# jklebes/MetropolisEngine

Measured on AMD Instinct MI355X. Metric: MC steps/sec (chains x sweeps) at 2^20 chains, 16 params, higher is better.
Workload: dtype f64

## Files before the change

### metropolisengine_amd/csrc/me_api.hip

```cpp
#include <algorithm>
#include <cmath>
#include <cstdlib>
#include <cstring>
#include <dlfcn.h>
#include <mutex>
#include <memory>
#include <string>
#include <atomic>
#include <chrono>
#include <vector>

#include "me_engine.h"

namespace me {

static std::vector<const KernelSet *> &registry() {
  static std::vector<const KernelSet *> sets;
  return sets;
}
static std::mutex &registry_mutex() {
  static std::mutex m;
  return m;
}
void register_kernel_set(const KernelSet *set) {
// ... 62 lines not shown
    for (int k = 0; k < j; ++k) s -= m[cre(j, k)] * m[cre(j, k)] + m[cim(j, k)] * m[cim(j, k)];
    if (!(s > 0)) return false;
    const double dg = std::sqrt(s);
    m[cdg(j)] = dg;
    for (int i = j + 1; i < nc; ++i) {
      double tr = m[cre(i, j)], ti = m[cim(i, j)];
      for (int k = 0; k < j; ++k) {
        const double ar = m[cre(i, k)], ai = m[cim(i, k)], br = m[cre(j, k)], bi = m[cim(j, k)];
        tr -= ar * br + ai * bi;
        ti -= ai * br - ar * bi;
      }
      m[cre(i, j)] = tr / dg;
      m[cim(i, j)] = ti / dg;
    }
  }
  return true;
}

static bool initial_shape_is_identity(const me_config *c) {
  if (c->covariance_real)
    for (int i = 0; i < c->n_real; ++i)
      for (int j = 0; j <= i; ++j)
        if (c->covariance_real[i * c->n_real + j] != (i == j ? 1.0 : 0.0)) return false;
  if (c->covariance_complex)
    for (int i = 0; i < c->n_complex; ++i)
      for (int j = 0; j <= i; ++j) {
        const double re = c->covariance_complex[2 * (i * c->n_complex + j)], im = c->covariance_complex[2 * (i * c->n_complex + j) + 1];
        if (re != (i == j ? 1.0 : 0.0) || (i != j && im != 0.0)) return false;
      }
  return true;
}

int fail(me_engine *e, int code, const std::string &msg) {
  if (e) e->err = msg;
  else g_create_error = msg;
  return code;
}

static void to_device_type(const double *src, size_t count, int dtype, std::vector<unsigned char> &out) {
  out.resize(count * (dtype == ME_F32 ? 4 : 8));
  if (dtype == ME_F32) {
    float *o = reinterpret_cast<float *>(out.data());
    for (size_t i = 0; i < count; ++i) o[i] = (float)src[i];
  } else {
    std::memcpy(out.data(), src, count * 8);
  }
}

hipError_t upload(DeviceBuffer &dst, const double *src, size_t count, int dtype) {
  std::vector<unsigned char> bytes;
  to_device_type(src, count, dtype, bytes);
  const hipError_t err = dst.resize(bytes.size());
  return err != hipSuccess ? err : hipMemcpy(dst.get(), bytes.data(), bytes.size(), hipMemcpyHostToDevice);
}

int refuse_stale_total(me_engine *e, const char *subject) {
  if (!e->stale_total) return ME_OK;
  return fail(e, ME_ERR_UNSUPPORTED, std::string(subject) + " not available with ME_FLAG_REFERENCE_ENERGY_LEDGERS: its two ledgers "
                                                            "make the energy of a chain ambiguous");
}

static int report_status(me_engine *e, unsigned int bits) {
  if (!bits) return ME_OK;
  ME_HIP(e, hipMemsetAsync(e->status.get(), 0, sizeof(unsigned int), e->stream));
  std::string msg = "numeric failure in at least one chain:";
  if (bits & ST_NONFINITE_ENERGY) msg += " non-finite energy;";
  if (bits & ST_BAD_PIVOT) msg += " non-positive Cholesky pivot (proposal covariance not positive definite);";
  if (bits & ST_BAD_WIDTH) msg += " sampling width <= 0;";
  return fail(e, ME_ERR_NUMERIC, msg);
}
int check_status(me_engine *e) {
  unsigned long long *scratch = e->host_scratch.get<unsigned long long>();
  ME_HIP(e, hipMemcpyAsync(&scratch[0], e->status.get(), sizeof(unsigned int), hipMemcpyDeviceToHost, e->stream));
  ME_HIP(e, hipStreamSynchronize(e->stream));
  return report_status(e, (unsigned int)scratch[0]);
}

}

using namespace me;

namespace {

int broadcast(me_engine *e, DeviceBuffer &dst, const std::vector<double> &row, bool tiled = false) {
  std::vector<unsigned char> bytes;
  to_device_type(row.data(), row.size(), e->dtype, bytes);
  ME_HIP(e, hipMemcpyAsync(e->row_dev.get(), bytes.data(), bytes.size(), hipMemcpyHostToDevice, e->stream));
  if (tiled) ME_HIP(e, launch_broadcast_tiled(dst.get(), e->row_dev.get(), (int)row.size(), e->n, e->dtype, e->stream));
  else ME_HIP(e, launch_broadcast_rows(dst.get(), e->row_dev.get(), (int)row.size(), e->n, e->dtype, e->stream));
  ME_HIP(e, hipStreamSynchronize(e->stream));
  return ME_OK;
}

template <typename T>
void gather_rows(const T *t, int comps, int64_t n_chains, double *dst) {
  for (int r = 0; r < comps; ++r)
    for (int64_t c = 0; c < n_chains; ++c) dst[c * comps + r] = (double)t[(size_t)r * n_chains + c];
}
template <typename T>
void scatter_rows(T *t, int comps, int64_t n_chains, const double *src) {
  for (int r = 0; r < comps; ++r)
    for (int64_t c = 0; c < n_chains; ++c) t[(size_t)r * n_chains + c] = (T)src[c * comps + r];
}
template <typename T>
void transpose_tiled(T *t, int entries, int64_t tile0, int64_t chain_begin, int64_t n_chains, double *dst, const double *src) {
  const size_t tile_values = (size_t)entries * 64;
  auto at = [&](int64_t c, int k) { return (size_t)((c >> 6) - tile0) * tile_values + (size_t)k * 64 + (size_t)(c & 63); };
  for (int64_t i = 0; i < n_chains; ++i)
    for (int k = 0; k < entries; ++k) {
      if (dst) dst[i * entries + k] = (double)t[at(chain_begin + i, k)];
      else t[at(chain_begin + i, k)] = (T)src[i * entries + k];
    }
}

int copy_tiled(me_engine *e, void *field_ptr, int entries, int64_t chain_begin, int64_t n_chains, double *dst, const double *src) {
  const int64_t tile0 = chain_begin >> 6, tile1 = (chain_begin + n_chains - 1) >> 6;
  const size_t tile_values = (size_t)entries * 64, n_values = (size_t)(tile1 - tile0 + 1) * tile_values;
  unsigned char *dev = (unsigned char *)field_ptr + (size_t)tile0 * tile_values * e->esize;
  std::vector<unsigned char> tmp(n_values * e->esize);
  const bool whole = (chain_begin & 63) == 0 && (((chain_begin + n_chains) & 63) == 0 || chain_begin + n_chains == e->n);
  if (dst || !whole) {
    ME_HIP(e, hipMemcpyAsync(tmp.data(), dev, tmp.size(), hipMemcpyDeviceToHost, e->stream));
    ME_HIP(e, hipStreamSynchronize(e->stream));
  }
  if (e->dtype == ME_F32) transpose_tiled(reinterpret_cast<float *>(tmp.data()), entries, tile0, chain_begin, n_chains, dst, src);
  else transpose_tiled(reinterpret_cast<double *>(tmp.data()), entries, tile0, chain_begin, n_chains, dst, src);
  if (src) {
    ME_HIP(e, hipMemcpyAsync(dev, tmp.data(), tmp.size(), hipMemcpyHostToDevice, e->stream));
    ME_HIP(e, hipStreamSynchronize(e->stream));
  }
  return dst ? check_status(e) : ME_OK;
}

int field_info(me_engine *e, int field, void **ptr, int *comps) {
  switch (field) {
    case ME_FIELD_PARAMS: *ptr = e->x.get(); *comps = e->d; return ME_OK;
    case ME_FIELD_ENERGY: *ptr = e->energy.get(); *comps = e->n_terms; return ME_OK;
    case ME_FIELD_WIDTH: *ptr = e->width.get(); *comps = e->width_rows; return ME_OK;
    case ME_FIELD_MEAN: *ptr = e->mean.get(); *comps = e->d; return ME_OK;
    case ME_FIELD_OBS_MEAN: *ptr = e->obs_mean.get(); *comps = e->nobs; return ME_OK;
    case ME_FIELD_COV:
      if (!e->cov)
        return fail(e, ME_ERR_UNSUPPORTED, "this engine keeps no per-chain covariance: for large parameter spaces it is "
                                           "kept on request only (me_config.flags: ME_FLAG_TRACK_COVARIANCE), and not "
                                           "at all where the field would pass 4 GiB");
      *ptr = e->cov.get(); *comps = e->p; return ME_OK;
    case ME_FIELD_ENERGY_TOTAL:
      if (!e->stale_total)
        return fail(e, ME_ERR_UNSUPPORTED, "this engine keeps one coherent energy ledger (sum ME_FIELD_ENERGY); a separate "
                                           "energy_total exists with ME_FLAG_REFERENCE_ENERGY_LEDGERS only");
      *ptr = e->energy.get<unsigned char>() + (size_t)e->n_terms * (size_t)e->n * e->esize; *comps = 1; return ME_OK;
    case ME_FIELD_FACTOR:
      if (!e->factor) return fail(e, ME_ERR_UNSUPPORTED, "this engine keeps no per-chain proposal factors (dimensions "
                                                         "without per-chain kernels, or a field beyond 4 GiB)");
      *ptr = e->factor.get(); *comps = e->p; return ME_OK;
    default: return fail(e, ME_ERR_INVALID, "unknown field id");
  }
}

int upload_shared_factor(me_engine *e, const double *packed) {
  ME_HIP(e, upload(e->shared_factor, packed, (size_t)e->p, e->dtype));
  if (e->shared_full) {
    std::vector<double> full((size_t)e->nr * e->nr, 0.0);
    for (int i = 0; i < e->nr; ++i)
      for (int j = 0; j <= i; ++j) full[(size_t)i * e->nr + j] = packed[i * (i + 1) / 2 + j];
    ME_HIP(e, upload(e->shared_full, full.data(), full.size(), e->dtype));
    if (e->shared_image) ME_HIP(e, e->ks->prepare_matrix(e->shared_full.get(), e->shared_image.get(), e->stream));
  }
  return ME_OK;
}

void fill_step_launch(me_engine *e, StepLaunch &l, int n_sweeps) {
  l.n_real = e->nr;
  l.n_complex = e->nc;
  l.x = e->x.get();
  l.energy = e->energy.get();
  l.width = e->width.get();
  l.factor = e->cov_kind == CK_PER_CHAIN ? e->factor.get() : e->shared_factor.get();
  l.factor_full = e->shared_full.get();
  l.factor_image = e->shared_image.get();
  l.energy_image = e->energy_image.get();
  l.coef_device = e->coef_dev.get();
  l.coef_host = e->coef.data();
  l.n_coef = (int)e->coef.size();
  l.inj_normals = nullptr;
  l.inj_uniforms = nullptr;
  l.group = GROUP_ALL;
  l.split_widths = (e->width_rows == 3 && !e->widths_synced) ? 1 : 0;
  l.stale_total = e->stale_total ? 1 : 0;
  l.cov = e->cov.get();
  l.accept_slots = e->accept_slots.get<unsigned long long>();
  l.status = e->status.get<unsigned int>();
  l.n = e->n;
  l.chain_offset = e->chain_offset;
  l.step_index = e->step_index;
  l.seed = e->seed;
  l.n_sweeps = n_sweeps;
  l.energy_kind = e->energy_kind;
  l.cov_kind = e->cov_kind;
  l.reject_kind = e->reject_kind;
  l.grid_blocks = e->grid_blocks;
  l.reject_bound = e->reject_bound;
  l.temp = e->temp;
  l.ratio = e->ratio;
  l.target_acceptance = e->target_acceptance;
  l.damping = std::max((double)e->measure_count / (double)e->m, 200.0);
  l.ladder = e->ladder.n_rungs ? e->ladder.table.get() : nullptr;
  l.tiles_per_rung = e->ladder.n_rungs ? (int)(e->n / (64ll * e->ladder.n_rungs)) : 0;
}
// ... 30 lines not shown
  return ME_OK;
}

int me_abi_version(void) { return ME_ABI_VERSION; }

int me_supported(int32_t dtype, int32_t n_real, int32_t n_complex, int32_t energy_kind) {
  return find_kernel_set(dtype, n_real, n_complex, energy_kind, nullptr) ? 1 : 0;
}

namespace {

int validate_config(const me_config *c, const KernelSet **ks_out) {
  if (c->abi_version != ME_ABI_VERSION) return fail(nullptr, ME_ERR_INVALID, "me_config.abi_version mismatch");
  if (c->n_real < 0 || c->n_complex < 0 || c->n_real + c->n_complex == 0)
    return fail(nullptr, ME_ERR_INVALID,
                "must give at least one real or complex parameter (metropolis_engine.py:37-39)");
  if (c->n_chains <= 0) return fail(nullptr, ME_ERR_INVALID, "n_chains must be positive");
  if (!(c->temp >= 0)) return fail(nullptr, ME_ERR_INVALID, "temp must be >= 0 (metropolis_engine.py:92)");
  if (!(c->target_acceptance > 0 && c->target_acceptance < 1))
    return fail(nullptr, ME_ERR_INVALID, "target_acceptance must be in (0, 1)");
  if (!(c->sampling_width > 0)) return fail(nullptr, ME_ERR_INVALID, "sampling_width must be > 0");
  if (c->dtype != ME_F32 && c->dtype != ME_F64) return fail(nullptr, ME_ERR_INVALID, "unknown dtype");
  if (!c->initial_params) return fail(nullptr, ME_ERR_INVALID, "initial_params is required");
  if (c->n_energy_coeffs < 0 || (c->n_energy_coeffs > 0 && !c->energy_coeffs))
    return fail(nullptr, ME_ERR_INVALID, "energy coefficients missing");
  int rc = check_reject_kind(nullptr, c->reject_kind, c->energy_kind, c->n_real);
  if (rc != ME_OK) return rc;
  if (c->cov_mode < ME_COV_REFERENCE || c->cov_mode > ME_COV_POOLED)
    return fail(nullptr, ME_ERR_INVALID, "unknown cov_mode");
  const KernelSet *ks = *ks_out = find_kernel_set(c->dtype, c->n_real, c->n_complex, c->energy_kind, c->user_energy_name);
  if (!ks) {
    if (is_user_kind(c->energy_kind))
      return fail(nullptr, ME_ERR_UNSUPPORTED,
                  std::string("no user-energy plugin named '") + (c->user_energy_name ? c->user_energy_name : "") +
                      "' is loaded for these dimensions (build it with metropolisengine_amd.build.build_user_energy "
                      "and load it with me_load_plugin)");
    if (!has_dims(c->dtype, c->n_real, c->n_complex))
      return fail(nullptr, ME_ERR_UNSUPPORTED,
                  "no kernel set compiled for (dtype, n_real, n_complex) = (" + std::to_string(c->dtype) + ", " +
                      std::to_string(c->n_real) + ", " + std::to_string(c->n_complex) + ")");
    return fail(nullptr, ME_ERR_UNSUPPORTED, "energy kind " + std::to_string(c->energy_kind) +
                                                  " is not compiled for these dimensions");
  }
  if ((rc = check_user_reject(nullptr, c->reject_kind, ks)) != ME_OK) return rc;
  if (ks->n_real < 0) {
    if (c->cov_mode == ME_COV_POOLED && c->n_complex > 0)
      return fail(nullptr, ME_ERR_UNSUPPORTED,
                  "parameter spaces beyond " + std::to_string(kMaxRegisterDof) + " real degrees of freedom with complex "
                  "parameters run with the identity proposal shape (ME_COV_FIXED, cov_mode=\"fixed\") or per-chain shapes "
                  "(ME_COV_REFERENCE); one shared factor (ME_COV_POOLED) is there for pure real spaces");
    const bool starts_shared = !initial_shape_is_identity(c) && c->cov_mode != ME_COV_REFERENCE;
    if (starts_shared && c->n_complex > 0)
      return fail(nullptr, ME_ERR_UNSUPPORTED,
                  "parameter spaces beyond " + std::to_string(kMaxRegisterDof) + " real degrees of freedom with complex "
                  "parameters run with the identity proposal shape only: leave covariance_matrix_real / _complex unset");
    {
      const long long per_block = (long long)(c->n_real + 2 * c->n_complex) * 64 * (c->dtype == ME_F32 ? 4 : 8);
      const bool dense = c->energy_kind == ME_ENERGY_DENSE_QUAD, pooled = c->cov_mode == ME_COV_POOLED || starts_shared;
      const bool per_chain = c->cov_mode == ME_COV_REFERENCE || (c->flags & ME_FLAG_TRACK_COVARIANCE) != 0;
      if ((dense || pooled || per_chain) && per_block * (pooled ? 2 : 1) > 150 * 1024)
        return fail(nullptr, ME_ERR_UNSUPPORTED,
                    "a dense quadratic form, a shared proposal factor or per-chain shapes beyond " + std::to_string(kMaxRegisterDof) +
                        " degrees of freedom are staged in LDS: this many parameters do not fit (float64: about 290, 145 with "
                        "a shared factor or an initial covariance that ME_COV_FIXED keeps; float32 twice that)");
    }
    if (c->flags & ME_FLAG_REFERENCE_ENERGY_LEDGERS)
      return fail(nullptr, ME_ERR_UNSUPPORTED, "ME_FLAG_REFERENCE_ENERGY_LEDGERS is not available beyond " +
                                                   std::to_string(kMaxRegisterDof) + " real degrees of freedom");
    if (c->reject_kind == ME_REJECT_USER) return fail(nullptr, ME_ERR_UNSUPPORTED, "no user plugins at these dimensions");
  }
  if ((c->flags & ME_FLAG_REFERENCE_ENERGY_LEDGERS) && (c->n_real == 0 || c->n_complex == 0))
    return fail(nullptr, ME_ERR_INVALID,
                "ME_FLAG_REFERENCE_ENERGY_LEDGERS applies to mixed engines (real and complex parameters): only their "
                "step_all keeps a separate energy_total (metropolis_engine.py:241-259)");
  if (c->cov_mode == ME_COV_REFERENCE && !ks->per_chain_cov)
    return fail(nullptr, ME_ERR_UNSUPPORTED,
                "per-chain adaptive covariance is not compiled for these dimensions; use ME_COV_FIXED or ME_COV_POOLED");
  return ME_OK;
}

struct Layout {
  bool keep_per_chain;
  bool keep_cov;
  bool x_tiled;
  int width_rows;
};
int decide_layout(const me_config *c, const KernelSet *ks, Layout &l) {
  const long long esz = c->dtype == ME_F32 ? 4 : 8, limit = 1ll << 32, padded = padded_chains(c->n_chains);
  l.keep_per_chain = ks->per_chain_cov && (!ks->streams_packed || c->cov_mode == ME_COV_REFERENCE);
  if (l.keep_per_chain && !ks->streams_packed && (long long)packed_total(c->n_real, c->n_complex) * padded * esz >= limit) {
    if (c->cov_mode == ME_COV_REFERENCE)
      return fail(nullptr, ME_ERR_UNSUPPORTED,
                  "the per-chain covariance field would exceed 4 GiB on this engine; shard the chains over more "
                  "engines or use ME_COV_FIXED / ME_COV_POOLED");
    l.keep_per_chain = false;
  }
  const long long rows = std::max<long long>(c->n_real + 2 * c->n_complex, 2 * c->n_real + c->n_complex);
  if (rows * padded * esz >= limit)
    return fail(nullptr, ME_ERR_UNSUPPORTED,
                "a per-chain field would exceed 4 GiB on this engine; shard the chains over more engines");
  l.keep_cov = l.keep_per_chain ||
               ((!ks->per_chain_cov || ks->streams_packed) && ks->tracks_cov && (c->flags & ME_FLAG_TRACK_COVARIANCE));
  l.x_tiled = ks->tiled_state;
  l.width_rows = (c->n_real > 0 && c->n_complex > 0) ? 3 : 1;
  return ME_OK;
}

std::unique_ptr<me_engine> configure(const me_config *c, const KernelSet *ks, const Layout &l) {
  std::unique_ptr<me_engine> e(new me_engine);
  e->device = c->device_id;
  e->ks = ks;
  e->n_terms = ks->energy_terms(c->energy_kind);
  e->dtype = c->dtype;
  e->esize = c->dtype == ME_F32 ? 4 : 8;
  e->n = c->n_chains;
  e->nr = c->n_real;
  e->nc = c->n_complex;
  e->d = e->nr + 2 * e->nc;
  e->p = packed_total(e->nr, e->nc);
  e->nobs = n_observables(e->nr, e->nc);
  e->chain_offset = c->chain_offset;
  e->seed = c->seed;
  e->temp = c->temp;
  e->target_acceptance = c->target_acceptance;
  e->energy_kind = c->energy_kind;
  e->reject_kind = c->reject_kind;
  e->reject_bound = c->reject_bound;
  e->cov_mode = c->cov_mode;
  e->coef.assign(c->energy_coeffs, c->energy_coeffs + c->n_energy_coeffs);
  e->alpha = -norm_ppf(c->target_acceptance / 2.0);
  e->m = e->nr + e->nc;
  e->ratio = (1.0 - 1.0 / e->m) * std::sqrt(2.0 * M_PI) * std::exp(e->alpha * e->alpha / 2.0) / 2.0 * e->alpha +
             1.0 / (e->m * c->target_acceptance * (1.0 - c->target_acceptance));
  if (const char *g = std::getenv("ME_GRID_BLOCKS")) e->grid_blocks = std::atoi(g);
  e->x_tiled = l.x_tiled;
  e->stale_total = (c->flags & ME_FLAG_REFERENCE_ENERGY_LEDGERS) != 0;
  e->width_rows = l.width_rows;
  e->n_slots = (e->n + 31) / 32 + 8;
  return e;
}

int allocate(me_engine *e, const Layout &l) {
  const KernelSet *ks = e->ks;
  ME_HIP(e, hipSetDevice(e->device));
  ME_HIP(e, e->stream.create());
  const size_t n = (size_t)e->n, tiles = (size_t)padded_chains(e->n), es = e->esize;
  ME_HIP(e, e->x.resize((e->x_tiled ? tiles : n) * e->d * es));
  ME_HIP(e, e->energy.resize(n * (e->n_terms + (e->stale_total ? 1 : 0)) * es));
  ME_HIP(e, e->width.resize(n * e->width_rows * es));
  ME_HIP(e, e->mean.resize(n * e->d * es));
  ME_HIP(e, e->obs_mean.resize(n * e->nobs * es));
  if (l.keep_cov) ME_HIP(e, e->cov.resize(tiles * e->p * es));
  if (l.keep_per_chain) ME_HIP(e, e->factor.resize(tiles * e->p * es));
  ME_HIP(e, e->shared_factor.resize((size_t)e->p * es));
  if (e->nc == 0) ME_HIP(e, e->shared_full.resize((size_t)e->nr * e->nr * es));
  if (e->shared_full && ks->prepare_matrix) ME_HIP(e, e->shared_image.resize(ks->matrix_image_bytes));
  ME_HIP(e, e->row_dev.resize((size_t)std::max(std::max(e->d, e->p), e->nobs) * es));
  ME_HIP(e, e->accept_slots.resize((size_t)e->n_slots * sizeof(unsigned long long)));
  ME_HIP(e, e->accept_total.resize(sizeof(unsigned long long)));
  ME_HIP(e, e->status.resize(sizeof(unsigned int)));
  const size_t moments_bytes = sizeof(double) * (size_t)moments_size(e->nr, e->nc);
  ME_HIP(e, e->pool.dev.resize(moments_bytes));
  ME_HIP(e, e->host_scratch.allocate(64));
  e->host_scratch.get<unsigned long long>()[0] = e->host_scratch.get<unsigned long long>()[1] = 0;
  ME_HIP(e, e->pool.host.allocate(moments_bytes));
  if (pool_reduce_supported(e->nr, e->nc, e->dtype))
    ME_HIP(e, e->pool.partials.resize(sizeof(double) * (size_t)pool_reduce_blocks(e->n, e->nr, e->nc) *
                                      (size_t)(1 + e->d + e->nr + e->nc + e->d * (e->d + 1) / 2)));
  ME_HIP(e, hipMemsetAsync(e->accept_slots.get(), 0, e->accept_slots.bytes(), e->stream));
  ME_HIP(e, hipMemsetAsync(e->status.get(), 0, sizeof(unsigned int), e->stream));
  return ME_OK;
}

int upload_coefficients(me_engine *e) {
  const std::vector<double> &coef = e->coef;
  const bool runtime_dims = e->ks->n_real < 0;
  std::vector<double> form;
  if (runtime_dims && e->energy_kind == ME_ENERGY_DIAG_QUAD) {
    if ((int)coef.size() != e->nr + e->nc) return fail(e, ME_ERR_INVALID, "wrong number of energy coefficients for this energy kind");
    form.assign(coef.begin(), coef.end());
    form.insert(form.end(), coef.begin() + e->nr, coef.end());
  } else if (runtime_dims && e->energy_kind == ME_ENERGY_DENSE_QUAD) {
    if ((int)coef.size() != e->d * e->d) return fail(e, ME_ERR_INVALID, "wrong number of energy coefficients for this energy kind");
    form.reserve((size_t)e->d * (e->d + 1) / 2);
    for (int i = 0; i < e->d; ++i)
      for (int j = 0; j <= i; ++j)
        form.push_back(i == j ? coef[(size_t)i * e->d + i] : coef[(size_t)i * e->d + j] + coef[(size_t)j * e->d + i]);
  } else if (e->energy_kind == ME_ENERGY_DENSE_QUAD || (is_user_kind(e->energy_kind) && !coef.empty())) {
    form = coef;
  } else {
    return ME_OK;
  }
  ME_HIP(e, upload(e->coef_dev, form.data(), form.size(), e->dtype));
  if (!runtime_dims && e->energy_kind == ME_ENERGY_DENSE_QUAD && e->ks->prepare_matrix) {
    ME_HIP(e, e->energy_image.resize(e->ks->matrix_image_bytes));
    ME_HIP(e, e->ks->prepare_matrix(e->coef_dev.get(), e->energy_image.get(), e->stream));
  }
  return ME_OK;
}

int initial_state(me_engine *e, const me_config *c) {
  std::vector<double> init(c->initial_params, c->initial_params + e->d);
  std::vector<double> obs(e->nobs);
  for (int i = 0; i < e->nr; ++i) {
    obs[i] = std::fabs(init[i]);
    obs[e->nr + e->nc + i] = init[i] * init[i];
  }
  for (int j = 0; j < e->nc; ++j) obs[e->nr + j] = std::hypot(init[e->nr + j], init[e->nr + e->nc + j]);
  const int pr = packed_real(e->nr);
  std::vector<double> c0(e->p, 0.0);
  bool identity = true;
  for (int i = 0; i < e->nr; ++i)
    for (int j = 0; j <= i; ++j) {
      const double v = c->covariance_real ? c->covariance_real[i * e->nr + j] : (i == j ? 1.0 : 0.0);
      c0[i * (i + 1) / 2 + j] = v;
      identity = identity && v == (i == j ? 1.0 : 0.0);
    }
  for (int i = 0; i < e->nc; ++i) {
    for (int j = 0; j < i; ++j) {
      const double re = c->covariance_complex ? c->covariance_complex[2 * (i * e->nc + j)] : 0.0;
      const double im = c->covariance_complex ? c->covariance_complex[2 * (i * e->nc + j) + 1] : 0.0;
      c0[pr + i * i + 2 * j] = re;
      c0[pr + i * i + 2 * j + 1] = im;
      identity = identity && re == 0.0 && im == 0.0;
    }
    const double dg = c->covariance_complex ? c->covariance_complex[2 * (i * e->nc + i)] : 1.0;
    c0[pr + i * i + 2 * i] = dg;
    identity = identity && dg == 1.0;
  }
  std::vector<double> f0 = c0;
  for (int i = 0; i < e->nc; ++i)
    for (int j = 0; j < i; ++j) f0[pr + i * i + 2 * j + 1] = -f0[pr + i * i + 2 * j + 1];
  if (!host_factor(f0, e->nr, e->nc))
    return fail(e, ME_ERR_INVALID, "initial covariance matrix is not positive definite (metropolis_engine.py:270)");
  int rc = ME_OK;
  std::vector<double> width_row((size_t)e->width_rows, c->sampling_width);
  if ((rc = broadcast(e, e->x, init, e->x_tiled)) || (rc = broadcast(e, e->mean, init)) || (rc = broadcast(e, e->obs_mean, obs)) ||
      (rc = broadcast(e, e->width, width_row)) || (e->cov && (rc = broadcast(e, e->cov, c0, true))) ||
      (e->factor && (rc = broadcast(e, e->factor, f0, true))) || (rc = upload_shared_factor(e, f0.data())))
    return rc;
  e->cov_kind = identity ? CK_IDENTITY : (e->ks->n_real < 0 && e->factor) ? CK_PER_CHAIN : CK_SHARED;
  return ME_OK;
}

int initial_energy(me_engine *e) {
  const int rc = me_recompute_energy(e);
  if (rc != ME_OK) return rc;
  const hipError_t herr = hipStreamSynchronize(e->stream);
  if (herr != hipSuccess) return fail(e, ME_ERR_HIP, std::string("initial energy evaluation: ") + hipGetErrorString(herr));
  return ME_OK;
}

}

int me_create(const me_config *c, me_engine **out) {
  if (!c || !out) return fail(nullptr, ME_ERR_INVALID, "null config or output pointer");
  *out = nullptr;
  const KernelSet *ks = nullptr;
  Layout layout;
  int rc;
  if ((rc = validate_config(c, &ks)) || (rc = decide_layout(c, ks, layout))) return rc;
  int n_dev = 0;
  if (hipGetDeviceCount(&n_dev) != hipSuccess || n_dev <= 0)
    return fail(nullptr, ME_ERR_HIP, "no HIP device available (this library has no CPU fallback)");
  if (c->device_id < 0 || c->device_id >= n_dev) return fail(nullptr, ME_ERR_INVALID, "device_id out of range");

  std::unique_ptr<me_engine> e = configure(c, ks, layout);
  if ((rc = allocate(e.get(), layout)) || (rc = upload_coefficients(e.get())) || (rc = initial_state(e.get(), c)) ||
      (rc = initial_energy(e.get())))
    return fail(nullptr, rc, e->err);
  *out = e.release();
  return ME_OK;
}

int me_set_reject_condition(me_engine *e, int32_t reject_kind, double reject_bound) {
  if (!e) return ME_ERR_INVALID;
  int rc;
  if ((rc = check_reject_kind(e, reject_kind, e->energy_kind, e->nr)) || (rc = check_user_reject(e, reject_kind, e->ks))) return rc;
  e->reject_kind = reject_kind;
  e->reject_bound = reject_bound;
  return ME_OK;
}

int me_set_energy(me_engine *e, int32_t energy_kind, const double *coeffs, int32_t n_coeffs, const char *user_name) {
  if (!e) return ME_ERR_INVALID;
  if (n_coeffs < 0 || (n_coeffs > 0 && !coeffs)) return fail(e, ME_ERR_INVALID, "energy coefficients missing");
  if (e->ks->n_real < 0) return fail(e, ME_ERR_UNSUPPORTED, "me_set_energy: not available on the runtime-dimension kernel set");
  if (energy_kind == ME_ENERGY_DENSE_QUAD)
    return fail(e, ME_ERR_UNSUPPORTED, "me_set_energy: the dense quadratic form keeps device images of its matrix; create a new engine");
  const KernelSet *ks = find_kernel_set(e->dtype, e->nr, e->nc, energy_kind, user_name);
  if (!ks || ks->n_real < 0)
    return fail(e, ME_ERR_UNSUPPORTED, is_user_kind(energy_kind)
                    ? std::string("no user-energy plugin named '") + (user_name ? user_name : "") + "' is loaded for these dimensions"
                    : "energy kind " + std::to_string(energy_kind) + " is not compiled for these dimensions");
  if (ks->tiled_state != e->ks->tiled_state || ks->per_chain_cov != e->ks->per_chain_cov || ks->streams_packed != e->ks->streams_packed ||
      ks->tracks_cov != e->ks->tracks_cov)
    return fail(e, ME_ERR_UNSUPPORTED, "me_set_energy: the plugin was built with other per-chain covariance options than this engine's kernel set");
  if (e->reject_kind == ME_REJECT_USER && !ks->has_user_reject)
    return fail(e, ME_ERR_UNSUPPORTED, "me_set_energy: the engine's wall is the plugin's me_user_reject, which the new energy does not define");
  const int n_terms = ks->energy_terms(energy_kind);
  ME_HIP(e, hipSetDevice(e->device));
  ME_HIP(e, hipStreamSynchronize(e->stream));
  DeviceBuffer ledger, coef_dev;
  if (n_terms != e->n_terms)
    ME_HIP(e, ledger.resize((size_t)e->n * (size_t)(n_terms + (e->stale_total ? 1 : 0)) * e->esize));
  if (is_user_kind(energy_kind) && n_coeffs > 0) ME_HIP(e, upload(coef_dev, coeffs, (size_t)n_coeffs, e->dtype));
  if (n_terms != e->n_terms) {
    e->energy = std::move(ledger);
    e->n_terms = n_terms;
    if (e->trace.chains > 0) e->trace.restart();
  }
  e->coef.assign(coeffs, coeffs + n_coeffs);
  e->coef_dev = std::move(coef_dev);
  e->ks = ks;
  e->energy_kind = energy_kind;
  const int rc = me_recompute_energy(e);
  if (rc != ME_OK) return rc;
  ME_HIP(e, hipStreamSynchronize(e->stream));
  return check_status(e);
}

int me_load_plugin(const char *path) {
  if (!path) return fail(nullptr, ME_ERR_INVALID, "null plugin path");
  void *handle = dlopen(path, RTLD_NOW | RTLD_GLOBAL);
  if (!handle) return fail(nullptr, ME_ERR_INVALID, std::string("dlopen failed: ") + dlerror());
  return ME_OK;
}

int me_destroy(me_engine *e) {
  if (!e) return ME_ERR_INVALID;
  (void)hipSetDevice(e->device);
  if (e->stream) (void)hipStreamSynchronize(e->stream);
  if (e->pool.copy_stream) (void)hipStreamSynchronize(e->pool.copy_stream);
  delete e;
  return ME_OK;
}

int me_recompute_energy(me_engine *e) {
  if (!e) return ME_ERR_INVALID;
  ME_HIP(e, hipSetDevice(e->device));
  EnergyLaunch l;
  l.n_real = e->nr;
  l.n_complex = e->nc;
  l.total_row = e->stale_total ? e->n_terms : -1;
  l.x = e->x.get();
  l.energy = e->energy.get();
  l.coef_device = e->coef_dev.get();
  l.coef_host = e->coef.data();
  l.n_coef = (int)e->coef.size();
  l.status = e->status.get<unsigned int>();
  l.n = e->n;
  l.energy_kind = e->energy_kind;
  l.grid_blocks = e->grid_blocks;
  hipError_t err = e->ks->init_energy(l, e->stream);
  if (err == hipErrorInvalidValue) return fail(e, ME_ERR_INVALID, "wrong number of energy coefficients for this energy kind");
  ME_HIP(e, err);
  return ME_OK;
}

static int split_widths(me_engine *e) {
  if (e->width_rows != 3 || !e->widths_synced) return ME_OK;
  const size_t row = (size_t)e->n * e->esize;
  for (int r = 1; r <= 2; ++r)
    ME_HIP(e, hipMemcpyAsync(e->width.get<unsigned char>() + r * row, e->width.get(), row, hipMemcpyDeviceToDevice, e->stream));
  e->widths_synced = false;
  return ME_OK;
}

static int resolve_step_kind(me_engine *e, int kind, int *group, bool *magphase) {
  *magphase = false;
  *group = GROUP_ALL;
  const bool mixed = e->nr > 0 && e->nc > 0;
  switch (kind) {
    case ME_STEP_ALL: return ME_OK;
    case ME_STEP_REAL_GROUP:
      if (e->nr == 0) return fail(e, ME_ERR_INVALID, "this engine has no real parameters");
      *group = mixed ? GROUP_REAL : GROUP_ALL;
      return ME_OK;
// ... 28 lines not shown
  l.group = group;
  l.inj_normals = inj_normals;
  l.inj_uniforms = inj_uniforms;
  hipError_t err = magphase ? e->ks->magphase(l, e->stream) : e->ks->step(l, e->stream);
  if (err == hipErrorNotSupported) return fail(e, ME_ERR_UNSUPPORTED, "this step kind is not compiled for this engine");
  ME_HIP(e, err);
  count_steps(e, n_sweeps, group, magphase);
  return ME_OK;
}

int me_step(me_engine *e, int32_t n_sweeps) { return me_step_kind(e, ME_STEP_ALL, n_sweeps); }

int me_step_kind(me_engine *e, int32_t kind, int32_t n_sweeps) {
  if (!e) return ME_ERR_INVALID;
  if (n_sweeps <= 0) return fail(e, ME_ERR_INVALID, "n_sweeps must be positive");
  ME_HIP(e, hipSetDevice(e->device));
  return launch_step_kind(e, kind, n_sweeps, nullptr, nullptr);
}

int me_step_injected(me_engine *e, int32_t kind, int32_t n_sweeps, const double *normals, const double *uniforms) {
  if (!e || !normals || !uniforms) return ME_ERR_INVALID;
  if (n_sweeps <= 0) return fail(e, ME_ERR_INVALID, "n_sweeps must be positive");
  if (e->dtype != ME_F64) return fail(e, ME_ERR_UNSUPPORTED, "injected-stream replay is compiled for float64 engines only");
  ME_HIP(e, hipSetDevice(e->device));
  const bool magphase = kind == ME_STEP_COMPLEX_MAGNITUDE_PHASE;
  const size_t n = (size_t)e->n, k = (size_t)n_sweeps;
  const size_t nz = magphase ? (size_t)e->nc : (size_t)e->d, nu = magphase ? (size_t)e->nc + 2 : 1;
  std::vector<double> zn(k * nz * n), un(k * nu * n);
  for (size_t s = 0; s < k; ++s)
    for (size_t c = 0; c < n; ++c) {
      for (size_t j = 0; j < nz; ++j) zn[(s * nz + j) * n + c] = normals[(s * n + c) * nz + j];
      for (size_t j = 0; j < nu; ++j) un[(s * nu + j) * n + c] = uniforms[(s * n + c) * nu + j];
    }
  DeviceBuffer zd, ud;
  ME_HIP(e, zd.resize(zn.size() * sizeof(double)));
  if (ud.resize(un.size() * sizeof(double)) != hipSuccess) return fail(e, ME_ERR_HIP, "hipMalloc of the injected uniforms failed");
  if (hipMemcpy(zd.get(), zn.data(), zd.bytes(), hipMemcpyHostToDevice) != hipSuccess ||
      hipMemcpy(ud.get(), un.data(), ud.bytes(), hipMemcpyHostToDevice) != hipSuccess)
    return fail(e, ME_ERR_HIP, "upload of the injected streams failed");
  int rc = launch_step_kind(e, kind, n_sweeps, zd.get(), ud.get());
  if (rc == ME_OK && hipStreamSynchronize(e->stream) != hipSuccess) rc = fail(e, ME_ERR_HIP, "injected step failed");
  return rc;
}

namespace {
void fill_measure_launch(me_engine *e, MeasureLaunch &l, unsigned long long count) {
  l.n_real = e->nr;
  l.n_complex = e->nc;
  l.x = e->x.get();
  l.width = e->width.get();
  l.mean = e->mean.get();
  l.cov = e->cov.get();
  l.obs_mean = e->obs_mean.get();
  l.factor = e->factor.get();
  l.status = e->status.get<unsigned int>();
  l.n = e->n;
  l.measure_count = count;
  l.update_cov = (count > 50 && e->cov) ? 1 : 0;
  l.split_widths = (e->width_rows == 3 && !e->widths_synced) ? 1 : 0;
  l.write_factor = (l.update_cov && e->cov_mode == ME_COV_REFERENCE) ? 1 : 0;
  l.grid_blocks = e->grid_blocks;
}

int commit_measure(me_engine *e, const MeasureLaunch &l) {
  e->measure_count = l.measure_count;
  if (l.write_factor) e->cov_kind = CK_PER_CHAIN;
  if (e->trace.chains > 0) {
    const long long cols = e->d + e->n_terms + e->width_rows;
    if (e->trace.rows == e->trace.capacity) {
      const long long cap = e->trace.capacity ? 2 * e->trace.capacity : 1024;
      DeviceBuffer bigger;
      ME_HIP(e, bigger.resize(sizeof(double) * (size_t)(cap * cols * e->trace.chains)));
      if (e->trace.dev) {
        ME_HIP(e, hipMemcpyAsync(bigger.get(), e->trace.dev.get(), sizeof(double) * (size_t)(e->trace.rows * cols * e->trace.chains),
                                 hipMemcpyDeviceToDevice, e->stream));
        ME_HIP(e, hipStreamSynchronize(e->stream));
      }
      e->trace.dev = std::move(bigger);
      e->trace.capacity = cap;
    }
    const int rows_valid = (e->width_rows == 3 && e->widths_synced) ? 1 : e->width_rows;
    double *row = e->trace.dev.get<double>() + e->trace.rows * cols * e->trace.chains;
    ME_HIP(e, launch_trace(e->x.get(), e->energy.get(), e->width.get(), e->n, e->d, e->n_terms, rows_valid, e->dtype, e->trace.chains,
                           e->trace.stride, row, e->stream, e->x_tiled));
    if (rows_valid != e->width_rows) {
      double *widths = row + (size_t)(e->d + e->n_terms) * e->trace.chains;
      for (int r = 1; r < 3; ++r)
        ME_HIP(e, hipMemcpyAsync(widths + (size_t)r * e->trace.chains, widths, sizeof(double) * (size_t)e->trace.chains,
                                 hipMemcpyDeviceToDevice, e->stream));
    }
    e->trace.rows += 1;
  }
  return ME_OK;
}
}

int me_measure(me_engine *e) {
  if (!e) return ME_ERR_INVALID;
  ME_HIP(e, hipSetDevice(e->device));
  MeasureLaunch l;
  fill_measure_launch(e, l, e->measure_count + 1);
  ME_HIP(e, e->ks->measure(l, e->stream));
  return commit_measure(e, l);
}

int me_cycle(me_engine *e, int32_t n_sweeps) {
  if (!e) return ME_ERR_INVALID;
  if (n_sweeps <= 0) return fail(e, ME_ERR_INVALID, "n_sweeps must be positive");
  ME_HIP(e, hipSetDevice(e->device));
  if (e->ks->cycle) {
    StepLaunch sl;
    fill_step_launch(e, sl, n_sweeps);
    MeasureLaunch ml;
    fill_measure_launch(e, ml, e->measure_count + 1);
    ml.split_widths = 0;
    const hipError_t err = e->ks->cycle(sl, ml, e->stream);
    if (err == hipSuccess) {
      count_steps(e, n_sweeps);
      e->fused_cycles += 1;
      return commit_measure(e, ml);
    }
    if (err != hipErrorNotSupported) ME_HIP(e, err);
    (void)hipGetLastError();
  }
  const int rc = me_step(e, n_sweeps);
  return rc != ME_OK ? rc : me_measure(e);
}

int me_cycle_stats(me_engine *e, uint64_t *fused_cycles) {
  if (!e || !fused_cycles) return ME_ERR_INVALID;
  *fused_cycles = e->fused_cycles;
  return ME_OK;
}

int me_trace_enable(me_engine *e, int64_t n_traced, int64_t stride) {
  if (!e) return ME_ERR_INVALID;
  if (n_traced < 0 || stride < 1 || (n_traced > 0 && (n_traced - 1) * stride >= e->n))
    return fail(e, ME_ERR_INVALID, "traced chains out of range");
  ME_HIP(e, hipSetDevice(e->device));
  ME_HIP(e, hipStreamSynchronize(e->stream));
  e->trace.restart();
  e->trace.chains = n_traced;
  e->trace.stride = stride;
  return ME_OK;
}

int me_trace_shape(me_engine *e, int64_t *rows, int64_t *cols, int64_t *n_traced) {
  if (!e) return ME_ERR_INVALID;
  if (rows) *rows = e->trace.rows;
  if (cols) *cols = e->d + e->n_terms + e->width_rows;
  if (n_traced) *n_traced = e->trace.chains;
  return ME_OK;
}

int me_trace_get(me_engine *e, double *dst, int64_t n_doubles) {
  if (!e || !dst) return ME_ERR_INVALID;
  const long long want = e->trace.rows * (e->d + e->n_terms + e->width_rows) * e->trace.chains;
  if (n_doubles != want) return fail(e, ME_ERR_INVALID, "wrong trace buffer length");
  if (want == 0) return ME_OK;
  ME_HIP(e, hipSetDevice(e->device));
  ME_HIP(e, hipStreamSynchronize(e->stream));
  ME_HIP(e, hipMemcpy(dst, e->trace.dev.get(), sizeof(double) * (size_t)want, hipMemcpyDeviceToHost));
  return ME_OK;
}

int me_field_components(me_engine *e, int32_t field, int32_t *n_components) {
  if (!e || !n_components) return ME_ERR_INVALID;
  void *ptr;
  int comps;
  int rc = field_info(e, field, &ptr, &comps);
  if (rc == ME_OK) *n_components = comps;
  return rc;
}

int me_energy_terms(me_engine *e, int32_t *n_terms) {
  if (!e || !n_terms) return ME_ERR_INVALID;
  *n_terms = e->n_terms;
  return ME_OK;
}

int me_get(me_engine *e, int32_t field, int64_t chain_begin, int64_t n_chains, double *dst) {
  if (!e || !dst) return ME_ERR_INVALID;
  if (chain_begin < 0 || n_chains < 0 || chain_begin + n_chains > e->n) return fail(e, ME_ERR_INVALID, "chain range out of bounds");
  ME_HIP(e, hipSetDevice(e->device));
  void *ptr;
  int comps;
  int rc = field_info(e, field, &ptr, &comps);
  if (rc != ME_OK) return rc;
  if (n_chains == 0) return ME_OK;
  if (field == ME_FIELD_COV || field == ME_FIELD_FACTOR || (field == ME_FIELD_PARAMS && e->x_tiled))
    return copy_tiled(e, ptr, comps, chain_begin, n_chains, dst, nullptr);
  std::vector<unsigned char> tmp((size_t)comps * n_chains * e->esize);
  for (int r = 0; r < comps; ++r)
    ME_HIP(e, hipMemcpyAsync(tmp.data() + (size_t)r * n_chains * e->esize,
                             (const unsigned char *)ptr + ((size_t)r * e->n + chain_begin) * e->esize,
                             (size_t)n_chains * e->esize, hipMemcpyDeviceToHost, e->stream));
  ME_HIP(e, hipStreamSynchronize(e->stream));
  if (e->dtype == ME_F32) gather_rows(reinterpret_cast<const float *>(tmp.data()), comps, n_chains, dst);
  else gather_rows(reinterpret_cast<const double *>(tmp.data()), comps, n_chains, dst);
  if (field == ME_FIELD_WIDTH && e->width_rows == 3 && e->widths_synced)
    for (int64_t c = 0; c < n_chains; ++c) dst[c * 3 + 1] = dst[c * 3 + 2] = dst[c * 3];
  return check_status(e);
}

int me_set(me_engine *e, int32_t field, int64_t chain_begin, int64_t n_chains, const double *src) {
  if (!e || !src) return ME_ERR_INVALID;
  if (chain_begin < 0 || n_chains < 0 || chain_begin + n_chains > e->n) return fail(e, ME_ERR_INVALID, "chain range out of bounds");
  ME_HIP(e, hipSetDevice(e->device));
  void *ptr;
  int comps;
  int rc = field_info(e, field, &ptr, &comps);
  if (rc != ME_OK) return rc;
  if (field == ME_FIELD_WIDTH && e->width_rows == 3 && (chain_begin != 0 || n_chains != e->n))
    return fail(e, ME_ERR_INVALID, "widths of a mixed engine must be set for all chains at once");
  if (n_chains == 0) return ME_OK;
  if (field == ME_FIELD_COV || field == ME_FIELD_FACTOR || (field == ME_FIELD_PARAMS && e->x_tiled)) {
    rc = copy_tiled(e, ptr, comps, chain_begin, n_chains, nullptr, src);
    if (rc != ME_OK) return rc;
    if (field == ME_FIELD_FACTOR) e->cov_kind = CK_PER_CHAIN;
    return ME_OK;
  }
  std::vector<unsigned char> tmp((size_t)comps * n_chains * e->esize);
  if (e->dtype == ME_F32) scatter_rows(reinterpret_cast<float *>(tmp.data()), comps, n_chains, src);
  else scatter_rows(reinterpret_cast<double *>(tmp.data()), comps, n_chains, src);
  for (int r = 0; r < comps; ++r)
    ME_HIP(e, hipMemcpyAsync((unsigned char *)ptr + ((size_t)r * e->n + chain_begin) * e->esize,
                             tmp.data() + (size_t)r * n_chains * e->esize, (size_t)n_chains * e->esize,
                             hipMemcpyHostToDevice, e->stream));
  ME_HIP(e, hipStreamSynchronize(e->stream));
  if (field == ME_FIELD_FACTOR) e->cov_kind = CK_PER_CHAIN;
  if (field == ME_FIELD_WIDTH && e->width_rows == 3) e->widths_synced = false;
  return ME_OK;
}

int me_constants(me_engine *e, double *alpha, int32_t *m, double *ratio) {
  if (!e) return ME_ERR_INVALID;
  if (alpha) *alpha = e->alpha;
  if (m) *m = e->m;
  if (ratio) *ratio = e->ratio;
  return ME_OK;
}

int me_counters(me_engine *e, uint64_t *step_index, uint64_t *measure_step_counter) {
  if (!e) return ME_ERR_INVALID;
  if (step_index) *step_index = e->step_index;
  if (measure_step_counter) *measure_step_counter = e->measure_count;
  return ME_OK;
}

int me_set_counters(me_engine *e, uint64_t step_index, uint64_t measure_step_counter) {
  if (!e) return ME_ERR_INVALID;
  if (measure_step_counter < 1) return fail(e, ME_ERR_INVALID, "measure_step_counter starts at 1");
  e->step_index = step_index;
  e->measure_count = measure_step_counter;
  return ME_OK;
}

int me_accept_stats(me_engine *e, uint64_t *accepted, uint64_t *proposed) {
  if (!e) return ME_ERR_INVALID;
  ME_HIP(e, hipSetDevice(e->device));
  unsigned long long *scratch = e->host_scratch.get<unsigned long long>();
  ME_HIP(e, launch_sum_slots(e->accept_slots.get<unsigned long long>(), e->n_slots, e->accept_total.get<unsigned long long>(), e->stream));
  ME_HIP(e, hipMemcpyAsync(&scratch[1], e->accept_total.get(), sizeof(unsigned long long), hipMemcpyDeviceToHost, e->stream));
  ME_HIP(e, hipMemcpyAsync(&scratch[0], e->status.get(), sizeof(unsigned int), hipMemcpyDeviceToHost, e->stream));
  ME_HIP(e, hipStreamSynchronize(e->stream));
  if (accepted) *accepted = scratch[1];
  if (proposed) *proposed = e->proposed;
  return report_status(e, (unsigned int)scratch[0]);
}

int me_set_accept_stats(me_engine *e, uint64_t accepted, uint64_t proposed) {
  if (!e) return ME_ERR_INVALID;
  if (accepted > proposed) return fail(e, ME_ERR_INVALID, "accepted exceeds proposed");
  ME_HIP(e, hipSetDevice(e->device));
  const unsigned long long total = accepted;
  ME_HIP(e, hipMemsetAsync(e->accept_slots.get(), 0, e->accept_slots.bytes(), e->stream));
  ME_HIP(e, hipMemcpyAsync(e->accept_slots.get(), &total, sizeof(total), hipMemcpyHostToDevice, e->stream));
  ME_HIP(e, hipStreamSynchronize(e->stream));
  e->proposed = proposed;
  return ME_OK;
}

int me_pooled_moments_size(me_engine *e, int64_t *n_doubles) {
  if (!e || !n_doubles) return ME_ERR_INVALID;
  *n_doubles = moments_size(e->nr, e->nc);
  return ME_OK;
}

int me_pooled_moments_geometry(me_engine *e, int32_t *matrix_core, int32_t *tile_chains, int32_t *partial_rows) {
  if (!e || !matrix_core || !tile_chains || !partial_rows) return ME_ERR_INVALID;
  if (!e->pool.partials) return fail(e, ME_ERR_UNSUPPORTED, "pooled moments: dimension too large for the reduction kernel");
  *matrix_core = e->ks->pool_stage1 ? 1 : 0;
  *tile_chains = e->ks->pool_stage1 ? 64 : pool_tile_chains(e->nr, e->nc, e->dtype);
  *partial_rows = pool_reduce_blocks(e->n, e->nr, e->nc);
  return ME_OK;
}

namespace {
hipError_t wait_polling(hipEvent_t ev) {
  const auto t0 = std::chrono::steady_clock::now();
  for (;;) {
    const hipError_t rc = hipEventQuery(ev);
    if (rc != hipErrorNotReady) return rc;
    if (std::chrono::steady_clock::now() - t0 > std::chrono::milliseconds(2)) return hipEventSynchronize(ev);
  }
}
hipError_t wait_polling(hipStream_t stream) {
  const auto t0 = std::chrono::steady_clock::now();
  for (;;) {
    const hipError_t rc = hipStreamQuery(stream);
    if (rc != hipErrorNotReady) return rc;
    if (std::chrono::steady_clock::now() - t0 > std::chrono::milliseconds(2)) return hipStreamSynchronize(stream);
  }
}

int check_pooled(me_engine *e, int64_t n_doubles) {
  if (n_doubles != moments_size(e->nr, e->nc)) return fail(e, ME_ERR_INVALID, "wrong pooled-moment buffer length");
  if (e->pool.pending) return fail(e, ME_ERR_STATE, "a pooled-moment reduction is in flight (me_pooled_moments_end first)");
  if (!e->pool.partials) return fail(e, ME_ERR_UNSUPPORTED, "pooled moments: dimension too large for the reduction kernel");
  ME_HIP(e, hipSetDevice(e->device));
  return ME_OK;
}
int enqueue_pool_reduce(me_engine *e, const void *x, long long n_chains, long long n_slots, double proposed, double *device_out) {
  hipError_t err = launch_pool_reduce(x, n_chains, e->nr, e->nc, e->dtype, e->accept_slots.get<unsigned long long>(), n_slots, proposed,
                                      e->pool.partials.get<double>(), device_out, e->stream, e->ks->pool_stage1, e->x_tiled);
  if (err == hipErrorInvalidValue) return fail(e, ME_ERR_UNSUPPORTED, "pooled moments: dimension too large for the reduction kernel");
  ME_HIP(e, err);
  return ME_OK;
}
int enqueue_pooled_moments(me_engine *e, double *device_out, int64_t n_doubles) {
  const int rc = check_pooled(e, n_doubles);
  return rc != ME_OK ? rc : enqueue_pool_reduce(e, e->x.get(), e->n, e->n_slots, (double)e->proposed, device_out);
}
int fetch_pooled_moments(me_engine *e, double *host_out, int64_t n_doubles) {
  const size_t bytes = sizeof(double) * (size_t)n_doubles;
  ME_HIP(e, hipMemcpyAsync(e->pool.host.get<double>(), e->pool.dev.get(), bytes, hipMemcpyDeviceToHost, e->stream));
  ME_HIP(e, wait_polling(e->stream));
  std::memcpy(host_out, e->pool.host.get<double>(), bytes);
  return ME_OK;
}
}

int me_pooled_moments_device(me_engine *e, void *device_out, int64_t n_doubles) {
  if (!e || !device_out) return ME_ERR_INVALID;
  int rc = enqueue_pooled_moments(e, (double *)device_out, n_doubles);
  if (rc != ME_OK) return rc;
  ME_HIP(e, wait_polling(e->stream));
  return ME_OK;
}

int me_pooled_moments(me_engine *e, double *host_out, int64_t n_doubles) {
  if (!e || !host_out) return ME_ERR_INVALID;
  const int rc = enqueue_pooled_moments(e, e->pool.dev.get<double>(), n_doubles);
  return rc != ME_OK ? rc : fetch_pooled_moments(e, host_out, n_doubles);
}

int me_pooled_moments_range(me_engine *e, int64_t chain_begin, int64_t n_chains, double *host_out, int64_t n_doubles) {
  if (!e || !host_out) return ME_ERR_INVALID;
  if (chain_begin < 0 || n_chains <= 0 || chain_begin + n_chains > e->n || chain_begin % 64 != 0 || n_chains % 64 != 0)
    return fail(e, ME_ERR_INVALID, "the chain range must be whole 64-chain tiles inside the engine");
  int rc = check_pooled(e, n_doubles);
  if (rc != ME_OK) return rc;
  const unsigned char *x = e->x.get<unsigned char>();
  if (e->x_tiled) {
    x += (size_t)chain_begin * e->d * e->esize;
  } else {
    const size_t row = (size_t)n_chains * e->esize;
    if (row * e->d > e->pool.range_x.bytes()) {
      ME_HIP(e, hipStreamSynchronize(e->stream));
      ME_HIP(e, e->pool.range_x.reserve(row * e->d));
    }
    ME_HIP(e, hipMemcpy2DAsync(e->pool.range_x.get(), row, x + (size_t)chain_begin * e->esize, (size_t)e->n * e->esize, row, (size_t)e->d,
                               hipMemcpyDeviceToDevice, e->stream));
    x = e->pool.range_x.get<unsigned char>();
  }
  if ((rc = enqueue_pool_reduce(e, x, n_chains, 0, 0.0, e->pool.dev.get<double>())) != ME_OK) return rc;
  return fetch_pooled_moments(e, host_out, n_doubles);
}

namespace {
int begin_pooled(me_engine *e, bool allreduce) {
  if (e->pool.pending) return fail(e, ME_ERR_STATE, "a pooled-moment reduction is already in flight: call me_pooled_moments_end first");
  if (allreduce && !e->comm)
    return fail(e, ME_ERR_STATE, "this engine has no communicator: call me_comm_init_rank first (single-GPU engines use me_pooled_moments)");
  ME_HIP(e, hipSetDevice(e->device));
  if (!e->pool.copy_stream) {
    ME_HIP(e, e->pool.copy_stream.create());
    ME_HIP(e, e->pool.reduced.create(hipEventDisableTiming));
    ME_HIP(e, e->pool.copied.create(hipEventDisableTiming));
  }
  const int64_t n_doubles = moments_size(e->nr, e->nc);
  int rc = enqueue_pooled_moments(e, e->pool.dev.get<double>(), n_doubles);
  if (rc != ME_OK) return rc;
  ME_HIP(e, hipEventRecord(e->pool.reduced, e->stream));
  ME_HIP(e, hipStreamWaitEvent(e->pool.copy_stream, e->pool.reduced, 0));
  if (allreduce) {
    const ncclResult_t nrc = e->rccl->all_reduce(e->pool.dev.get<double>(), e->pool.dev.get<double>(), (size_t)n_doubles, ncclDouble, ncclSum, e->comm, e->pool.copy_stream);
    if (nrc != ncclSuccess) return fail(e, ME_ERR_HIP, std::string("ncclAllReduce: ") + e->rccl->error_string(nrc));
  }
  ME_HIP(e, hipMemcpyAsync(e->pool.host.get<double>(), e->pool.dev.get<double>(), sizeof(double) * (size_t)n_doubles, hipMemcpyDeviceToHost, e->pool.copy_stream));
  ME_HIP(e, hipEventRecord(e->pool.copied, e->pool.copy_stream));
  e->pool.pending = true;
  return ME_OK;
}
}

int me_pooled_moments_begin(me_engine *e) {
  if (!e) return ME_ERR_INVALID;
  return begin_pooled(e, false);
}

int me_pooled_moments_allreduce_begin(me_engine *e) {
  if (!e) return ME_ERR_INVALID;
  return begin_pooled(e, true);
}

int me_pooled_moments_allreduce(me_engine *e, double *host_out, int64_t n_doubles) {
  if (!e || !host_out) return ME_ERR_INVALID;
  if (n_doubles != moments_size(e->nr, e->nc)) return fail(e, ME_ERR_INVALID, "wrong pooled-moment buffer length");
  const int rc = begin_pooled(e, true);
  return rc != ME_OK ? rc : me_pooled_moments_end(e, host_out, n_doubles);
}

int me_comm_unique_id(void *id_out, size_t bytes) {
  if (!id_out || bytes != ME_COMM_ID_BYTES) return fail(nullptr, ME_ERR_INVALID, "the unique id is ME_COMM_ID_BYTES bytes");
  static_assert(sizeof(ncclUniqueId) == ME_COMM_ID_BYTES, "ME_COMM_ID_BYTES must be sizeof(ncclUniqueId)");
  std::string err;
  const RcclApi *api = rccl_api(&err);
  if (!api) return fail(nullptr, ME_ERR_UNSUPPORTED, err);
  ncclUniqueId id;
  const ncclResult_t nrc = api->get_unique_id(&id);
  if (nrc != ncclSuccess) return fail(nullptr, ME_ERR_HIP, std::string("ncclGetUniqueId: ") + api->error_string(nrc));
  std::memcpy(id_out, &id, sizeof(id));
  return ME_OK;
}

int me_comm_init_rank(me_engine *e, const void *unique_id, size_t bytes, int32_t rank, int32_t world) {
  if (!e || !unique_id) return ME_ERR_INVALID;
  if (bytes != ME_COMM_ID_BYTES) return fail(e, ME_ERR_INVALID, "the unique id is ME_COMM_ID_BYTES bytes");
  if (world < 1 || rank < 0 || rank >= world) return fail(e, ME_ERR_INVALID, "rank out of range");
  if (e->comm) return fail(e, ME_ERR_STATE, "this engine already has a communicator (me_comm_destroy first)");
  if (e->pool.pending) return fail(e, ME_ERR_STATE, "a pooled-moment reduction is in flight");
  std::string err;
  const RcclApi *api = rccl_api(&err);
  if (!api) return fail(e, ME_ERR_UNSUPPORTED, err);
  ME_HIP(e, hipSetDevice(e->device));
  ncclUniqueId id;
// ... 118 lines not shown
```

### metropolisengine_amd/csrc/me_device.h

```cpp
#pragma once

#include <type_traits>
#include <utility>

#include <hip/hip_runtime.h>
#include <stdint.h>

#include "me_internal.h"
#include "me_math64.h"

namespace me {

struct U4 {
  uint32_t x, y, z, w;
};

__device__ __forceinline__ uint32_t xor3(uint32_t a, uint32_t b, uint32_t c) {
  return __builtin_amdgcn_bitop3_b32(a, b, c, 0x96);
}
__device__ __forceinline__ U4 philox4x32_10(U4 c, uint32_t k0, uint32_t k1) {
#pragma unroll
  for (int r = 0; r < 10; ++r) {
    const uint64_t p0 = (uint64_t)0xD2511F53u * c.x;
    const uint64_t p1 = (uint64_t)0xCD9E8D57u * c.z;
// ... 129 lines not shown
  __device__ __forceinline__ void store(int row, unsigned int chain_off, R value) const {
    if constexpr (sizeof(R) == 4) {
      __builtin_amdgcn_raw_buffer_store_b32(__builtin_bit_cast(unsigned int, value), rsrc, chain_off,
                                            (unsigned int)row * row_bytes, 0);
    } else {
      using v2 = decltype(__builtin_amdgcn_raw_buffer_load_b64(rsrc, 0u, 0u, 0));
      __builtin_amdgcn_raw_buffer_store_b64(__builtin_bit_cast(v2, value), rsrc, chain_off,
                                            (unsigned int)row * row_bytes, 0);
    }
  }
};

template <typename R>
__device__ __forceinline__ R chain_energy(const Field<R> &fe, unsigned int chain_off, int n_terms) {
  R e = fe.load(0, chain_off);
  for (int t = 1; t < n_terms; ++t) e = e + fe.load(t, chain_off);
  return e;
}

template <typename R>
__device__ __forceinline__ unsigned int tiled_offset(long long c, int entries) {
  return (unsigned int)(((c >> 6) * (long long)entries * 64 + (c & 63)) * (long long)sizeof(R));
}
template <typename R>
struct TiledField {
  __amdgpu_buffer_rsrc_t rsrc;
  __device__ __forceinline__ TiledField(const R *base, long long n, int entries)
      : rsrc(__builtin_amdgcn_make_buffer_rsrc(const_cast<R *>(base), 0,
                                               (unsigned int)(((n + 63) >> 6) * (long long)entries * 64 * (long long)sizeof(R)),
                                               0x00020000)) {}
  static constexpr unsigned int kEntryBytes = 64u * (unsigned int)sizeof(R);
  template <int AUX>
  __device__ __forceinline__ R load_aux(int k, unsigned int tile_off) const {
    if constexpr (sizeof(R) == 4) {
      return __builtin_bit_cast(R, __builtin_amdgcn_raw_buffer_load_b32(rsrc, tile_off, (unsigned int)k * kEntryBytes, AUX));
    } else {
      const auto v = __builtin_amdgcn_raw_buffer_load_b64(rsrc, tile_off, (unsigned int)k * kEntryBytes, AUX);
      return __builtin_bit_cast(R, v);
    }
  }
  template <int AUX>
  __device__ __forceinline__ void store_aux(int k, unsigned int tile_off, R value) const {
    if constexpr (sizeof(R) == 4) {
      __builtin_amdgcn_raw_buffer_store_b32(__builtin_bit_cast(unsigned int, value), rsrc, tile_off, (unsigned int)k * kEntryBytes, AUX);
    } else {
      using v2 = decltype(__builtin_amdgcn_raw_buffer_load_b64(rsrc, 0u, 0u, 0));
      __builtin_amdgcn_raw_buffer_store_b64(__builtin_bit_cast(v2, value), rsrc, tile_off, (unsigned int)k * kEntryBytes, AUX);
    }
  }
  __device__ __forceinline__ R load(int k, unsigned int tile_off) const { return load_aux<0>(k, tile_off); }
  __device__ __forceinline__ R load_nt(int k, unsigned int tile_off) const { return load_aux<ME_NT_AUX>(k, tile_off); }
  __device__ __forceinline__ void store(int k, unsigned int tile_off, R value) const { store_aux<0>(k, tile_off, value); }
  __device__ __forceinline__ void store_nt(int k, unsigned int tile_off, R value) const { store_aux<ME_NT_AUX>(k, tile_off, value); }
};

template <bool NT, class F>
__device__ __forceinline__ auto packed_load(const F &f, int row, unsigned int chain_off) {
  if constexpr (NT) return f.load_nt(row, chain_off);
  else return f.load(row, chain_off);
}
template <bool NT, class F, typename R>
__device__ __forceinline__ void packed_store(const F &f, int row, unsigned int chain_off, R value) {
  if constexpr (NT) f.store_nt(row, chain_off, value);
  else f.store(row, chain_off, value);
}

template <typename R, bool NTS>
struct StateField : Field<R> {
  using Field<R>::Field;
  __device__ __forceinline__ R load(int row, unsigned int chain_off) const {
    if constexpr (NTS) return Field<R>::load_nt(row, chain_off);
    else return Field<R>::load(row, chain_off);
  }
  __device__ __forceinline__ void store(int row, unsigned int chain_off, R value) const {
    if constexpr (NTS) Field<R>::store_nt(row, chain_off, value);
    else Field<R>::store(row, chain_off, value);
  }
};

#ifndef ME_TILED_STATE_DOF
#define ME_TILED_STATE_DOF 16
#endif
constexpr int kTiledStateDof = ME_TILED_STATE_DOF;
template <typename R, int D, bool NTS = false>
struct XField {
  static constexpr bool kTiled = D >= kTiledStateDof;
  std::conditional_t<kTiled, TiledField<R>, StateField<R, NTS>> f;
  __device__ __forceinline__ XField(const R *base, long long n) : f(base, n, D) {}
  static __device__ __forceinline__ unsigned int offset(long long c) {
    if constexpr (kTiled) return tiled_offset<R>(c, D);
    else return (unsigned int)c * (unsigned int)sizeof(R);
  }
  __device__ __forceinline__ R load(int row, unsigned int off) const {
    if constexpr (kTiled && NTS) return f.load_nt(row, off);
    else return f.load(row, off);
  }
  __device__ __forceinline__ void store(int row, unsigned int off, R value) const {
    if constexpr (kTiled && NTS) f.store_nt(row, off, value);
    else f.store(row, off, value);
  }
};
template <typename R, int D>
__device__ __forceinline__ long long state_index(long long c, int row, long long n) {
  if constexpr (D >= kTiledStateDof) return ((c >> 6) * (long long)D + row) * 64 + (c & 63);
  else return (long long)row * n + c;
}

constexpr int kMaxPackedInRegisters = 160;
#ifndef ME_STREAM_F64_ENTRIES
#define ME_STREAM_F64_ENTRIES 96
#endif
constexpr int kStreamF64Entries = ME_STREAM_F64_ENTRIES;

template <typename R, int NR, int NC>
struct EnergyIso {
  static constexpr int D = NR + 2 * NC;
  R a;
  __device__ __forceinline__ R operator()(const R (&x)[D]) const {
    R s0 = 0, s1 = 0;
#pragma unroll
    for (int d = 0; d + 1 < D; d += 2) {
      s0 += x[d] * x[d];
      s1 += x[d + 1] * x[d + 1];
    }
    if constexpr (D % 2 == 1) s0 += x[D - 1] * x[D - 1];
    return a * (s0 + s1);
  }
};

template <typename R, int NR, int NC>
struct EnergyDiag {
  static constexpr int D = NR + 2 * NC;
  R w[D];
  __device__ __forceinline__ R operator()(const R (&x)[D]) const {
    R s0 = 0, s1 = 0;
#pragma unroll
    for (int d = 0; d + 1 < D; d += 2) {
      s0 += w[d] * x[d] * x[d];
      s1 += w[d + 1] * x[d + 1] * x[d + 1];
    }
    if constexpr (D % 2 == 1) s0 += w[D - 1] * x[D - 1] * x[D - 1];
    return s0 + s1;
  }
};

template <typename R, int NR, int NC>
struct EnergyDense {
  static constexpr int D = NR + 2 * NC;
  static constexpr int PT = D * (D + 1) / 2;
  const R *a;
  static __device__ __forceinline__ R *folded() {
    __shared__ R t[PT];
    return t;
  }
  __device__ __forceinline__ void prepare() const {
    R *t = folded();
    constexpr int kBatch = 8;
    for (int k0 = threadIdx.x; k0 < PT; k0 += kBatch * (int)blockDim.x) {
      R lo[kBatch], hi[kBatch];
#pragma unroll
      for (int u = 0; u < kBatch; ++u) {
        const int k = k0 + u * (int)blockDim.x;
        lo[u] = hi[u] = R(0);
        if (k < PT) {
          int i = (int)((__builtin_sqrtf((float)(8 * k + 1)) - 1.0f) * 0.5f);
          if ((i + 1) * (i + 2) / 2 <= k) ++i;
          if (i * (i + 1) / 2 > k) --i;
          const int j = k - i * (i + 1) / 2;
          lo[u] = a[i * D + j];
          if (i != j) hi[u] = a[j * D + i];
        }
      }
#pragma unroll
      for (int u = 0; u < kBatch; ++u) {
        const int k = k0 + u * (int)blockDim.x;
        if (k < PT) t[k] = lo[u] + hi[u];
      }
    }
    __syncthreads();
  }
  __device__ __forceinline__ R operator()(const R (&x)[D]) const {
    const R *t = folded();
    asm volatile("" ::: "memory");
    R e = 0;
#pragma unroll
    for (int i = 0; i < D; ++i) {
      R y = 0;
#pragma unroll
// ... 237 lines not shown
  constexpr int NW = 2 * ((D + 1) / 2);
  constexpr int NBLK = (NW + 1 + 3) / 4;
  using N_ = Num<R>;
  [[maybe_unused]] const unsigned long long step = a.step_index + (unsigned long long)s;
  if constexpr (INJECT) {
#pragma unroll
    for (int j = 0; j < D; ++j) g[j] = a.inj_normals[((long long)s * D + j) * a.n + c];
    u = a.inj_uniforms[(long long)s * a.n + c];
  } else {
    uint32_t words[4 * NBLK];
#pragma unroll
    for (int b = 0; b < NBLK; ++b) {
      const U4 o = philox_block(gid, step, b, a.seed_lo, a.seed_hi);
      words[4 * b + 0] = o.x;
      words[4 * b + 1] = o.y;
      words[4 * b + 2] = o.z;
      words[4 * b + 3] = o.w;
    }
#pragma unroll
    for (int q = 0; q < NW / 2; ++q) N_::normal_pair(words[2 * q], words[2 * q + 1], g[2 * q], g[2 * q + 1]);
    u = N_::unit(words[NW]);
  }

}

template <typename R, int NR, int NC, int CK, int GROUP, class Fac>
__device__ __forceinline__ void propose_registers(const R (&x)[NR + 2 * NC], const R (&g)[2 * ((NR + 2 * NC + 1) / 2)], R w_r, R w_c,
                                                  Fac &&fac, R (&xp)[NR + 2 * NC]) {
  constexpr int D = NR + 2 * NC;
  [[maybe_unused]] constexpr int PR = NR * (NR + 1) / 2;
  constexpr bool MOVE_REAL = NR > 0 && GROUP != GROUP_COMPLEX;
  constexpr bool MOVE_COMPLEX = NC > 0 && GROUP != GROUP_REAL;
#pragma unroll
  for (int d = 0; d < D; ++d) xp[d] = x[d];
  if constexpr (CK == CK_IDENTITY) {
    if constexpr (MOVE_REAL) {
#pragma unroll
      for (int i = 0; i < NR; ++i) xp[i] = x[i] + w_r * g[i];
    }
    if constexpr (MOVE_COMPLEX) {
#pragma unroll
      for (int j = 0; j < NC; ++j) {
        xp[NR + j] = x[NR + j] + w_c * (g[NR + j] * R(0.70710678118654752440));
        xp[NR + NC + j] = x[NR + NC + j] + w_c * (g[NR + NC + j] * R(0.70710678118654752440));
      }
    }
  } else {
    if constexpr (MOVE_REAL) {
#pragma unroll
      for (int i = 0; i < NR; ++i) {
        R acc = 0;
#pragma unroll
        for (int j = 0; j <= i; ++j) acc += fac(tri(i, j)) * g[j];
        xp[i] = x[i] + w_r * acc;
      }
    }
    if constexpr (MOVE_COMPLEX) {
#pragma unroll
      for (int i = 0; i < NC; ++i) {
        R are = 0, aim = 0;
#pragma unroll
        for (int j = 0; j < i; ++j) {
          const R lre = fac(cre(PR, i, j));
          const R lim = fac(cim(PR, i, j));
          const R wre = g[NR + j] * R(0.70710678118654752440), wim = g[NR + NC + j] * R(0.70710678118654752440);
          are += lre * wre - lim * wim;
          aim += lre * wim + lim * wre;
        }
        const R ld = fac(cdiag(PR, i));
        are += ld * (g[NR + i] * R(0.70710678118654752440));
        aim += ld * (g[NR + NC + i] * R(0.70710678118654752440));
        xp[NR + i] = x[NR + i] + w_c * are;
        xp[NR + NC + i] = x[NR + NC + i] + w_c * aim;
      }
    }
  }

}

template <typename R, int NR, int NC, class Energy, int CK, int GROUP, bool LADDER, class Ledger>
__device__ __forceinline__ void decide_step(const StepArgs<R> &a, long long c, const Energy &en, bool stale_total, R u,
                                            const R (&g)[2 * ((NR + 2 * NC + 1) / 2)], R (&x)[NR + 2 * NC], const R (&xp)[NR + 2 * NC],
                                            Ledger &ledger, R &total_q5, R &w, R &w_r, R &w_c, unsigned int &wave_accepted,
                                            bool &bad_energy) {
  [[maybe_unused]] constexpr int D = NR + 2 * NC;
  constexpr bool MOVE_REAL = NR > 0 && GROUP != GROUP_COMPLEX;
  constexpr bool MOVE_COMPLEX = NC > 0 && GROUP != GROUP_REAL;
  using N_ = Num<R>;
  bool rejected = false;
  if (a.reject_kind == ME_REJECT_ABS_REAL0_GE) rejected = !(N_::abs_(xp[0]) < a.reject_bound);
  else if (a.reject_kind == ME_REJECT_USER) rejected = energy_reject(en, xp, 0);
  R terms_new[Ledger::T];
  const R e_new = ledger.propose(en, xp, terms_new);
  const R diff = e_new - (stale_total ? total_q5 : ledger.partial());
  bool accept = diff <= R(0);
  if constexpr (LADDER) accept = accept || uphill_at<true>(a, c, u, diff);
  else if (a.temp > R(0)) accept = accept || N_::uphill(u, diff, a.inv_temp, a.inv_temp_log2e);
  accept = accept && !rejected;
  bad_energy |= (!rejected && !N_::finite(e_new));
  if constexpr (CK == CK_IDENTITY) {
    const R wa_r = accept ? w_r : R(0), wa_c = accept ? w_c : R(0);
    if constexpr (MOVE_REAL) {
#pragma unroll
      for (int i = 0; i < NR; ++i) x[i] = x[i] + wa_r * g[i];
    }
    if constexpr (MOVE_COMPLEX) {
#pragma unroll
      for (int j = 0; j < NC; ++j) {
        x[NR + j] = x[NR + j] + wa_c * (g[NR + j] * R(0.70710678118654752440));
        x[NR + NC + j] = x[NR + NC + j] + wa_c * (g[NR + NC + j] * R(0.70710678118654752440));
      }
    }
  } else {
#pragma unroll
    for (int d = 0; d < D; ++d) x[d] = accept ? xp[d] : x[d];
  }
  if (stale_total) total_q5 = accept ? e_new : total_q5;
  else ledger.commit(accept, terms_new);
  w = N_::adapt(w, accept, a.ratio, a.p, a.damping, a.up, a.down);
  if constexpr (GROUP == GROUP_ALL) w_r = w_c = w;
  else if constexpr (GROUP == GROUP_REAL) w_r = w;
  else w_c = w;
  wave_accepted += (unsigned int)__popcll(__ballot(accept));
}

template <typename R, int NR, int NC, class Energy, int CK, bool INJECT, int GROUP, bool LADDER, class Ledger, class Fac>
__device__ __forceinline__ void run_sweeps(const StepArgs<R> &a, const Energy &en, long long c, unsigned long long gid,
                                           bool stale_total, R (&x)[NR + 2 * NC], Ledger &ledger, R &total_q5, R &w, R &w_r,
                                           R &w_c, Fac &&fac, unsigned int &wave_accepted, bool &bad_energy) {
  constexpr int D = NR + 2 * NC;
  constexpr int NW = 2 * ((D + 1) / 2);
  for (int s = 0; s < a.n_sweeps; ++s) {
    R g[NW], u, xp[D];
    draw_step<R, NR, NC, INJECT>(a, c, gid, s, g, u);
    propose_registers<R, NR, NC, CK, GROUP>(x, g, w_r, w_c, fac, xp);
    decide_step<R, NR, NC, Energy, CK, GROUP, LADDER>(a, c, en, stale_total, u, g, x, xp, ledger, total_q5, w, w_r, w_c, wave_accepted, bad_energy);
  }
}

#ifndef ME_STEP_WAVES_PER_EU
#define ME_STEP_WAVES_PER_EU 0
#endif
#if ME_STEP_WAVES_PER_EU > 0
#define ME_STEP_BOUNDS __launch_bounds__(kFusedStepThreads, ME_STEP_WAVES_PER_EU)
#else
#define ME_STEP_BOUNDS __launch_bounds__(kFusedStepThreads)
#endif

#ifndef ME_STEP_PRIO_SHIFT
#define ME_STEP_PRIO_SHIFT 8
#endif
__device__ __forceinline__ void stagger_priority() {
#if ME_STEP_PRIO_SHIFT >= 0
  switch ((blockIdx.x >> ME_STEP_PRIO_SHIFT) & 3u) {
    case 0: __builtin_amdgcn_s_setprio(3); break;
    case 1: __builtin_amdgcn_s_setprio(2); break;
    case 2: __builtin_amdgcn_s_setprio(1); break;
    default: break;
  }
#endif
}

template <typename R, int NR, int NC, class Energy, int CK, bool INJECT = false, int GROUP = GROUP_ALL, bool NTS = false,
          bool LADDER = false>
__global__ void ME_STEP_BOUNDS k_step(StepArgs<R> a, Energy en) {
  constexpr int D = NR + 2 * NC;
  constexpr bool MIXED = NR > 0 && NC > 0;
  static_assert(GROUP == GROUP_ALL || MIXED, "group-wise kernels exist for mixed engines only");
  using N_ = Num<R>;

  stagger_priority();
  if constexpr (!INJECT) N_::prepare();
  energy_prepare(en, 0);
  unsigned int wave_accepted = 0;
  bool bad_energy = false, bad_width = false;
  const long long stride = (long long)gridDim.x * blockDim.x;
  using Ledger = EnergyLedger<R, Energy, GROUP>;
  const XField<R, D, NTS> fx(a.x, a.n);
  const StateField<R, NTS> fe(a.energy, a.n, Ledger::T + (MIXED ? 1 : 0)), fw(a.width, a.n, MIXED ? 3 : 1);
  const bool stale_total = MIXED && GROUP == GROUP_ALL && a.stale_total != 0;
  constexpr bool PER_CHAIN = CK == CK_PER_CHAIN || CK == CK_PER_CHAIN_NT;
  constexpr int PF = PER_CHAIN ? NR * (NR + 1) / 2 + NC * NC : 0;
  constexpr bool STREAM_FACTOR = PER_CHAIN && (PF > kMaxPackedInRegisters ||
                                               (!INJECT && sizeof(R) == 8 && NC == 0 && PF > kStreamF64Entries));
  const TiledField<R> ffac(a.factor, a.n, STREAM_FACTOR ? 0 : PF);
  for (long long c = (long long)blockIdx.x * blockDim.x + threadIdx.x; c < a.n; c += stride) {
    const unsigned int coff = (unsigned int)c * (unsigned int)sizeof(R);
    const unsigned int xoff = fx.offset(c);
    R x[D];
#pragma unroll
    for (int d = 0; d < D; ++d) x[d] = fx.load(d, xoff);
    Ledger ledger;
    R total_q5 = R(0);
    if (stale_total) total_q5 = fe.load(Ledger::T, coff);
    else ledger.load(fe, coff);
    R w = fw.load(MIXED ? GROUP : 0, coff);
    R w_r = w, w_c = w;
    if constexpr (MIXED && GROUP == GROUP_ALL) {
      if (a.split_widths) {
        w_r = fw.load(GROUP_REAL, coff);
        w_c = fw.load(GROUP_COMPLEX, coff);
      }
    }
    const unsigned long long gid = a.chain_offset + (unsigned long long)c;
    [[maybe_unused]] const unsigned int toff = tiled_offset<R>(c, PF);
    auto fac = [&](int k) -> R {
      if constexpr (CK == CK_PER_CHAIN_NT) return ffac.load_nt(k, toff);
      else if constexpr (CK == CK_PER_CHAIN) return ffac.load(k, toff);
      else return a.factor[k];
    };

    if constexpr (STREAM_FACTOR) {
      constexpr int NW = 2 * ((D + 1) / 2);
      for (int s = 0; s < a.n_sweeps; ++s) {
        static_assert(!INJECT, "the streamed-factor form has no replay hook");
        constexpr int NBLK = (NW + 1 + 3) / 4;
        const unsigned long long step = a.step_index + (unsigned long long)s;
        R g[NW];
        R u_accept;
        {
          uint32_t words[4 * NBLK];
#pragma unroll
          for (int b = 0; b < NBLK; ++b) {
            const U4 o = philox_block(gid, step, b, a.seed_lo, a.seed_hi);
            words[4 * b + 0] = o.x;
            words[4 * b + 1] = o.y;
            words[4 * b + 2] = o.z;
            words[4 * b + 3] = o.w;
          }
#pragma unroll
          for (int q = 0; q < NW / 2; ++q) N_::normal_pair(words[2 * q], words[2 * q + 1], g[2 * q], g[2 * q + 1]);
          u_accept = N_::unit(words[NW]);
        }
        R xp[D];
#pragma unroll
        for (int d = 0; d < D; ++d) xp[d] = x[d];
        asm volatile("" ::: "memory");
        constexpr int CH = (int)(ME_STREAM_CHUNK_BYTES / sizeof(R));
        const R *tile_base = a.factor + (c >> 6) * (long long)PF * 64;
        const unsigned long long tb = (unsigned long long)tile_base;
        const R *tile_uniform = (const R *)join_halves(__builtin_amdgcn_readfirstlane((int)(tb >> 32)),
                                                       __builtin_amdgcn_readfirstlane((int)(unsigned int)tb));
        const __amdgpu_buffer_rsrc_t tile = __builtin_amdgcn_make_buffer_rsrc(const_cast<R *>(tile_uniform), 0,
                                                                               (unsigned int)(PF * 64 * sizeof(R)), 0x00020000);
        const unsigned int lane_off = (unsigned int)(c & 63) * (unsigned int)sizeof(R);
        auto entry = [&](int k) -> R {
          constexpr int AUX = CK == CK_PER_CHAIN_NT ? ME_NT_AUX : 0;
          if constexpr (sizeof(R) == 4)
            return __builtin_bit_cast(R, __builtin_amdgcn_raw_buffer_load_b32(tile, lane_off, (unsigned int)k * 64u * 4u, AUX));
          else
            return __builtin_bit_cast(R, __builtin_amdgcn_raw_buffer_load_b64(tile, lane_off, (unsigned int)k * 64u * 8u, AUX));
        };
        R f[2][CH];
#pragma unroll
        for (int u = 0; u < CH; ++u)
          if (u < PF) f[0][u] = entry(u);
        auto use = [&](auto entry_index) -> R {
          constexpr int k = decltype(entry_index)::value;
          if constexpr (k % CH == 0) {
            __builtin_amdgcn_sched_barrier(0);
#pragma unroll
            for (int u = 0; u < CH; ++u)
              if (k + CH + u < PF) f[(k / CH + 1) & 1][u] = entry(k + CH + u);
            __builtin_amdgcn_sched_barrier(0);
          }
          return f[(k / CH) & 1][k % CH];
        };
        static_for<NR>([&](auto row_index) {
          constexpr int i = decltype(row_index)::value;
          R acc = 0;
          static_for<i + 1>([&](auto col_index) {
            constexpr int j = decltype(col_index)::value, k = tri(i, j);
            const R l = use(std::integral_constant<int, k>{});
            acc = j == 0 ? l * g[0] : acc + l * g[j];
          });
          if constexpr (GROUP != GROUP_COMPLEX) xp[i] = x[i] + w_r * acc;
        });
        static_for<NC>([&](auto row_index) {
          constexpr int i = decltype(row_index)::value;
          R are = 0, aim = 0;
          static_for<i>([&](auto col_index) {
            constexpr int j = decltype(col_index)::value;
            const R lre = use(std::integral_constant<int, cre(NR * (NR + 1) / 2, i, j)>{});
            const R lim = use(std::integral_constant<int, cim(NR * (NR + 1) / 2, i, j)>{});
            const R wre = g[NR + j] * R(0.70710678118654752440), wim = g[NR + NC + j] * R(0.70710678118654752440);
            are += lre * wre - lim * wim;
            aim += lre * wim + lim * wre;
          });
          const R ld = use(std::integral_constant<int, cdiag(NR * (NR + 1) / 2, i)>{});
          are += ld * (g[NR + i] * R(0.70710678118654752440));
          aim += ld * (g[NR + NC + i] * R(0.70710678118654752440));
          if constexpr (GROUP != GROUP_REAL) {
            xp[NR + i] = x[NR + i] + w_c * are;
            xp[NR + NC + i] = x[NR + NC + i] + w_c * aim;
          }
        });
        bool rejected = false;
        if (a.reject_kind == ME_REJECT_ABS_REAL0_GE) rejected = !(N_::abs_(xp[0]) < a.reject_bound);
        else if (a.reject_kind == ME_REJECT_USER) rejected = energy_reject(en, xp, 0);
        R terms_new[Ledger::T];
        const R e_new = ledger.propose(en, xp, terms_new);
        const R diff = e_new - (stale_total ? total_q5 : ledger.partial());
        bool accept = diff <= R(0);
        if constexpr (LADDER) accept = accept || uphill_at<true>(a, c, u_accept, diff);
        else if (a.temp > R(0)) accept = accept || N_::uphill(u_accept, diff, a.inv_temp, a.inv_temp_log2e);
        accept = accept && !rejected;
        bad_energy |= (!rejected && !N_::finite(e_new));
#pragma unroll
        for (int d = 0; d < D; ++d) x[d] = accept ? xp[d] : x[d];
        if (stale_total) total_q5 = accept ? e_new : total_q5;
        else ledger.commit(accept, terms_new);
        w = N_::adapt(w, accept, a.ratio, a.p, a.damping, a.up, a.down);
        if constexpr (GROUP == GROUP_ALL) w_r = w_c = w;
        else if constexpr (GROUP == GROUP_REAL) w_r = w;
        else w_c = w;
        wave_accepted += (unsigned int)__popcll(__ballot(accept));
      }
    } else {
      run_sweeps<R, NR, NC, Energy, CK, INJECT, GROUP, LADDER>(a, en, c, gid, stale_total, x, ledger, total_q5, w, w_r, w_c, fac, wave_accepted, bad_energy);
    }
    bad_width |= !(w > R(0));
#pragma unroll
    for (int d = 0; d < D; ++d) fx.store(d, xoff, x[d]);
    if (stale_total) fe.store(Ledger::T, coff, total_q5);
    else ledger.store(fe, coff);
    fw.store(MIXED ? GROUP : 0, coff, w);
  }
  publish_step(a, blockDim.x >> 6, wave_accepted, bad_energy, bad_width);
}

template <typename R, int NR, int NC, class Energy>
__global__ void __launch_bounds__(kStepThreads) k_init_energy(const R *xs, R *energy, long long n, unsigned int *status,
                                                                Energy en, int total_row) {
  constexpr int D = NR + 2 * NC;
  energy_prepare(en, 0);
  const long long stride = (long long)gridDim.x * kStepThreads;
  for (long long c = (long long)blockIdx.x * kStepThreads + threadIdx.x; c < n; c += stride) {
    R x[D];
#pragma unroll
    for (int d = 0; d < D; ++d) x[d] = xs[state_index<R, D>(c, d, n)];
    constexpr int T = term_count<Energy>::value;
    bool finite = true;
    R total = R(0);
#pragma unroll
    for (int t = 0; t < T; ++t) {
      R e;
      if constexpr (T == 1) e = en(x);
      else e = en.term(t, x);
      energy[(long long)t * n + c] = e;
      total = t == 0 ? e : total + e;
      finite = finite && Num<R>::finite(e);
    }
    if (total_row >= 0) energy[(long long)total_row * n + c] = total;
    if (!finite) atomicOr(status, (unsigned int)ST_NONFINITE_ENERGY);
  }
}

}
#include "me_packed_walk.h"
namespace me {

template <typename R>
struct MeasureArgs {
  const R *x, *width;
  R *mean, *cov, *obs_mean, *factor;
  unsigned int *status;
  long long n;
  R keep;
  R inv_i;
  R cov_keep;
  int update_cov, write_factor, split_widths;
};

template <typename R>
MeasureArgs<R> typed_measure(const MeasureLaunch &l) {
  MeasureArgs<R> a;
  a.x = (const R *)l.x;
  a.width = (const R *)l.width;
  a.mean = (R *)l.mean;
  a.cov = (R *)l.cov;
  a.obs_mean = (R *)l.obs_mean;
  a.factor = (R *)l.factor;
  a.status = l.status;
  a.n = l.n;
  const double i = (double)l.measure_count;
  a.keep = (R)((i - 1.0) / i);
  a.inv_i = (R)(1.0 / i);
  a.cov_keep = (R)((i - 2.0) / (i - 1.0));
  a.update_cov = l.update_cov;
  a.split_widths = l.split_widths;
  a.write_factor = l.write_factor;
  return a;
}

template <typename R, int NR, int NC>
__device__ __forceinline__ void cholesky_packed(R (&m)[NR * (NR + 1) / 2 + NC * NC], bool &bad_pivot) {
  constexpr int PR = NR * (NR + 1) / 2;
  using N_ = Num<R>;
#pragma unroll
    for (int j = 0; j < NR; ++j) {
      R s = m[tri(j, j)];
#pragma unroll
      for (int k = 0; k < j; ++k) s = fma_(-m[tri(j, k)], m[tri(j, k)], s);
      if (!(s > R(0))) { bad_pivot = true; s = R(1e-30); }
      const R dg = N_::sqrt_(s);
      const R inv = R(1) / dg;
// ... 69 lines not shown
      if (k0 + u < NOBS) m[u] = packed_load<NTM>(fobs, k0 + u, coff);
#pragma unroll
    for (int u = 0; u < kBatch; ++u) {
      const int k = k0 + u;
      if (k < NOBS) {
        R o;
        if (k < NR) o = N_::abs_(x[k]);
        else if (k < NR + NC) o = N_::sqrt_(fma_(x[k], x[k], x[k + NC] * x[k + NC]));
        else o = x[k - NR - NC] * x[k - NR - NC];
        packed_store<NTM>(fobs, k, coff, fma_(o, a.inv_i, m[u] * a.keep));
      }
    }
  }
  if constexpr (PER_CHAIN_COV) {
    if (a.update_cov) {
      R w_real, w_cplx;
      widths(w_real, w_cplx);
      const R w2_real = w_real * w_real, w2_cplx = w_cplx * w_cplx;
      if constexpr (STREAM) {
        covariance_walk(a.cov + (c >> 6) * (long long)P * 64 + (c & 63), s_delta, NR, NC, (int)threadIdx.x, a.inv_i, a.cov_keep,
                        w2_real, w2_cplx);
      } else {
      R m[P];
#pragma unroll
      for (int k = 0; k < P; ++k) m[k] = packed_load<NT>(fcov, k, toff);
#pragma unroll
      for (int i = 0; i < NR; ++i)
#pragma unroll
        for (int j = 0; j <= i; ++j) {
          const int k = tri(i, j);
          R v = fma_(delta[i] * delta[j], a.inv_i, m[k] * a.cov_keep);
          if (i == j) v = fma_(w2_real, a.inv_i, v);
          packed_store<NT>(fcov, k, toff, v);
          m[k] = v;
        }
#pragma unroll
      for (int i = 0; i < NC; ++i) {
        const R ai = delta[NR + i], bi = delta[NR + NC + i];
#pragma unroll
        for (int j = 0; j < i; ++j) {
          const R aj = delta[NR + j], bj = delta[NR + NC + j];
          const int kr = cre(PR, i, j), ki = cim(PR, i, j);
          const R vr = fma_(fma_(ai, aj, bi * bj), a.inv_i, m[kr] * a.cov_keep);
          const R vi = fma_(fma_(bi, aj, -(ai * bj)), a.inv_i, m[ki] * a.cov_keep);
          packed_store<NT>(fcov, kr, toff, vr);
          packed_store<NT>(fcov, ki, toff, vi);
          m[kr] = vr;
          m[ki] = -vi;
        }
        const int kd = cdiag(PR, i);
        const R vd = fma_(w2_cplx, a.inv_i, fma_(fma_(ai, ai, bi * bi), a.inv_i, m[kd] * a.cov_keep));
        packed_store<NT>(fcov, kd, toff, vd);
        m[kd] = vd;
      }
      if constexpr (FUSED) {
        if (a.write_factor) {
          cholesky_packed<R, NR, NC>(m, bad_pivot);
#pragma unroll
          for (int k = 0; k < P; ++k) packed_store<NT>(ffac, k, toff, m[k]);
        }
      }
      }
    }
  }
}

template <typename R, int NR, int NC, bool PER_CHAIN_COV, bool FUSED, bool NT, bool NTM>
__global__ void __launch_bounds__(kStepThreads, ME_MEASURE_WAVES) k_measure(MeasureArgs<R> a) {
  constexpr int D = NR + 2 * NC;
  constexpr int P = NR * (NR + 1) / 2 + NC * NC;
  constexpr int NOBS = 2 * NR + NC;
  bool bad_pivot = false;
  const long long stride = (long long)gridDim.x * kStepThreads;
  const XField<R, D> fx(a.x, a.n);
  const Field<R> fw(a.width, a.n, (NR > 0 && NC > 0) ? 3 : 1), fmean(a.mean, a.n, D), fobs(a.obs_mean, a.n, NOBS);
  constexpr bool STREAM = PER_CHAIN_COV && P > kMaxPackedInRegisters;
  const TiledField<R> fcov(a.cov, a.n, (PER_CHAIN_COV && !STREAM) ? P : 0);
  const TiledField<R> ffac(a.factor, a.n, (PER_CHAIN_COV && FUSED) ? P : 0);
  __shared__ R s_delta[STREAM ? D : 1][kStepThreads];
  for (long long c = (long long)blockIdx.x * kStepThreads + threadIdx.x; c < a.n; c += stride) {
    const unsigned int coff = (unsigned int)c * (unsigned int)sizeof(R);
    const unsigned int xoff = fx.offset(c);
    R x[D];
#pragma unroll
    for (int d = 0; d < D; ++d) x[d] = fx.load(d, xoff);
    measure_chain<R, NR, NC, PER_CHAIN_COV, FUSED, NT, NTM>(a, c, x, fmean, fobs, fcov, ffac, s_delta, [&](R &w_real, R &w_cplx) {
      constexpr bool MIXED = NR > 0 && NC > 0;
      w_real = fw.load((MIXED && a.split_widths) ? 1 : 0, coff);
      w_cplx = fw.load((MIXED && a.split_widths) ? 2 : 0, coff);
    }, bad_pivot);
  }
  if (bad_pivot) atomicOr(a.status, (unsigned int)ST_BAD_PIVOT);
}

template <typename R, int NR, int NC, class Energy, int CK, bool NT, bool NTM, bool LADDER = false>
__global__ void ME_STEP_BOUNDS k_cycle(StepArgs<R> a, MeasureArgs<R> ma, Energy en) {
  constexpr int D = NR + 2 * NC;
  constexpr int P = NR * (NR + 1) / 2 + NC * NC;
  constexpr int NOBS = 2 * NR + NC;
  constexpr bool MIXED = NR > 0 && NC > 0;
  static_assert(P <= kMaxPackedInRegisters, "k_cycle keeps the packed matrix in registers");
  static_assert(CK == CK_IDENTITY || CK == CK_SHARED || CK == CK_PER_CHAIN, "NT selects the non-temporal factor read");
  constexpr int CKX = CK == CK_PER_CHAIN ? (NT ? CK_PER_CHAIN_NT : CK_PER_CHAIN) : CK;
  using N_ = Num<R>;
  N_::prepare();
  energy_prepare(en, 0);
  unsigned int wave_accepted = 0;
  bool bad_energy = false, bad_width = false, bad_pivot = false;
  const long long stride = (long long)gridDim.x * blockDim.x;
  using Ledger = EnergyLedger<R, Energy, GROUP_ALL>;
  const XField<R, D> fx(a.x, a.n);
  const Field<R> fe(a.energy, a.n, Ledger::T + (MIXED ? 1 : 0)), fw(a.width, a.n, MIXED ? 3 : 1);
  const Field<R> fmean(ma.mean, a.n, D), fobs(ma.obs_mean, a.n, NOBS);
  const TiledField<R> fcov(ma.cov, a.n, P), ffac(ma.factor, a.n, P);
  const bool stale_total = MIXED && a.stale_total != 0;
  for (long long c = (long long)blockIdx.x * blockDim.x + threadIdx.x; c < a.n; c += stride) {
    const unsigned int coff = (unsigned int)c * (unsigned int)sizeof(R);
    const unsigned int xoff = fx.offset(c);
    R x[D];
#pragma unroll
    for (int d = 0; d < D; ++d) x[d] = fx.load(d, xoff);
    Ledger ledger;
    R total_q5 = R(0);
    if (stale_total) total_q5 = fe.load(Ledger::T, coff);
    else ledger.load(fe, coff);
    R w = fw.load(0, coff);
    R w_r = w, w_c = w;
    if constexpr (MIXED) {
      if (a.split_widths) {
        w_r = fw.load(GROUP_REAL, coff);
        w_c = fw.load(GROUP_COMPLEX, coff);
      }
    }
    const unsigned long long gid = a.chain_offset + (unsigned long long)c;
    [[maybe_unused]] const unsigned int toff = tiled_offset<R>(c, P);
    auto fac = [&](int k) -> R {
      if constexpr (CK == CK_PER_CHAIN) return packed_load<NT>(ffac, k, toff);
      else return a.factor[k];
    };
    run_sweeps<R, NR, NC, Energy, CKX, false, GROUP_ALL, LADDER>(a, en, c, gid, stale_total, x, ledger, total_q5, w, w_r, w_c, fac,
                                                         wave_accepted, bad_energy);
    bad_width |= !(w > R(0));
#pragma unroll
    for (int d = 0; d < D; ++d) fx.store(d, xoff, x[d]);
    if (stale_total) fe.store(Ledger::T, coff, total_q5);
    else ledger.store(fe, coff);
    fw.store(0, coff, w);
    measure_chain<R, NR, NC, true, true, NT, NTM>(ma, c, x, fmean, fobs, fcov, ffac, nullptr,
                                                  [&](R &w_real, R &w_cplx) { w_real = w_cplx = w; }, bad_pivot);
  }
  publish_step(a, blockDim.x >> 6, wave_accepted, bad_energy, bad_width, bad_pivot);
}

template <typename R, int NR, bool NT>
__global__ void __launch_bounds__(kStepThreads) k_factor_stream(const R *cov, R *factor, unsigned int *status, long long n) {
  constexpr int P = NR * (NR + 1) / 2;
  constexpr int ROWS = sizeof(R) == 4 ? 4 : 2;
  __shared__ R rows[ROWS * NR][kStepThreads];
  bool bad_pivot = false;
  const long long stride = (long long)gridDim.x * kStepThreads;
  for (long long c = (long long)blockIdx.x * kStepThreads + threadIdx.x; c < n; c += stride) {
    const long long base = (c >> 6) * (long long)P * 64 + (c & 63);
    factor_real_rows<R, ROWS, NT>(cov + base, factor + base, NR, rows, (int)threadIdx.x, bad_pivot);
  }
  if (bad_pivot) atomicOr(status, (unsigned int)ST_BAD_PIVOT);
}

template <typename R, int NR, int NC, bool NT>
__global__ void __launch_bounds__(kStepThreads) k_factor_mixed(const R *cov, R *factor, unsigned int *status, long long n) {
  constexpr int PR = NR * (NR + 1) / 2, P = PR + NC * NC;
  using N_ = Num<R>;
  bool bad_pivot = false;
  const long long stride = (long long)gridDim.x * kStepThreads;
  for (long long c = (long long)blockIdx.x * kStepThreads + threadIdx.x; c < n; c += stride) {
    const long long base = (c >> 6) * (long long)P * 64 + (c & 63);
    const R *cv = cov + base;
    R *fc = factor + base;
    auto in = [&](int k) -> R { return NT ? __builtin_nontemporal_load(cv + (long long)k * 64) : cv[(long long)k * 64]; };
    for (int i = 0; i < NR; ++i)
      for (int j = 0; j <= i; ++j) {
        R s = in(tri(i, j));
        for (int k = 0; k < j; ++k) s = fma_(-fc[(long long)tri(i, k) * 64], fc[(long long)tri(j, k) * 64], s);
        if (j < i) {
          fc[(long long)tri(i, j) * 64] = s / fc[(long long)tri(j, j) * 64];
        } else {
          if (!(s > R(0))) { bad_pivot = true; s = R(1e-30); }
          fc[(long long)tri(i, i) * 64] = N_::sqrt_(s);
        }
      }
    factor_complex_rows<R, NT>(cv, fc, PR, NC, bad_pivot);
  }
  if (bad_pivot) atomicOr(status, (unsigned int)ST_BAD_PIVOT);
}

}
```

### metropolisengine_amd/csrc/me_engine.h

```cpp
#pragma once

#include <string>
#include <utility>
#include <vector>

#include "me_comm.h"
#include "me_internal.h"

#pragma GCC visibility push(hidden)

namespace me {


class DeviceBuffer {
 public:
  DeviceBuffer() = default;
  DeviceBuffer(DeviceBuffer &&o) noexcept : ptr_(std::exchange(o.ptr_, nullptr)), bytes_(std::exchange(o.bytes_, 0)) {}
  DeviceBuffer &operator=(DeviceBuffer &&o) noexcept {
    if (this != &o) {
      reset();
      ptr_ = std::exchange(o.ptr_, nullptr);
      bytes_ = std::exchange(o.bytes_, 0);
    }
    return *this;
// ... 36 lines not shown
  }
  hipError_t allocate(size_t bytes) {
    reset();
    return hipHostMalloc(&ptr_, bytes, hipHostMallocDefault);
  }
  template <typename T>
  T *get() const { return static_cast<T *>(ptr_); }

 private:
  void *ptr_ = nullptr;
};

class Stream {
 public:
  Stream() = default;
  Stream(const Stream &) = delete;
  Stream &operator=(const Stream &) = delete;
  ~Stream() { lend(nullptr); }
  hipError_t create() {
    lend(nullptr);
    const hipError_t err = hipStreamCreateWithFlags(&stream_, hipStreamNonBlocking);
    owned_ = err == hipSuccess;
    return err;
  }
  void lend(hipStream_t theirs) {
    if (owned_ && stream_) (void)hipStreamDestroy(stream_);
    stream_ = theirs;
    owned_ = false;
  }
  operator hipStream_t() const { return stream_; }

 private:
  hipStream_t stream_ = nullptr;
  bool owned_ = false;
};

class Event {
 public:
  Event() = default;
  Event(const Event &) = delete;
  Event &operator=(const Event &) = delete;
  ~Event() { reset(); }
  void reset() {
    if (event_) (void)hipEventDestroy(event_);
    event_ = nullptr;
  }
  hipError_t create(unsigned flags = hipEventDefault) {
    reset();
    return hipEventCreateWithFlags(&event_, flags);
  }
  operator hipEvent_t() const { return event_; }

 private:
  hipEvent_t event_ = nullptr;
};

}

struct me_engine {
  int device = 0;
  me::Stream stream;
  const me::KernelSet *ks = nullptr;
  int dtype = ME_F32;
  size_t esize = 4;
  long long n = 0;
  int nr = 0, nc = 0, d = 0, p = 0, nobs = 0;
  unsigned long long chain_offset = 0, seed = 0;
  double temp = 0, target_acceptance = 0.3, alpha = 0, ratio = 0, reject_bound = 0;
  int m = 0, energy_kind = 0, reject_kind = 0, cov_mode = 0;
  bool stale_total = false;
  me::Event time_start, time_stop;
  std::vector<double> shared_host;
  int cov_kind = me::CK_IDENTITY;
  int grid_blocks = 0;
  int n_terms = 1;
  std::vector<double> coef;
  unsigned long long step_index = 0, measure_count = 1;
  unsigned long long fused_cycles = 0;
  me::DeviceBuffer x, energy, width, mean, cov, obs_mean;
  me::DeviceBuffer factor, shared_factor, shared_full, shared_image, energy_image, coef_dev, row_dev;
  me::DeviceBuffer accept_slots, accept_total;
  long long n_slots = 0;
  unsigned long long proposed = 0;
  bool x_tiled = false;
  int width_rows = 1;
  bool widths_synced = true;
  me::DeviceBuffer status;
  me::PinnedBuffer host_scratch;
  struct Pool {
    me::DeviceBuffer dev, partials;
    me::PinnedBuffer host;
    me::DeviceBuffer range_x;
    me::Stream copy_stream;
    me::Event reduced, copied;
    bool pending = false;
  } pool;
  const me::RcclApi *rccl = nullptr;
  ncclComm_t comm = nullptr;
  int comm_rank = 0, comm_world = 1;
  struct Trace {
    me::DeviceBuffer dev;
    long long chains = 0, stride = 1, rows = 0, capacity = 0;
    void restart() {
      dev.reset();
      rows = capacity = 0;
    }
  } trace;
  struct Ladder {
    int n_rungs = 0;
    std::vector<double> temps;
    me::DeviceBuffer table;
    me::DeviceBuffer pair_counts;
    unsigned long long round = 0;
  } ladder;
  struct Population {
    me::DeviceBuffer fam, fam_out;
    me::DeviceBuffer x, energy;
    me::DeviceBuffer anc;
    me::DeviceBuffer scratch;
    me::DeviceBuffer records;
    unsigned long long stages = 0, capacity = 0;
    std::vector<double> temps;
  } population;
  struct Samples {
    me::DeviceBuffer data;
    long long capacity = 0, rows = 0;
    me::DeviceBuffer obs;
    int n_obs = 0;
    int obs_index[ME_MAX_RECORDED_OBSERVABLES] = {};
  } samples;
  std::string err;

  ~me_engine() {
    (void)hipSetDevice(device);
    if (comm && rccl) (void)rccl->comm_destroy(comm);
  }
};

namespace me {

int fail(me_engine *e, int code, const std::string &msg);

#define ME_HIP(e, call)                                                                                      \
  do {                                                                                                       \
    hipError_t err__ = (call);                                                                               \
    if (err__ != hipSuccess)                                                                                 \
      return me::fail((e), ME_ERR_HIP, std::string(#call) + ": " + hipGetErrorString(err__));                \
  } while (0)

int check_status(me_engine *e);

hipError_t upload(DeviceBuffer &dst, const double *src, size_t count, int dtype);

int refuse_stale_total(me_engine *e, const char *subject);

inline long long padded_chains(long long n) { return (n + 63) / 64 * 64; }

}

#pragma GCC visibility pop
```

### metropolisengine_amd/csrc/me_generic.hip

```cpp
#include "me_internal.h"
#include "me_launch.h"

namespace me {
namespace {

template <typename R>
__global__ void __launch_bounds__(kBlockThreads) k_broadcast_rows(R *dst, const R *row_values, int rows, long long n) {
  const long long stride = (long long)gridDim.x * kBlockThreads;
  for (long long c = (long long)blockIdx.x * kBlockThreads + threadIdx.x; c < n; c += stride)
    for (int r = 0; r < rows; ++r) dst[(long long)r * n + c] = row_values[r];
}

template <typename R>
__global__ void __launch_bounds__(kBlockThreads) k_broadcast_tiled(R *dst, const R *entry_values, int entries, long long n_padded) {
  const long long total = n_padded * entries, stride = (long long)gridDim.x * kBlockThreads;
  for (long long i = (long long)blockIdx.x * kBlockThreads + threadIdx.x; i < total; i += stride)
    dst[i] = entry_values[(i >> 6) % entries];
}

__device__ __forceinline__ void pair_of(int p, int &i, int &j) {
  i = (int)((sqrtf(8.0f * (float)p + 1.0f) - 1.0f) * 0.5f);
  while (i * (i + 1) / 2 > p) --i;
  while ((i + 1) * (i + 2) / 2 <= p) ++i;
  j = p - i * (i + 1) / 2;
}

constexpr int kMaxEntries = 12;

template <typename R, int TILE>
__global__ void __launch_bounds__(kBlockThreads) k_pool_reduce(const R *x, long long n, int nr, int nc, int entry_base, int tiled, double *partials) {
  extern __shared__ __attribute__((aligned(16))) unsigned char smem_raw[];
  R *tile = reinterpret_cast<R *>(smem_raw);
  constexpr int kTilePitch = TILE + 1;
  const int d = nr + 2 * nc;
  const int n_aug = d + nr + nc;
  const int n_pair = d * (d + 1) / 2;
  const int n_entries = 1 + n_aug + n_pair;
  const int tid = threadIdx.x;
  auto at = [&](int r, long long c) -> long long { return tiled ? ((c >> 6) * (long long)d + r) * 64 + (c & 63) : (long long)r * n + c; };

  int row_i[kMaxEntries], row_j[kMaxEntries];
  bool active[kMaxEntries];
  double acc[kMaxEntries];
#pragma unroll
  for (int k = 0; k < kMaxEntries; ++k) {
    const int e = entry_base + tid + k * kBlockThreads;
    acc[k] = 0.0;
    row_i[k] = row_j[k] = -1;
    active[k] = e < n_entries;
    if (!active[k] || e == 0) continue;
    if (e <= n_aug) {
      row_i[k] = e - 1;
    } else {
      pair_of(e - 1 - n_aug, row_i[k], row_j[k]);
    }
  }

  const long long n_tiles = (n + TILE - 1) / TILE;
  for (long long t = blockIdx.x; t < n_tiles; t += gridDim.x) {
    const long long base = t * TILE;
    const int valid = (int)((n - base) < TILE ? (n - base) : TILE);
    for (int r = tid / TILE; r < n_aug; r += kBlockThreads / TILE) {
      const int col = tid % TILE;
      R v = 0;
      if (col < valid) {
        const long long c = base + col;
        if (r < d) v = x[at(r, c)];
        else if (r < d + nr) {
          const R xv = x[at(r - d, c)];
          v = xv < 0 ? -xv : xv;
        } else {
          const int j = r - d - nr;
          const R re = x[at(nr + j, c)], im = x[at(nr + nc + j, c)];
          v = (R)sqrt((double)re * re + (double)im * im);
        }
      }
      tile[r * kTilePitch + col] = v;
    }
    __syncthreads();
#pragma unroll
    for (int k = 0; k < kMaxEntries; ++k) {
      if (!active[k]) continue;
      if (row_i[k] < 0) {
        acc[k] += (double)valid;
      } else if (row_j[k] < 0) {
        const R *ri = tile + row_i[k] * kTilePitch;
        R s = 0;
        for (int col = 0; col < TILE; ++col) s += ri[col];
        acc[k] += (double)s;
      } else {
        const R *ri = tile + row_i[k] * kTilePitch;
        const R *rj = tile + row_j[k] * kTilePitch;
        R s = 0;
        for (int col = 0; col < TILE; ++col) s += ri[col] * rj[col];
        acc[k] += (double)s;
      }
    }
    __syncthreads();
  }
#pragma unroll
  for (int k = 0; k < kMaxEntries; ++k)
    if (active[k]) partials[(long long)blockIdx.x * n_entries + entry_base + tid + k * kBlockThreads] = acc[k];
}

constexpr int kFinishThreads = 1024, kFinishSlices = kFinishThreads / 64;
__global__ void __launch_bounds__(kFinishThreads) k_pool_finish(const double *partials, int n_blocks, int nr, int nc,
                                                                const unsigned long long *slots, long long n_slots,
                                                                double proposed, double *out) {
  const int d = nr + 2 * nc;
  const int n_aug = d + nr + nc;
  const int n_pair = d * (d + 1) / 2;
  const int n_entries = 1 + n_aug + n_pair;
  const int lane = threadIdx.x & 63, slice = threadIdx.x >> 6;
  if (blockIdx.x == gridDim.x - 1) {
    __shared__ unsigned long long wave_sum[kFinishSlices];
    unsigned long long s = 0;
    long long i = threadIdx.x;
    for (; i + 7 * kFinishThreads < n_slots; i += 8 * kFinishThreads) {
      unsigned long long v[8];
#pragma unroll
      for (int u = 0; u < 8; ++u) v[u] = slots[i + u * kFinishThreads];
#pragma unroll
      for (int u = 0; u < 8; ++u) s += v[u];
    }
    for (; i < n_slots; i += kFinishThreads) s += slots[i];
#pragma unroll
    for (int w = 32; w > 0; w >>= 1) s += __shfl_xor(s, w, 64);
    if (lane == 0) wave_sum[slice] = s;
    __syncthreads();
    if (threadIdx.x == 0) {
      unsigned long long t = 0;
#pragma unroll
      for (int w = 0; w < kFinishSlices; ++w) t += wave_sum[w];
      const long long size = moments_size(nr, nc);
      out[size - 2] = (double)t;
      out[size - 1] = proposed;
    }
    return;
  }
  __shared__ double part[kFinishSlices][64];
  const int e = blockIdx.x * 64 + lane;
  double s = 0.0;
  if (e < n_entries) {
#pragma unroll 8
    for (int b = slice; b < n_blocks; b += kFinishSlices) s += partials[(long long)b * n_entries + e];
  }
  part[slice][lane] = s;
  __syncthreads();
  if (slice != 0) return;
  s = 0.0;
#pragma unroll
  for (int w = 0; w < kFinishSlices; ++w) s += part[w][lane];
  if (e == 0) {
    out[0] = s;
  } else if (e <= n_aug) {
    const int r = e - 1;
    out[r < d ? 1 + r : 1 + d + n_pair + (r - d)] = s;
  } else if (e < n_entries) {
    const int p = e - 1 - n_aug;
    int i, j;
    pair_of(p, i, j);
    out[1 + d + p] = s;
    if (i == j && i < nr) out[1 + d + n_pair + nr + nc + i] = s;
  }
}

}

hipError_t launch_broadcast_rows(void *dst, const void *row_values, int rows, long long n, int dtype,
                                 hipStream_t stream) {
  long long blocks = (n + kBlockThreads - 1) / kBlockThreads;
  if (blocks > 4096) blocks = 4096;
  if (blocks < 1) blocks = 1;
  if (dtype == ME_F32)
    hipLaunchKernelGGL(k_broadcast_rows<float>, dim3((unsigned)blocks), dim3(kBlockThreads), 0, stream, (float *)dst,
                       (const float *)row_values, rows, n);
  else
    hipLaunchKernelGGL(k_broadcast_rows<double>, dim3((unsigned)blocks), dim3(kBlockThreads), 0, stream, (double *)dst,
                       (const double *)row_values, rows, n);
  return hipGetLastError();
}

hipError_t launch_broadcast_tiled(void *dst, const void *entry_values, int entries, long long n, int dtype,
                                  hipStream_t stream) {
  const long long n_padded = (n + 63) / 64 * 64;
  long long blocks = (n_padded * entries + kBlockThreads - 1) / kBlockThreads;
  if (blocks > 8192) blocks = 8192;
  if (blocks < 1) blocks = 1;
  if (dtype == ME_F32)
    hipLaunchKernelGGL(k_broadcast_tiled<float>, dim3((unsigned)blocks), dim3(kBlockThreads), 0, stream, (float *)dst,
                       (const float *)entry_values, entries, n_padded);
  else
    hipLaunchKernelGGL(k_broadcast_tiled<double>, dim3((unsigned)blocks), dim3(kBlockThreads), 0, stream, (double *)dst,
                       (const double *)entry_values, entries, n_padded);
  return hipGetLastError();
}

constexpr int kSumThreads = 1024;
__global__ void __launch_bounds__(kSumThreads) k_sum_slots(const unsigned long long *slots, long long n_slots,
                                                           unsigned long long *total) {
  __shared__ unsigned long long part[kSumThreads / 64];
  unsigned long long s = 0;
  long long i = threadIdx.x;
  for (; i + 7 * kSumThreads < n_slots; i += 8 * kSumThreads) {
    unsigned long long v[8];
#pragma unroll
    for (int u = 0; u < 8; ++u) v[u] = slots[i + u * kSumThreads];
#pragma unroll
    for (int u = 0; u < 8; ++u) s += v[u];
  }
  for (; i < n_slots; i += kSumThreads) s += slots[i];
#pragma unroll
  for (int w = 32; w > 0; w >>= 1) s += __shfl_xor(s, w, 64);
  if ((threadIdx.x & 63) == 0) part[threadIdx.x >> 6] = s;
  __syncthreads();
  if (threadIdx.x == 0) {
    unsigned long long t = 0;
#pragma unroll
    for (int w = 0; w < kSumThreads / 64; ++w) t += part[w];
    total[0] = t;
  }
}

template <typename R>
__global__ void __launch_bounds__(kBlockThreads) k_trace(const R *x, const R *energy, const R *width, long long n, int d,
                                                         int n_terms, int width_rows, long long n_traced, long long stride,
                                                         int tiled, double *out) {
  const long long t = (long long)blockIdx.x * kBlockThreads + threadIdx.x;
  if (t >= n_traced) return;
  const long long c = t * stride;
  for (int k = 0; k < d; ++k)
    out[(long long)k * n_traced + t] = (double)x[tiled ? ((c >> 6) * (long long)d + k) * 64 + (c & 63) : (long long)k * n + c];
  for (int k = 0; k < n_terms; ++k) out[(long long)(d + k) * n_traced + t] = (double)energy[(long long)k * n + c];
  for (int r = 0; r < width_rows; ++r)
    out[(long long)(d + n_terms + r) * n_traced + t] = (double)width[(long long)r * n + c];
}

hipError_t launch_trace(const void *x, const void *energy, const void *width, long long n, int d, int n_terms,
                        int width_rows, int dtype, long long n_traced, long long stride, double *out, hipStream_t stream,
                        bool tiled_state) {
  const dim3 grid((unsigned)((n_traced + kBlockThreads - 1) / kBlockThreads)), block(kBlockThreads);
  if (dtype == ME_F32)
    hipLaunchKernelGGL(k_trace<float>, grid, block, 0, stream, (const float *)x, (const float *)energy, (const float *)width,
                       n, d, n_terms, width_rows, n_traced, stride, tiled_state ? 1 : 0, out);
  else
    hipLaunchKernelGGL(k_trace<double>, grid, block, 0, stream, (const double *)x, (const double *)energy,
                       (const double *)width, n, d, n_terms, width_rows, n_traced, stride, tiled_state ? 1 : 0, out);
  return hipGetLastError();
}

hipError_t launch_sum_slots(const unsigned long long *slots, long long n_slots, unsigned long long *total,
                            hipStream_t stream) {
  hipLaunchKernelGGL(k_sum_slots, dim3(1), dim3(kSumThreads), 0, stream, slots, n_slots, total);
  return hipGetLastError();
}

constexpr size_t kPoolLdsLimit = 160 * 1024;
int pool_tile_chains(int nr, int nc, int dtype) {
  const int n_aug = nr + 2 * nc + nr + nc;
  const size_t elem = dtype == ME_F32 ? sizeof(float) : sizeof(double);
  for (int tile : {64, 32, 16})
    if ((size_t)n_aug * (size_t)(tile + 1) * elem <= kPoolLdsLimit) return tile;
  return 0;
}

bool pool_reduce_supported(int nr, int nc, int dtype) { return pool_tile_chains(nr, nc, dtype) != 0; }

int pool_reduce_blocks(long long n, int nr, int nc) {
  const int d = nr + 2 * nc;
  const long long n_entries = 1 + d + nr + nc + (long long)d * (d + 1) / 2;
  long long cap = (32ll << 20) / (8 * n_entries);
  if (cap > 1024) cap = 1024;
  if (cap < 64) cap = 64;
  if (d + nr + nc <= 32) cap = 256;
  const long long tiles = (n + 63) / 64;
  return (int)(tiles < cap ? (tiles < 1 ? 1 : tiles) : cap);
}

namespace {
template <typename R, int TILE>
hipError_t launch_pool_stage1(const void *x, long long n, int nr, int nc, int n_entries, int blocks, double *partials, hipStream_t stream, bool tiled) {
  const size_t lds = (size_t)(nr + 2 * nc + nr + nc) * (size_t)(TILE + 1) * sizeof(R);
  if (lds > 64 * 1024)
    if (hipError_t rc = raise_lds_limit<k_pool_reduce<R, TILE>>(kPoolLdsLimit); rc != hipSuccess) return rc;
  for (int base = 0; base < n_entries; base += kMaxEntries * kBlockThreads)
    hipLaunchKernelGGL((k_pool_reduce<R, TILE>), dim3((unsigned)blocks), dim3(kBlockThreads), lds, stream, (const R *)x, n, nr, nc, base,
                       tiled ? 1 : 0, partials);
  return hipGetLastError();
}
template <typename R>
hipError_t launch_pool_stage1_tile(int tile, const void *x, long long n, int nr, int nc, int n_entries, int blocks, double *partials, hipStream_t stream, bool tiled) {
  switch (tile) {
    case 64: return launch_pool_stage1<R, 64>(x, n, nr, nc, n_entries, blocks, partials, stream, tiled);
    case 32: return launch_pool_stage1<R, 32>(x, n, nr, nc, n_entries, blocks, partials, stream, tiled);
    case 16: return launch_pool_stage1<R, 16>(x, n, nr, nc, n_entries, blocks, partials, stream, tiled);
    default: return hipErrorInvalidValue;
  }
}
}

hipError_t launch_pool_reduce(const void *x, long long n, int nr, int nc, int dtype, const unsigned long long *slots,
                              long long n_slots, double proposed, double *partials, double *out_device,
                              hipStream_t stream,
                              hipError_t (*stage1)(const void *, long long, double *, int, hipStream_t), bool tiled_state) {
  const int d = nr + 2 * nc;
  const int n_aug = d + nr + nc;
  const int n_entries = 1 + n_aug + d * (d + 1) / 2;
  const int tile = pool_tile_chains(nr, nc, dtype);
  if (!stage1 && tile == 0) return hipErrorInvalidValue;
  const int blocks = pool_reduce_blocks(n, nr, nc);
  hipError_t err;
  if (stage1) err = stage1(x, n, partials, blocks, stream);
  else if (dtype == ME_F32) err = launch_pool_stage1_tile<float>(tile, x, n, nr, nc, n_entries, blocks, partials, stream, tiled_state);
  else err = launch_pool_stage1_tile<double>(tile, x, n, nr, nc, n_entries, blocks, partials, stream, tiled_state);
  if (err != hipSuccess) return err;
  hipLaunchKernelGGL(k_pool_finish, dim3((unsigned)((n_entries + 63) / 64 + 1)), dim3(kFinishThreads), 0, stream,
                     (const double *)partials, blocks, nr, nc, slots, n_slots, proposed, out_device);
  return hipGetLastError();
}

}
```

### metropolisengine_amd/csrc/me_internal.h

```cpp
#pragma once

#include <hip/hip_runtime.h>
#include <stdint.h>

#include "../../include/metropolis_engine.h"

namespace me {

enum CovKind { CK_IDENTITY = 0, CK_SHARED = 1, CK_PER_CHAIN = 2, CK_PER_CHAIN_NT = 3 };

enum StepGroup { GROUP_ALL = 0, GROUP_REAL = 1, GROUP_COMPLEX = 2 };

enum StatusBits : uint32_t {
  ST_NONFINITE_ENERGY = 1u,
  ST_BAD_PIVOT = 2u,
  ST_BAD_WIDTH = 4u
};

long long cache_budget_bytes();
void set_cache_budget_bytes(long long bytes);

constexpr int kBlockThreads = 256;
#ifndef ME_STEP_THREADS
#define ME_STEP_THREADS 64
#endif
constexpr int kStepThreads = ME_STEP_THREADS;
constexpr int kFusedStepThreads = 256;
constexpr int kFusedSweepsThreshold = 4;

struct StepLaunch {
  int n_real, n_complex;
  void *x, *energy, *width;
  const void *factor;
  const void *factor_full;
  const void *factor_image;
  const void *energy_image;
  const void *coef_device;
  const double *coef_host;
  int n_coef;
  const void *inj_normals;
  const void *inj_uniforms;
  unsigned long long *accept_slots;
  unsigned int *status;
  long long n;
  unsigned long long chain_offset, step_index, seed;
  int n_sweeps, energy_kind, cov_kind, reject_kind, grid_blocks;
  int group;
  int split_widths;
  int stale_total;
  const void *cov;
  double reject_bound, temp, ratio, target_acceptance, damping;
  const void *ladder;
  int tiles_per_rung;
};

struct MeasureLaunch {
  int n_real, n_complex;
  void *x, *width, *mean, *cov, *obs_mean, *factor;
  unsigned int *status;
  long long n;
  unsigned long long measure_count;
  int update_cov;
  int split_widths;
  int write_factor;
  int grid_blocks;
};

struct EnergyLaunch {
  int n_real, n_complex;
  int total_row;
  void *x, *energy;
  const void *coef_device;
  const double *coef_host;
  int n_coef;
  unsigned int *status;
  long long n;
  int energy_kind, grid_blocks;
};

constexpr int kMaxRegisterDof = 96;

struct KernelSet {
  const char *user_name;
  int dtype, n_real, n_complex;
  bool per_chain_cov;
  bool tracks_cov;
  bool (*has_energy)(int energy_kind);
  int (*energy_terms)(int energy_kind);
  hipError_t (*step)(const StepLaunch &, hipStream_t);
  hipError_t (*magphase)(const StepLaunch &, hipStream_t);
  hipError_t (*measure)(const MeasureLaunch &, hipStream_t);
  hipError_t (*init_energy)(const EnergyLaunch &, hipStream_t);
  size_t matrix_image_bytes;
  hipError_t (*prepare_matrix)(const void *matrix, void *image, hipStream_t);
  hipError_t (*pool_stage1)(const void *x, long long n, double *partials, int n_rows, hipStream_t);
  bool has_user_reject;
  bool streams_packed;
  hipError_t (*cycle)(const StepLaunch &, const MeasureLaunch &, hipStream_t);
  bool tiled_state;
};

void register_kernel_set(const KernelSet *set);
const KernelSet *find_kernel_set(int dtype, int n_real, int n_complex, int energy_kind, const char *user_name);
bool has_dims(int dtype, int n_real, int n_complex);

hipError_t launch_broadcast_rows(void *dst, const void *row_values, int rows, long long n, int dtype,
                                 hipStream_t stream);
hipError_t launch_broadcast_tiled(void *dst, const void *entry_values, int entries, long long n, int dtype,
                                  hipStream_t stream);
hipError_t launch_pool_reduce(const void *x, long long n, int n_real, int n_complex, int dtype,
                              const unsigned long long *slots, long long n_slots, double proposed, double *partials,
                              double *out_device, hipStream_t stream,
                              hipError_t (*stage1)(const void *, long long, double *, int, hipStream_t) = nullptr,
                              bool tiled_state = false);
int pool_reduce_blocks(long long n, int n_real, int n_complex);
bool pool_reduce_supported(int n_real, int n_complex, int dtype);
int pool_tile_chains(int n_real, int n_complex, int dtype);
hipError_t launch_trace(const void *x, const void *energy, const void *width, long long n, int d, int n_terms,
                        int width_rows, int dtype, long long n_traced, long long stride, double *out, hipStream_t stream,
                        bool tiled_state = false);
hipError_t launch_sum_slots(const unsigned long long *slots, long long n_slots, unsigned long long *total,
                            hipStream_t stream);

inline int grid_for(long long n, int requested, int threads = kStepThreads) {
  long long blocks = (n + threads - 1) / threads;
  if (requested > 0 && blocks > requested) blocks = requested;
  if (blocks < 1) blocks = 1;
  return (int)blocks;
}

__host__ __device__ inline int packed_real(int nr) { return nr * (nr + 1) / 2; }
__host__ __device__ inline int packed_total(int nr, int nc) { return nr * (nr + 1) / 2 + nc * nc; }
__host__ __device__ inline int n_observables(int nr, int nc) { return 2 * nr + nc; }
__host__ __device__ inline long long moments_size(int nr, int nc) {
  const int d = nr + 2 * nc;
  return 1 + d + (long long)d * (d + 1) / 2 + n_observables(nr, nc) + 2;
}

}
```

### metropolisengine_amd/csrc/me_kernels.hip

```cpp
#include <type_traits>

#include "me_device.h"
#include "me_dense_mfma.h"
#include "me_dense_bf16x3.h"
#include "me_dense_f64.h"
#include "me_factor_tile.h"
#include "me_per_device.h"
#include "me_pool_gram.h"
#include "me_magphase.h"

#ifdef ME_USER_SOURCE
#include ME_USER_SOURCE
#endif

#ifndef ME_NR
#error "compile with -DME_NR=<n_real> -DME_NC=<n_complex>"
#endif
#ifndef ME_DENSE
#define ME_DENSE 0
#endif
#ifndef ME_PER_CHAIN
#define ME_PER_CHAIN 1
#endif
#ifndef ME_TRACK_COV
// ... 354 lines not shown
  static_assert(ME_PER_CHAIN != 1 || P <= kMaxPackedInRegisters, "ME_PER_CHAIN=1 keeps the packed matrix in registers");
  const dim3 grid(grid_for(l.n, l.grid_blocks)), block(kStepThreads);
  constexpr long long mean_bytes = (long long)sizeof(R) * (2 * D + (2 * NR + NC));
  constexpr long long all_bytes = mean_bytes + (long long)sizeof(R) * 2 * P;
  const bool nt = all_bytes * l.n > cache_budget_bytes(), ntm = mean_bytes * l.n > cache_budget_bytes();
  constexpr bool kCov = (ME_PER_CHAIN != 0 || ME_TRACK_COV != 0);
  if (l.cov) {
    if (ntm) hipLaunchKernelGGL((k_measure<R, NR, NC, kCov, kFused, true, true>), grid, block, 0, stream, a);
    else if (nt) hipLaunchKernelGGL((k_measure<R, NR, NC, kCov, kFused, true, false>), grid, block, 0, stream, a);
    else hipLaunchKernelGGL((k_measure<R, NR, NC, kCov, kFused, false, false>), grid, block, 0, stream, a);
  } else {
    if (ntm) hipLaunchKernelGGL((k_measure<R, NR, NC, false, false, false, true>), grid, block, 0, stream, a);
    else hipLaunchKernelGGL((k_measure<R, NR, NC, false, false, false, false>), grid, block, 0, stream, a);
  }
#if ME_PER_CHAIN == 2
  static_assert(P > kMaxPackedInRegisters, "ME_PER_CHAIN=2 is for spaces with more than 160 packed entries");
  if (l.cov && l.update_cov && l.write_factor) {
    if constexpr (NC > 0) {
      if (nt) hipLaunchKernelGGL((k_factor_mixed<R, NR, NC, true>), grid, block, 0, stream, (const R *)l.cov, (R *)l.factor, l.status, l.n);
      else hipLaunchKernelGGL((k_factor_mixed<R, NR, NC, false>), grid, block, 0, stream, (const R *)l.cov, (R *)l.factor, l.status, l.n);
    } else if constexpr (NR <= 64 && ME_FACTOR_TILE) {
      const hipError_t err = nt ? launch_factor_tile<R, NR, true>((const R *)l.cov, (R *)l.factor, l.status, l.n, stream)
                                : launch_factor_tile<R, NR, false>((const R *)l.cov, (R *)l.factor, l.status, l.n, stream);
      if (err != hipSuccess) return err;
    } else {
      if (nt) hipLaunchKernelGGL((k_factor_stream<R, NR, true>), grid, block, 0, stream, (const R *)l.cov, (R *)l.factor, l.status, l.n);
      else hipLaunchKernelGGL((k_factor_stream<R, NR, false>), grid, block, 0, stream, (const R *)l.cov, (R *)l.factor, l.status, l.n);
    }
  }
#endif
  return hipGetLastError();
}

#ifdef ME_USER_SOURCE
#define ME_SET_NAME ME_USER_NAME
#else
#define ME_SET_NAME nullptr
#endif
constexpr auto pool_stage1_f32() -> hipError_t (*)(const void *, long long, double *, int, hipStream_t) {
  if constexpr (NR == 64 && NC == 0) return launch_pool_gram64;
  else if constexpr (D + NR + NC <= 32) return launch_pool_gram32<NR, NC>;
  else return nullptr;
}
constexpr auto pool_stage1_f64() -> hipError_t (*)(const void *, long long, double *, int, hipStream_t) {
  if constexpr (NR == 64 && NC == 0) return launch_pool_gram64_f64;
  else if constexpr (D + NR + NC <= 32) return launch_pool_gram32_f64<NR, NC>;
  else return nullptr;
}
#if ME_DENSE && !defined(ME_USER_SOURCE)
hipError_t prepare_matrix_f32(const void *factor_full, void *image, hipStream_t stream) {
  if constexpr (NR == 64 && NC == 0) {
    hipLaunchKernelGGL(k_dense64_bf16_fragments<0>, dim3(1), dim3(256), 0, stream, (const float *)factor_full,
                       (unsigned int *)image);
    return hipGetLastError();
  }
  return hipSuccess;
}
[[maybe_unused]] constexpr size_t kMatrixImageBytes = (NR == 64 && NC == 0) ? sizeof(unsigned int) * kBf16FragWords : 0;
#define ME_PREPARE_MATRIX_F32 kMatrixImageBytes, (kMatrixImageBytes ? prepare_matrix_f32 : nullptr), pool_stage1_f32()
hipError_t prepare_matrix_f64(const void *matrix, void *image, hipStream_t stream) {
  if constexpr (NR == 64 && NC == 0) {
    hipLaunchKernelGGL(k_dense64_f64_fragments<0>, dim3(1), dim3(256), 0, stream, (const double *)matrix, (double *)image);
    return hipGetLastError();
  }
  return hipSuccess;
}
[[maybe_unused]] constexpr size_t kMatrixImageBytesF64 = (NR == 64 && NC == 0) ? sizeof(double) * kDense64F64ImageDoubles : 0;
#define ME_PREPARE_MATRIX_F64 kMatrixImageBytesF64, (kMatrixImageBytesF64 ? prepare_matrix_f64 : nullptr), pool_stage1_f64()
#else
#define ME_PREPARE_MATRIX_F32 0, nullptr, pool_stage1_f32()
#define ME_PREPARE_MATRIX_F64 0, nullptr, pool_stage1_f64()
#endif
#ifdef ME_USER_HAS_REJECT
constexpr bool kHasUserReject = true;
#else
constexpr bool kHasUserReject = false;
#endif
#ifndef ME_ONLY_DTYPE
#define ME_ONLY_DTYPE 0
#endif
#if ME_ONLY_DTYPE != 64
const KernelSet kSetF32 = {ME_SET_NAME, ME_F32, NR, NC, ME_PER_CHAIN != 0, (ME_PER_CHAIN != 0 || ME_TRACK_COV != 0), has_energy, energy_terms, step<float>,
                           (NC > 0 && ME_PER_CHAIN == 1) ? magphase<float> : nullptr, measure<float>, init_energy<float>,
                           ME_PREPARE_MATRIX_F32, kHasUserReject, ME_PER_CHAIN == 2, cycle<float>, D >= kTiledStateDof};
#endif
#if ME_ONLY_DTYPE != 32
const KernelSet kSetF64 = {ME_SET_NAME, ME_F64, NR, NC, ME_PER_CHAIN != 0, (ME_PER_CHAIN != 0 || ME_TRACK_COV != 0), has_energy, energy_terms, step<double>,
                           (NC > 0 && ME_PER_CHAIN == 1) ? magphase<double> : nullptr, measure<double>, init_energy<double>,
                           ME_PREPARE_MATRIX_F64, kHasUserReject, ME_PER_CHAIN == 2, cycle<double>, D >= kTiledStateDof};
#endif

struct Registrar {
  Registrar() {
#if ME_ONLY_DTYPE != 64
    register_kernel_set(&kSetF32);
#endif
#if ME_ONLY_DTYPE != 32
    register_kernel_set(&kSetF64);
#endif
  }
} registrar;

}
}
```

### metropolisengine_amd/csrc/me_mbar_obs.hip

```cpp
#include "me_mbar.h"

#pragma clang fp contract(off)

namespace me {
namespace mbar {
namespace {

constexpr int kObsTargets = 4;
constexpr int kObsCols = 4;

struct ObsSelection {
  int q[ME_MAX_RECORDED_OBSERVABLES];
};

template <typename R>
__global__ void __launch_bounds__(kThreads) k_observable_record(const R *__restrict__ x, const R *__restrict__ energy, long long n,
                                                                 int nr, int nc, int n_terms, int tiled, ObsSelection sel,
                                                                 int n_sel, double *dst) {
  const long long c = (long long)blockIdx.x * kThreads + threadIdx.x;
  if (c >= n) return;
  const int d = nr + 2 * nc, nobs = 2 * nr + nc;
  const long long x0 = tiled ? (c >> 6) * (long long)d * 64 + (c & 63) : c;
  const long long xs = tiled ? 64 : n;
  for (int j = 0; j < n_sel; ++j) {
    const int q = sel.q[j];
    double v;
    if (q < d) {
      v = (double)x[x0 + (long long)q * xs];
    } else if (q < d + nobs) {
      const int o = q - d;
      if (o < nr) {
        v = fabs((double)x[x0 + (long long)o * xs]);
      } else if (o < nr + nc) {
        const double re = (double)x[x0 + (long long)o * xs], im = (double)x[x0 + (long long)(o + nc) * xs];
        v = __builtin_sqrt(__builtin_fma(re, re, im * im));
      } else {
        const double xr = (double)x[x0 + (long long)(o - nr - nc) * xs];
        v = xr * xr;
      }
    } else {
      v = (double)energy[(long long)(q - d - nobs) * n + c];
    }
    dst[(long long)j * n + c] = v;
  }
}

struct TargetState {
  double M, W, Q2, mean_e;
  double mean[kObsCols], M2[kObsCols], C[kObsCols];
};
static_assert(sizeof(TargetState) == 16 * sizeof(double), "partials are addressed as 16 doubles per state");

__device__ __forceinline__ void clear(TargetState &s) {
  s.M = -INFINITY;
  s.W = s.Q2 = s.mean_e = 0.0;
#pragma unroll
  for (int q = 0; q < kObsCols; ++q) s.mean[q] = s.M2[q] = s.C[q] = 0.0;
}

__device__ __forceinline__ void add_sample(TargetState &s, double l, double e, const double (&a)[kObsCols], int nq) {
  const bool higher = l > s.M;
  const double x = math64::exp_nonpos(higher ? s.M - l : l - s.M);
  const double scale = higher ? x : 1.0, w = higher ? 1.0 : x;
  const double W = s.W * scale + w;
  const double r = w / W;
  const double mean_e = s.mean_e + (e - s.mean_e) * r;
  const double we = w * (e - mean_e);
#pragma unroll
  for (int q = 0; q < kObsCols; ++q)
    if (q < nq) {
      const double delta = a[q] - s.mean[q];
      const double mean = s.mean[q] + delta * r;
      s.M2[q] = s.M2[q] * scale + (w * delta) * (a[q] - mean);
      s.C[q] = s.C[q] * scale + delta * we;
      s.mean[q] = mean;
    }
  s.Q2 = s.Q2 * (scale * scale) + w * w;
  s.mean_e = mean_e;
  s.W = W;
  s.M = higher ? l : s.M;
}

__device__ __forceinline__ double pick(bool first, double a, double b) { return first ? a : b; }

__device__ __forceinline__ TargetState merge(const TargetState &a, const TargetState &b, int nq) {
  const bool keep_a = !(b.W > 0.0), keep_b = !keep_a && !(a.W > 0.0);
  TargetState r;
  const double M = fmax(a.M, b.M);
  const double sa = math64::exp_nonpos(a.M - M), sb = math64::exp_nonpos(b.M - M);
  const double Wa = a.W * sa, Wb = b.W * sb;
  const double W = Wa + Wb;
  const double fb = Wb / W, cross = Wa * fb;
  const double delta_e = b.mean_e - a.mean_e;
  r.M = pick(keep_a, a.M, pick(keep_b, b.M, M));
  r.W = pick(keep_a, a.W, pick(keep_b, b.W, W));
  r.mean_e = pick(keep_a, a.mean_e, pick(keep_b, b.mean_e, a.mean_e + delta_e * fb));
  r.Q2 = pick(keep_a, a.Q2, pick(keep_b, b.Q2, a.Q2 * (sa * sa) + b.Q2 * (sb * sb)));
#pragma unroll
  for (int q = 0; q < kObsCols; ++q) {
    if (q < nq) {
      const double delta = b.mean[q] - a.mean[q];
      r.mean[q] = pick(keep_a, a.mean[q], pick(keep_b, b.mean[q], a.mean[q] + delta * fb));
      r.M2[q] = pick(keep_a, a.M2[q], pick(keep_b, b.M2[q], (a.M2[q] * sa + b.M2[q] * sb) + (delta * delta) * cross));
      r.C[q] = pick(keep_a, a.C[q], pick(keep_b, b.C[q], (a.C[q] * sa + b.C[q] * sb) + (delta * delta_e) * cross));
    } else {
      r.mean[q] = a.mean[q], r.M2[q] = a.M2[q], r.C[q] = a.C[q];
// ... 123 lines not shown
  if (threadIdx.x != 0) return;
#pragma unroll
  for (int q = 0; q < kObsCols; ++q)
    if (q < nq) {
      mean[(size_t)t * q_total + q] = b.mean[q];
      var[(size_t)t * q_total + q] = b.M2[q] / b.W;
      cov[(size_t)t * q_total + q] = b.C[q] / b.W;
    }
  if (write_neff) neff[t] = (b.W * b.W) / (n_used * b.Q2);
}

hipError_t reweight_observables(Problem &p, const Source &src, const double *f, const double *temps, int n_temps, double *mean,
                                double *var, double *cov, double *neff) {
  ME_MBAR_HIP(prepare(p, src, f));
  if (p.empty_rung >= 0) return hipSuccess;
  Work &w = p.w;
  const size_t cells = (size_t)n_temps * src.columns.n_columns;
  std::vector<double> inv;
  ObsScratch scratch;
  ME_MBAR_HIP(upload_targets(p, temps, n_temps, 3 * cells + (size_t)n_temps, inv));
  ME_MBAR_HIP(reweight_observables_enqueue(p, p.sm, src.columns, w.inv_temps.get<const double>(), n_temps, scratch, w.out.get<double>()));
  std::vector<double> out(3 * cells + (size_t)n_temps);
  ME_MBAR_HIP(hipMemcpyAsync(out.data(), w.out.get(), out.size() * sizeof(double), hipMemcpyDeviceToHost, p.stream));
  ME_MBAR_HIP(hipStreamSynchronize(p.stream));
  if (mean) std::copy(out.begin(), out.begin() + cells, mean);
  if (var) std::copy(out.begin() + cells, out.begin() + 2 * cells, var);
  if (cov) std::copy(out.begin() + 2 * cells, out.begin() + 3 * cells, cov);
  if (neff) std::copy(out.begin() + 3 * cells, out.end(), neff);
  return hipSuccess;
}

int reweight_observables_common(const Source &src, const double *f, const double *temps, int n, double *mean, double *var, double *cov,
                                double *neff) {
  const int rc = check_f_and_targets(src.e, f, src.n_rungs, temps, n, 1);
  if (rc) return rc;
  Problem p;
  return mbar_check_common(src.e, p, reweight_observables(p, src, f, temps, n, mean, var, cov, neff));
}

int catalogue_size(const me_engine *e) { return e->d + e->nobs + e->n_terms; }

}

hipError_t log_denominator_enqueue(Problem &p, const MbarSamples &sm, DeviceBuffer &d) {
  const long long n_padded = tiles_of(sm.n_samples) * kTile;
  ME_MBAR_HIP(d.resize((size_t)n_padded * sizeof(double)));
  hipLaunchKernelGGL(k_mbar_log_denominator, dim3(blocks_of(sm.n_samples)), dim3(kThreads), 0, p.stream, sm.energies, sm.n_samples,
                     n_padded, p.n_rungs, p.w.table.get<const double>(), d.get<double>());
  return hipGetLastError();
}

hipError_t reweight_observables_enqueue(Problem &p, const MbarSamples &sm, const ObsColumns &oc, const double *inv_temps, int n_temps,
                                        ObsScratch &scratch, double *out) {
  hipStream_t stream = p.stream;
  const int n_blocks = blocks_of(sm.n_samples), nq_all = oc.n_columns;
  const long long n_tiles = tiles_of(sm.n_samples);
  const size_t cells = (size_t)n_temps * nq_all;
  ME_MBAR_HIP(log_denominator_enqueue(p, sm, scratch.d));
  ME_MBAR_HIP(scratch.partials.resize((size_t)n_blocks * kObsTargets * sizeof(TargetState)));
  double *o_mean = out, *o_var = o_mean + cells, *o_cov = o_var + cells, *o_neff = o_cov + cells;
  for (int t0 = 0; t0 < n_temps; t0 += kObsTargets) {
    const int nt = std::min(kObsTargets, n_temps - t0);
    for (int q0 = 0; q0 < nq_all; q0 += kObsCols) {
      const int nq = std::min(kObsCols, nq_all - q0);
      const size_t cell = (size_t)t0 * nq_all + q0;
      hipLaunchKernelGGL(k_mbar_reweight_obs, dim3(n_blocks), dim3(kThreads), 0, stream, sm.energies, scratch.d.get<const double>(),
                         oc.data + (size_t)q0 * oc.column_stride, sm.n_samples, oc.n_chains, oc.record_stride, oc.column_stride, nq,
                         inv_temps + t0, nt, n_tiles, scratch.partials.get<TargetState>());
      hipLaunchKernelGGL(k_mbar_reweight_obs_finish, dim3(nt), dim3(kThreads), 0, stream, scratch.partials.get<const TargetState>(),
                         n_blocks, nq, nq_all, p.n_used, q0 == 0 ? 1 : 0, o_mean + cell, o_var + cell, o_cov + cell, o_neff + t0);
    }
  }
  return hipGetLastError();
}

hipError_t observable_record_enqueue(me_engine *e, long long row) {
  me_engine::Samples &s = e->samples;
  ObsSelection sel;
  for (int j = 0; j < ME_MAX_RECORDED_OBSERVABLES; ++j) sel.q[j] = j < s.n_obs ? s.obs_index[j] : 0;
  double *dst = s.obs.get<double>() + (size_t)row * (size_t)s.n_obs * (size_t)e->n;
  const dim3 grid((unsigned)((e->n + kThreads - 1) / kThreads));
  if (e->dtype == ME_F32)
    hipLaunchKernelGGL(k_observable_record<float>, grid, dim3(kThreads), 0, e->stream, e->x.get<const float>(), e->energy.get<const float>(),
                       e->n, e->nr, e->nc, e->n_terms, e->x_tiled ? 1 : 0, sel, s.n_obs, dst);
  else
    hipLaunchKernelGGL(k_observable_record<double>, grid, dim3(kThreads), 0, e->stream, e->x.get<const double>(),
                       e->energy.get<const double>(), e->n, e->nr, e->nc, e->n_terms, e->x_tiled ? 1 : 0, sel, s.n_obs, dst);
  return hipGetLastError();
}

}
}

using namespace me;
using namespace me::mbar;

extern "C" {

int me_observable_samples_enable(me_engine *e, const int32_t *indices, int32_t n_observables) {
  if (!e) return ME_ERR_INVALID;
  const int rc = refuse_stale_total(e, "observable samples are");
  if (rc != ME_OK) return rc;
  if (n_observables < 0 || n_observables > ME_MAX_RECORDED_OBSERVABLES)
    return fail(e, ME_ERR_INVALID, "n_observables must lie in [0, " + std::to_string(ME_MAX_RECORDED_OBSERVABLES) + "]");
  me_engine::Samples &s = e->samples;
  ME_HIP(e, hipSetDevice(e->device));
  if (n_observables == 0) {
    ME_HIP(e, hipStreamSynchronize(e->stream));
    s.obs.reset();
    s.n_obs = 0;
    return ME_OK;
  }
  if (!s.data) return fail(e, ME_ERR_STATE, "observable samples need the energy store: call me_energy_samples_enable first");
  if (!indices) return fail(e, ME_ERR_INVALID, "indices missing");
  for (int j = 0; j < n_observables; ++j)
    if (indices[j] < 0 || indices[j] >= catalogue_size(e))
      return fail(e, ME_ERR_INVALID, "observable index " + std::to_string(indices[j]) + " outside the catalogue of " +
                                         std::to_string(catalogue_size(e)) + " quantities");
  ME_HIP(e, hipStreamSynchronize(e->stream));
  s.obs.reset();
  s.n_obs = 0;
  s.rows = 0;
  const size_t bytes = (size_t)s.capacity * (size_t)n_observables * (size_t)e->n * sizeof(double);
  ME_HIP(e, s.obs.resize(bytes));
  if (bytes) {
    ME_HIP(e, hipMemsetAsync(s.obs.get(), 0, bytes, e->stream));
    ME_HIP(e, hipStreamSynchronize(e->stream));
  }
  s.n_obs = n_observables;
  for (int j = 0; j < n_observables; ++j) s.obs_index[j] = indices[j];
  return ME_OK;
}

int me_observable_samples_info(me_engine *e, int32_t *n_observables, int32_t *indices) {
  if (!e) return ME_ERR_INVALID;
  if (n_observables) *n_observables = e->samples.n_obs;
  if (indices)
    for (int j = 0; j < e->samples.n_obs; ++j) indices[j] = e->samples.obs_index[j];
  return ME_OK;
}

int me_observable_samples_get(me_engine *e, int64_t record_begin, int64_t n_records, double *dst) {
  if (!e || (!dst && n_records > 0)) return ME_ERR_INVALID;
  const me_engine::Samples &s = e->samples;
  if (s.n_obs == 0) return fail(e, ME_ERR_STATE, "observable samples are not enabled: call me_observable_samples_enable first");
  if (record_begin < 0 || n_records < 0 || record_begin + n_records > s.rows)
    return fail(e, ME_ERR_INVALID, "record range outside the recorded samples");
  if (n_records == 0) return ME_OK;
  const size_t row = (size_t)s.n_obs * (size_t)e->n;
  ME_HIP(e, hipSetDevice(e->device));
  ME_HIP(e, hipMemcpyAsync(dst, s.obs.get<double>() + (size_t)record_begin * row, (size_t)n_records * row * sizeof(double),
                           hipMemcpyDeviceToHost, e->stream));
  ME_HIP(e, hipStreamSynchronize(e->stream));
  return ME_OK;
}

int me_observable_samples_set(me_engine *e, int64_t n_records, const double *src) {
  if (!e || (!src && n_records > 0)) return ME_ERR_INVALID;
  const me_engine::Samples &s = e->samples;
  if (s.n_obs == 0) return fail(e, ME_ERR_STATE, "observable samples are not enabled: call me_observable_samples_enable first");
  if (n_records != s.rows)
    return fail(e, ME_ERR_INVALID, "n_records must equal the energy record count (" + std::to_string(s.rows) +
                                       "): call me_energy_samples_set first");
  if (n_records == 0) return ME_OK;
  ME_HIP(e, hipSetDevice(e->device));
  ME_HIP(e, hipMemcpyAsync(s.obs.get(), src, (size_t)n_records * (size_t)s.n_obs * (size_t)e->n * sizeof(double), hipMemcpyHostToDevice,
                           e->stream));
  ME_HIP(e, hipStreamSynchronize(e->stream));
  return ME_OK;
}
// ... 22 lines not shown
```

### metropolisengine_amd/csrc/me_population.hip

```cpp
#include <algorithm>
#include <cmath>
#include <vector>

#include "me_device.h"
#include "me_engine.h"

namespace me {
namespace {

constexpr int kPopThreads = 256;
constexpr int kPopWaves = kPopThreads / 64;
constexpr int kPopItems = 8;
constexpr int kPopChunk = kPopThreads * kPopItems;
constexpr int kFinalThreads = 256;
constexpr long long kSerialSlots = 8;

struct PopParams {
  double M, W, u;
  long long hi;
  long long n_finite;
};

template <typename R>
__device__ __forceinline__ double chain_log_weight(const Field<R> &fe, long long c, long long n, int n_terms, double neg_dbeta,
// ... 174 lines not shown
  const double u = ((double)philox4x32_10(ctr, seed_lo, seed_hi).x + 0.5) * (1.0 / 4294967296.0);
  PopParams p;
  p.u = u;
  p.n_finite = n_finite;
  p.M = M;
  p.W = W;
  const double t = ceil((N * W) / W - u);
  p.hi = t <= 0.0 ? 0 : (t >= N ? n : (long long)t);
  *params = p;
  record[0] = M + log(W / N);
  record[1] = (W * W) / (N * s2);
  record[2] = (double)n_finite;
}

__device__ __forceinline__ long long slot_bound(double c, double N, double W, double u, long long hi) {
  const double t = ceil((N * c) / W - u);
  return t <= 0.0 ? 0 : (t >= (double)hi ? hi : (long long)t);
}

template <typename R>
__global__ void __launch_bounds__(kPopThreads) k_pop_scan_ancestors(const R *energy, long long n, int n_terms, double neg_dbeta,
                                                                   const double *partials, const double *factors,
                                                                   const double *offsets, const PopParams *params,
                                                                   unsigned int *ancestors) {
  __shared__ double wave_tot[kPopWaves], wave_last[kPopWaves];
  const PopParams p = *params;
  const long long base = (long long)blockIdx.x * kPopChunk;
  if (p.n_finite == 0) {
    for (int r = 0; r < kPopItems; ++r) {
      const long long c = base + r * kPopThreads + threadIdx.x;
      if (c < n) ancestors[c] = (unsigned int)c;
    }
    return;
  }
  const Field<R> fe(energy, n, n_terms);
  const double m = partials[4 * (size_t)blockIdx.x], f = factors[blockIdx.x], o = offsets[blockIdx.x];
  const double N = (double)n;
  double l[kPopItems];
  bool ok[kPopItems];
#pragma unroll
  for (int r = 0; r < kPopItems; ++r) l[r] = chain_log_weight(fe, base + r * kPopThreads + threadIdx.x, n, n_terms, neg_dbeta, ok[r]);
  double carry = 0.0, prev;
#pragma unroll
  for (int r = 0; r < kPopItems; ++r) {
    const double v = ok[r] ? exp(l[r] - m) : 0.0;
    const double q = round_running_sum(v, carry, prev, wave_tot, wave_last);
    const long long c = base + r * kPopThreads + threadIdx.x;
    long long lo = 0, up = 0;
    if (q > prev) {
      lo = slot_bound(o + f * prev, N, p.W, p.u, p.hi);
      up = slot_bound(o + f * q, N, p.W, p.u, p.hi);
    }
    const bool long_run = up - lo > kSerialSlots;
    if (!long_run)
      for (long long j = lo; j < up; ++j) ancestors[j] = (unsigned int)c;
    unsigned long long runs = __ballot(long_run);
    while (runs) {
      const int src = __ffsll((long long)runs) - 1;
      runs &= runs - 1;
      const long long run_lo = __shfl(lo, src), run_up = __shfl(up, src);
      const unsigned int run_c = (unsigned int)__shfl(c, src);
      for (long long j = run_lo + (threadIdx.x & 63); j < run_up; j += 64) ancestors[j] = run_c;
    }
  }
}

template <class F>
__device__ __forceinline__ void copy_rows(const F &src, const F &dst, unsigned int src_off, unsigned int dst_off, int rows) {
  constexpr int B = 8;
  for (int r0 = 0; r0 < rows; r0 += B) {
    decltype(src.load(0, 0u)) v[B];
#pragma unroll
    for (int k = 0; k < B; ++k)
      if (r0 + k < rows) v[k] = src.load(r0 + k, src_off);
#pragma unroll
    for (int k = 0; k < B; ++k)
      if (r0 + k < rows) dst.store(r0 + k, dst_off, v[k]);
  }
}

template <typename R>
__global__ void __launch_bounds__(kPopThreads) k_pop_gather(const R *x, const R *energy, const long long *fam, R *x_out,
                                                           R *energy_out, long long *fam_out, long long n, int d, int n_terms,
                                                           int tiled, const unsigned int *ancestors, const PopParams *params) {
  const long long j = (long long)blockIdx.x * kPopThreads + threadIdx.x;
  if (j >= n) return;
  const long long hi = params->hi;
  const long long a = (long long)ancestors[j < hi ? j : hi - 1];
  const unsigned int a_off = (unsigned int)a * (unsigned int)sizeof(R), j_off = (unsigned int)j * (unsigned int)sizeof(R);
  if (tiled) copy_rows(TiledField<R>(x, n, d), TiledField<R>(x_out, n, d), tiled_offset<R>(a, d), tiled_offset<R>(j, d), d);
  else copy_rows(Field<R>(x, n, d), Field<R>(x_out, n, d), a_off, j_off, d);
  copy_rows(Field<R>(energy, n, n_terms), Field<R>(energy_out, n, n_terms), a_off, j_off, n_terms);
  fam_out[j] = fam[a];
}

__global__ void __launch_bounds__(kPopThreads) k_pop_init_families(long long *fam, long long n, unsigned long long chain_offset) {
  const long long j = (long long)blockIdx.x * kPopThreads + threadIdx.x;
  if (j < n) fam[j] = (long long)(chain_offset + (unsigned long long)j);
}

template <typename R>
hipError_t launch(me_engine *e, double neg_dbeta) {
  me_engine::Population &pop = e->population;
  const long long n = e->n;
  hipStream_t stream = e->stream;
  const int n_blocks = (int)((n + kPopChunk - 1) / kPopChunk);
  const unsigned slot_blocks = (unsigned)((n + kPopThreads - 1) / kPopThreads);
  double *partials = pop.scratch.get<double>(), *factors = partials + 4 * (size_t)n_blocks, *offsets = factors + n_blocks;
  PopParams *params = (PopParams *)(offsets + n_blocks + 1);
  double *record = pop.records.get<double>() + 3 * (size_t)pop.stages;
  hipLaunchKernelGGL(k_pop_weights<R>, dim3(n_blocks), dim3(kPopThreads), 0, stream, e->energy.get<const R>(), n, e->n_terms,
                     neg_dbeta, partials);
  hipLaunchKernelGGL(k_pop_finalize, dim3(1), dim3(kFinalThreads), 0, stream, (const double *)partials, n_blocks, n,
                     e->chain_offset, pop.stages, (uint32_t)e->seed, (uint32_t)(e->seed >> 32), factors, offsets, params, record);
  hipLaunchKernelGGL(k_pop_scan_ancestors<R>, dim3(n_blocks), dim3(kPopThreads), 0, stream, e->energy.get<const R>(), n,
                     e->n_terms, neg_dbeta, (const double *)partials, (const double *)factors, (const double *)offsets,
                     (const PopParams *)params, pop.anc.get<unsigned int>());
  hipLaunchKernelGGL(k_pop_gather<R>, dim3(slot_blocks), dim3(kPopThreads), 0, stream, e->x.get<const R>(), e->energy.get<const R>(),
                     pop.fam.get<const long long>(), pop.x.get<R>(), pop.energy.get<R>(), pop.fam_out.get<long long>(), n, e->d,
                     e->n_terms, e->x_tiled ? 1 : 0, pop.anc.get<const unsigned int>(), (const PopParams *)params);
  return hipGetLastError();
}

size_t population_scratch_doubles(long long n) {
  const long long n_blocks = (n + kPopChunk - 1) / kPopChunk;
  return (size_t)(4 * n_blocks + n_blocks + n_blocks + 1) + (sizeof(PopParams) + sizeof(double) - 1) / sizeof(double);
}

int ensure_families(me_engine *e) {
  me_engine::Population &pop = e->population;
  if (pop.fam) return ME_OK;
  ME_HIP(e, pop.fam.resize((size_t)e->n * sizeof(long long)));
  hipLaunchKernelGGL(k_pop_init_families, dim3((unsigned)((e->n + kPopThreads - 1) / kPopThreads)), dim3(kPopThreads), 0, e->stream,
                     pop.fam.get<long long>(), e->n, e->chain_offset);
  ME_HIP(e, hipGetLastError());
  return ME_OK;
}
int ensure_population_scratch(me_engine *e) {
  me_engine::Population &pop = e->population;
  const size_t energy_bytes = (size_t)e->n * (size_t)e->n_terms * e->esize;
  if (pop.energy.bytes() < energy_bytes) {
    if (pop.energy) ME_HIP(e, hipStreamSynchronize(e->stream));
    ME_HIP(e, pop.energy.reserve(energy_bytes));
  }
  if (!pop.x) {
    ME_HIP(e, pop.x.resize(e->x.bytes()));
    ME_HIP(e, hipMemcpyAsync(pop.x.get(), e->x.get(), pop.x.bytes(), hipMemcpyDeviceToDevice, e->stream));
  }
  ME_HIP(e, pop.fam_out.resize((size_t)e->n * sizeof(long long)));
  ME_HIP(e, pop.anc.resize((size_t)e->n * sizeof(unsigned int)));
  ME_HIP(e, pop.scratch.resize(population_scratch_doubles(e->n) * sizeof(double)));
  return ME_OK;
}
int ensure_records(me_engine *e, unsigned long long stages) {
  me_engine::Population &pop = e->population;
  if (stages <= pop.capacity) return ME_OK;
  unsigned long long cap = std::max<unsigned long long>(256, pop.capacity);
  while (cap < stages) cap *= 2;
  DeviceBuffer grown;
  ME_HIP(e, grown.resize((size_t)cap * 3 * sizeof(double)));
  if (pop.records) {
    ME_HIP(e, hipMemcpyAsync(grown.get(), pop.records.get(), (size_t)pop.stages * 3 * sizeof(double), hipMemcpyDeviceToDevice, e->stream));
    ME_HIP(e, hipStreamSynchronize(e->stream));
  }
  pop.records = std::move(grown);
  pop.capacity = cap;
  return ME_OK;
}
int check_family_range(me_engine *e, int64_t chain_begin, int64_t n) {
  if (chain_begin < 0 || n < 0 || chain_begin + n > e->n) return fail(e, ME_ERR_INVALID, "family range outside the engine's chains");
  return ME_OK;
}

}
}

using namespace me;

extern "C" {

int me_set_temperature(me_engine *e, double temp) {
  if (!e) return ME_ERR_INVALID;
  if (!(std::isfinite(temp) && temp >= 0)) return fail(e, ME_ERR_INVALID, "temp must be finite and >= 0");
  if (e->ladder.n_rungs) return fail(e, ME_ERR_STATE, "this engine has a temperature ladder: its rungs carry the temperatures");
  e->temp = temp;
  return ME_OK;
}

int me_population_resample(me_engine *e, double new_temp) {
  if (!e) return ME_ERR_INVALID;
  if (!(std::isfinite(new_temp) && new_temp > 0)) return fail(e, ME_ERR_INVALID, "the new temperature must be finite and > 0");
  int rc = refuse_stale_total(e, "population annealing is");
  if (rc != ME_OK) return rc;
  if (e->ladder.n_rungs) return fail(e, ME_ERR_STATE, "population annealing needs the scalar temp: this engine has a temperature ladder");
  if (!(e->temp > 0)) return fail(e, ME_ERR_STATE, "population annealing cannot reweight from temp = 0: set a temperature first");
  ME_HIP(e, hipSetDevice(e->device));
  if ((rc = ensure_families(e)) || (rc = ensure_population_scratch(e)) || (rc = ensure_records(e, e->population.stages + 1))) return rc;
  me_engine::Population &pop = e->population;
  const double neg_dbeta = -(1.0 / new_temp - 1.0 / e->temp);
  ME_HIP(e, e->dtype == ME_F32 ? launch<float>(e, neg_dbeta) : launch<double>(e, neg_dbeta));
  ME_HIP(e, hipMemcpyAsync(e->x.get(), pop.x.get(), pop.x.bytes(), hipMemcpyDeviceToDevice, e->stream));
  ME_HIP(e, hipMemcpyAsync(e->energy.get(), pop.energy.get(), (size_t)e->n * (size_t)e->n_terms * e->esize, hipMemcpyDeviceToDevice, e->stream));
  ME_HIP(e, hipMemcpyAsync(pop.fam.get(), pop.fam_out.get(), (size_t)e->n * sizeof(long long), hipMemcpyDeviceToDevice, e->stream));
// ... 79 lines not shown
```

### metropolisengine_amd/csrc/me_replica.hip

```cpp
#include <algorithm>
#include <cmath>
#include <string>
#include <vector>

#include "me_device.h"
#include "me_engine.h"

namespace me {
namespace {

constexpr int kSwapThreads = 256;
constexpr int kSwapBlocks = 2048;

template <typename R>
struct SwapArgs {
  R *x, *energy;
  const R *ladder;
  unsigned long long *pair_counts;
  long long n, rung_chains;
  unsigned long long chain_offset, round;
  uint32_t seed_lo, seed_hi;
  int d, n_terms, first_rung, tiled;
};

template <class F>
__device__ __forceinline__ void swap_rows(const F &f, unsigned int off_a, unsigned int off_b, int rows) {
  constexpr int B = 8;
  for (int r0 = 0; r0 < rows; r0 += B) {
    decltype(f.load(0, 0u)) va[B], vb[B];
#pragma unroll
    for (int u = 0; u < B; ++u)
      if (r0 + u < rows) {
        va[u] = f.load(r0 + u, off_a);
        vb[u] = f.load(r0 + u, off_b);
      }
#pragma unroll
    for (int u = 0; u < B; ++u)
      if (r0 + u < rows) {
        f.store(r0 + u, off_a, vb[u]);
        f.store(r0 + u, off_b, va[u]);
      }
  }
}

template <typename R>
__device__ __forceinline__ bool swap_pair(const SwapArgs<R> &s, const Field<R> &fe, int k, long long j, R dbeta, R dbeta_log2e) {
  using N_ = Num<R>;
  const long long a = (long long)k * s.rung_chains + j, b = a + s.rung_chains;
  const unsigned int ea_off = (unsigned int)a * (unsigned int)sizeof(R), eb_off = (unsigned int)b * (unsigned int)sizeof(R);
  const R ea = chain_energy(fe, ea_off, s.n_terms), eb = chain_energy(fe, eb_off, s.n_terms);
  const unsigned long long gid = s.chain_offset + (unsigned long long)a;
  U4 ctr;
  ctr.x = (uint32_t)gid;
  ctr.y = (uint32_t)(gid >> 32);
  ctr.z = (uint32_t)s.round;
  ctr.w = ((uint32_t)(s.round >> 32) << 16) | 0xffffu;
  const R u = N_::unit(philox4x32_10(ctr, s.seed_lo, s.seed_hi).x);
  const R delta = dbeta * (ea - eb);
  const bool accept = N_::finite(ea) && N_::finite(eb) && (delta >= R(0) || N_::uphill(u, eb - ea, dbeta, dbeta_log2e));
  if (accept) {
    if (s.tiled) swap_rows(TiledField<R>(s.x, s.n, s.d), tiled_offset<R>(a, s.d), tiled_offset<R>(b, s.d), s.d);
    else swap_rows(Field<R>(s.x, s.n, s.d), ea_off, eb_off, s.d);
    swap_rows(fe, ea_off, eb_off, s.n_terms);
  }
  return accept;
}

template <typename R>
__global__ void __launch_bounds__(kSwapThreads) k_replica_swap(SwapArgs<R> s) {
  const int k = s.first_rung + 2 * (int)blockIdx.y;
  const Field<R> fe(s.energy, s.n, s.n_terms);
  const R dbeta = s.ladder[2 * k] - s.ladder[2 * k + 2], dbeta_log2e = s.ladder[2 * k + 1] - s.ladder[2 * k + 3];
  unsigned int attempted = 0, accepted = 0;
  for (long long j = (long long)blockIdx.x * kSwapThreads + threadIdx.x; j < s.rung_chains; j += (long long)gridDim.x * kSwapThreads) {
    const bool acc = swap_pair(s, fe, k, j, dbeta, dbeta_log2e);
    attempted += (unsigned int)__popcll(__ballot(true));
    accepted += (unsigned int)__popcll(__ballot(acc));
  }
  __shared__ unsigned int wave_counts[kSwapThreads / 64][2];
  if ((threadIdx.x & 63) == 0) {
    wave_counts[threadIdx.x >> 6][0] = attempted;
    wave_counts[threadIdx.x >> 6][1] = accepted;
  }
  __syncthreads();
  if (threadIdx.x < 2) {
    unsigned long long total = 0;
#pragma unroll
    for (int w = 0; w < kSwapThreads / 64; ++w) total += wave_counts[w][threadIdx.x];
    if (total) atomicAdd(&s.pair_counts[2 * k + threadIdx.x], total);
  }
}

template <typename R>
hipError_t launch(void *x, void *energy, long long n, int d, int n_terms, bool tiled_state, const void *ladder, int n_rungs,
                  unsigned long long round, unsigned long long chain_offset, unsigned long long seed,
                  unsigned long long *pair_counts, hipStream_t stream) {
  SwapArgs<R> s;
  s.x = (R *)x;
  s.energy = (R *)energy;
  s.ladder = (const R *)ladder;
  s.pair_counts = pair_counts;
  s.n = n;
  s.rung_chains = n / n_rungs;
  s.first_rung = (int)(round & 1ull);
  const int n_pairs = (n_rungs - s.first_rung) / 2;
  s.chain_offset = chain_offset;
  s.round = round;
  s.seed_lo = (uint32_t)seed;
  s.seed_hi = (uint32_t)(seed >> 32);
  s.d = d;
  s.n_terms = n_terms;
  s.tiled = tiled_state ? 1 : 0;
  if (n_pairs == 0) return hipSuccess;
  const long long per_pair = std::min<long long>((s.rung_chains + kSwapThreads - 1) / kSwapThreads, std::max(kSwapBlocks / n_pairs, 1));
  hipLaunchKernelGGL(k_replica_swap<R>, dim3((unsigned)per_pair, (unsigned)n_pairs), dim3(kSwapThreads), 0, stream, s);
  return hipGetLastError();
}

int check_ladder_capable(me_engine *e) {
  if (e->ks->n_real < 0)
    return fail(e, ME_ERR_UNSUPPORTED, "temperature ladders are not available on the runtime-dimension kernel set (beyond " +
                                           std::to_string(kMaxRegisterDof) + " real degrees of freedom)");
  if (e->energy_kind == ME_ENERGY_DENSE_QUAD && e->nr == 64 && e->nc == 0)
    return fail(e, ME_ERR_UNSUPPORTED, "temperature ladders are not available on the matrix-core kernels of the dense 64-parameter form");
  return refuse_stale_total(e, "temperature ladders are");
}
int free_ladder(me_engine *e) {
  ME_HIP(e, hipStreamSynchronize(e->stream));
  e->ladder = me_engine::Ladder();
  e->samples.rows = 0;
  return ME_OK;
}
}
}

using namespace me;

extern "C" {

int me_set_temperature_ladder(me_engine *e, const double *temps, int32_t n_rungs) {
  if (!e) return ME_ERR_INVALID;
  if (n_rungs < 0 || (n_rungs > 0 && !temps)) return fail(e, ME_ERR_INVALID, "n_rungs must be >= 0 and temps given");
  ME_HIP(e, hipSetDevice(e->device));
  if (n_rungs == 0) return free_ladder(e);
  int rc = check_ladder_capable(e);
  if (rc != ME_OK) return rc;
  for (int k = 0; k < n_rungs; ++k) {
    if (!(std::isfinite(temps[k]) && temps[k] > 0))
      return fail(e, ME_ERR_INVALID, "ladder temperatures must be finite and > 0");
    if (k > 0 && !(temps[k] > temps[k - 1]))
      return fail(e, ME_ERR_INVALID, "ladder temperatures must be strictly increasing");
  }
  if (e->n % (64ll * n_rungs) != 0)
    return fail(e, ME_ERR_INVALID, "n_chains must be a multiple of 64 * n_rungs: every rung is a run of whole 64-chain tiles");
  std::vector<double> table(2 * (size_t)n_rungs);
  for (int k = 0; k < n_rungs; ++k) {
    table[2 * k] = 1.0 / temps[k];
    table[2 * k + 1] = 1.4426950408889634 / temps[k];
  }
  if ((rc = free_ladder(e)) != ME_OK) return rc;
  ME_HIP(e, upload(e->ladder.table, table.data(), table.size(), e->dtype));
  ME_HIP(e, e->ladder.pair_counts.resize(2 * (size_t)std::max(n_rungs - 1, 1) * sizeof(unsigned long long)));
  ME_HIP(e, hipMemset(e->ladder.pair_counts.get(), 0, e->ladder.pair_counts.bytes()));
  e->ladder.temps.assign(temps, temps + n_rungs);
  e->ladder.n_rungs = n_rungs;
  return ME_OK;
}

int me_temperature_ladder(me_engine *e, double *temps, int32_t capacity, int32_t *n_rungs) {
  if (!e || !n_rungs) return ME_ERR_INVALID;
  *n_rungs = e->ladder.n_rungs;
  if (e->ladder.n_rungs == 0 || !temps) return ME_OK;
  if (capacity < e->ladder.n_rungs) return fail(e, ME_ERR_INVALID, "temps must hold n_rungs doubles");
  std::copy(e->ladder.temps.begin(), e->ladder.temps.end(), temps);
  return ME_OK;
}

int me_replica_exchange(me_engine *e, int32_t n_rounds) {
  if (!e) return ME_ERR_INVALID;
  if (n_rounds < 0) return fail(e, ME_ERR_INVALID, "n_rounds must be >= 0");
  if (e->ladder.n_rungs == 0) return fail(e, ME_ERR_STATE, "no temperature ladder: call me_set_temperature_ladder first");
  ME_HIP(e, hipSetDevice(e->device));
  const auto swap = e->dtype == ME_F32 ? launch<float> : launch<double>;
  for (int i = 0; i < n_rounds; ++i) {
    ME_HIP(e, swap(e->x.get(), e->energy.get(), e->n, e->d, e->n_terms, e->x_tiled, e->ladder.table.get(), e->ladder.n_rungs, e->ladder.round,
                   e->chain_offset, e->seed, e->ladder.pair_counts.get<unsigned long long>(), e->stream));
    e->ladder.round += 1;
  }
  return ME_OK;
}

int me_replica_stats(me_engine *e, uint64_t *round, uint64_t *attempted, uint64_t *accepted, int32_t n_pairs) {
  if (!e) return ME_ERR_INVALID;
  if (e->ladder.n_rungs == 0) return fail(e, ME_ERR_STATE, "no temperature ladder");
  if (n_pairs != e->ladder.n_rungs - 1) return fail(e, ME_ERR_INVALID, "n_pairs must be n_rungs - 1");
  if (round) *round = e->ladder.round;
  if (n_pairs == 0) return ME_OK;
  ME_HIP(e, hipSetDevice(e->device));
  std::vector<unsigned long long> counts(2 * (size_t)n_pairs);
  ME_HIP(e, hipMemcpyAsync(counts.data(), e->ladder.pair_counts.get(), counts.size() * sizeof(unsigned long long), hipMemcpyDeviceToHost,
                           e->stream));
  ME_HIP(e, hipStreamSynchronize(e->stream));
  for (int k = 0; k < n_pairs; ++k) {
    if (attempted) attempted[k] = counts[2 * k];
    if (accepted) accepted[k] = counts[2 * k + 1];
  }
  return ME_OK;
}

int me_set_replica_stats(me_engine *e, uint64_t round, const uint64_t *attempted, const uint64_t *accepted, int32_t n_pairs) {
  if (!e) return ME_ERR_INVALID;
  if (e->ladder.n_rungs == 0) return fail(e, ME_ERR_STATE, "no temperature ladder");
  if (n_pairs != e->ladder.n_rungs - 1) return fail(e, ME_ERR_INVALID, "n_pairs must be n_rungs - 1");
  if (n_pairs > 0 && (!attempted || !accepted)) return fail(e, ME_ERR_INVALID, "attempted / accepted missing");
  std::vector<unsigned long long> counts(2 * (size_t)n_pairs);
  for (int k = 0; k < n_pairs; ++k) {
    if (accepted[k] > attempted[k]) return fail(e, ME_ERR_INVALID, "accepted swaps exceed attempted ones");
    counts[2 * k] = attempted[k];
    counts[2 * k + 1] = accepted[k];
  }
  ME_HIP(e, hipSetDevice(e->device));
  if (n_pairs > 0) {
    ME_HIP(e, hipMemcpyAsync(e->ladder.pair_counts.get(), counts.data(), counts.size() * sizeof(unsigned long long), hipMemcpyHostToDevice,
                             e->stream));
    ME_HIP(e, hipStreamSynchronize(e->stream));
  }
  e->ladder.round = round;
  return ME_OK;
}

}
```

Measured before the change: 19.29 billion.

## Store 16-dim f64 real chain state as contiguous per-chain lines with 128-bit I/O

Adds a new state layout (STATE_TILE_LINES) for pure-real f64 sets whose state is exactly 128 bytes per chain, storing each chain's parameters contiguously instead of component-interleaved tiles. The sweep kernel loads and stores the whole state with 128-bit buffer ops, and writes back only when some step was accepted (a dirty flag). The aim is fewer memory instructions and skipped stores for chains that never moved. In exchange, lanes access strided 128-byte lines rather than coalesced rows, and every auxiliary path (broadcast, host copies, trace, pooling, population, replica swap, observables) now dispatches on a layout enum.

```diff
diff --git a/metropolisengine_amd/csrc/me_api.hip b/metropolisengine_amd/csrc/me_api.hip
--- a/metropolisengine_amd/csrc/me_api.hip
+++ b/metropolisengine_amd/csrc/me_api.hip
@@ -168,11 +168,12 @@
 
 namespace {
 
-int broadcast(me_engine *e, DeviceBuffer &dst, const std::vector<double> &row, bool tiled = false) {
+int broadcast(me_engine *e, DeviceBuffer &dst, const std::vector<double> &row, int layout = STATE_COMPONENT_MAJOR) {
   std::vector<unsigned char> bytes;
   to_device_type(row.data(), row.size(), e->dtype, bytes);
   ME_HIP(e, hipMemcpyAsync(e->row_dev.get(), bytes.data(), bytes.size(), hipMemcpyHostToDevice, e->stream));
-  if (tiled) ME_HIP(e, launch_broadcast_tiled(dst.get(), e->row_dev.get(), (int)row.size(), e->n, e->dtype, e->stream));
+  if (layout != STATE_COMPONENT_MAJOR)
+    ME_HIP(e, launch_broadcast_tiled(dst.get(), e->row_dev.get(), (int)row.size(), e->n, e->dtype, e->stream, layout == STATE_TILE_LINES));
   else ME_HIP(e, launch_broadcast_rows(dst.get(), e->row_dev.get(), (int)row.size(), e->n, e->dtype, e->stream));
   ME_HIP(e, hipStreamSynchronize(e->stream));
   return ME_OK;
@@ -189,9 +190,8 @@
     for (int64_t c = 0; c < n_chains; ++c) t[(size_t)r * n_chains + c] = (T)src[c * comps + r];
 }
 template <typename T>
-void transpose_tiled(T *t, int entries, int64_t tile0, int64_t chain_begin, int64_t n_chains, double *dst, const double *src) {
-  const size_t tile_values = (size_t)entries * 64;
-  auto at = [&](int64_t c, int k) { return (size_t)((c >> 6) - tile0) * tile_values + (size_t)k * 64 + (size_t)(c & 63); };
+void transpose_tiled(T *t, int entries, int64_t tile0, int64_t chain_begin, int64_t n_chains, double *dst, const double *src, int layout) {
+  auto at = [&](int64_t c, int k) { return (size_t)state_value_index(layout, c - tile0 * 64, k, entries, 0); };
   for (int64_t i = 0; i < n_chains; ++i)
     for (int k = 0; k < entries; ++k) {
       if (dst) dst[i * entries + k] = (double)t[at(chain_begin + i, k)];
@@ -199,7 +199,8 @@
     }
 }
 
-int copy_tiled(me_engine *e, void *field_ptr, int entries, int64_t chain_begin, int64_t n_chains, double *dst, const double *src) {
+int copy_tiled(me_engine *e, void *field_ptr, int entries, int64_t chain_begin, int64_t n_chains, double *dst, const double *src,
+               int layout = STATE_TILE_ROWS) {
   const int64_t tile0 = chain_begin >> 6, tile1 = (chain_begin + n_chains - 1) >> 6;
   const size_t tile_values = (size_t)entries * 64, n_values = (size_t)(tile1 - tile0 + 1) * tile_values;
   unsigned char *dev = (unsigned char *)field_ptr + (size_t)tile0 * tile_values * e->esize;
@@ -209,8 +210,8 @@
     ME_HIP(e, hipMemcpyAsync(tmp.data(), dev, tmp.size(), hipMemcpyDeviceToHost, e->stream));
     ME_HIP(e, hipStreamSynchronize(e->stream));
   }
-  if (e->dtype == ME_F32) transpose_tiled(reinterpret_cast<float *>(tmp.data()), entries, tile0, chain_begin, n_chains, dst, src);
-  else transpose_tiled(reinterpret_cast<double *>(tmp.data()), entries, tile0, chain_begin, n_chains, dst, src);
+  if (e->dtype == ME_F32) transpose_tiled(reinterpret_cast<float *>(tmp.data()), entries, tile0, chain_begin, n_chains, dst, src, layout);
+  else transpose_tiled(reinterpret_cast<double *>(tmp.data()), entries, tile0, chain_begin, n_chains, dst, src, layout);
   if (src) {
     ME_HIP(e, hipMemcpyAsync(dev, tmp.data(), tmp.size(), hipMemcpyHostToDevice, e->stream));
     ME_HIP(e, hipStreamSynchronize(e->stream));
@@ -407,7 +408,7 @@
 struct Layout {
   bool keep_per_chain;
   bool keep_cov;
-  bool x_tiled;
+  int x_layout;
   int width_rows;
 };
 int decide_layout(const me_config *c, const KernelSet *ks, Layout &l) {
@@ -426,7 +427,7 @@
                 "a per-chain field would exceed 4 GiB on this engine; shard the chains over more engines");
   l.keep_cov = l.keep_per_chain ||
                ((!ks->per_chain_cov || ks->streams_packed) && ks->tracks_cov && (c->flags & ME_FLAG_TRACK_COVARIANCE));
-  l.x_tiled = ks->tiled_state;
+  l.x_layout = ks->state_layout;
   l.width_rows = (c->n_real > 0 && c->n_complex > 0) ? 3 : 1;
   return ME_OK;
 }
@@ -458,7 +459,7 @@
   e->ratio = (1.0 - 1.0 / e->m) * std::sqrt(2.0 * M_PI) * std::exp(e->alpha * e->alpha / 2.0) / 2.0 * e->alpha +
              1.0 / (e->m * c->target_acceptance * (1.0 - c->target_acceptance));
   if (const char *g = std::getenv("ME_GRID_BLOCKS")) e->grid_blocks = std::atoi(g);
-  e->x_tiled = l.x_tiled;
+  e->x_layout = l.x_layout;
   e->stale_total = (c->flags & ME_FLAG_REFERENCE_ENERGY_LEDGERS) != 0;
   e->width_rows = l.width_rows;
   e->n_slots = (e->n + 31) / 32 + 8;
@@ -470,7 +471,7 @@
   ME_HIP(e, hipSetDevice(e->device));
   ME_HIP(e, e->stream.create());
   const size_t n = (size_t)e->n, tiles = (size_t)padded_chains(e->n), es = e->esize;
-  ME_HIP(e, e->x.resize((e->x_tiled ? tiles : n) * e->d * es));
+  ME_HIP(e, e->x.resize((e->x_layout != STATE_COMPONENT_MAJOR ? tiles : n) * e->d * es));
   ME_HIP(e, e->energy.resize(n * (e->n_terms + (e->stale_total ? 1 : 0)) * es));
   ME_HIP(e, e->width.resize(n * e->width_rows * es));
   ME_HIP(e, e->mean.resize(n * e->d * es));
@@ -560,9 +561,9 @@
     return fail(e, ME_ERR_INVALID, "initial covariance matrix is not positive definite (metropolis_engine.py:270)");
   int rc = ME_OK;
   std::vector<double> width_row((size_t)e->width_rows, c->sampling_width);
-  if ((rc = broadcast(e, e->x, init, e->x_tiled)) || (rc = broadcast(e, e->mean, init)) || (rc = broadcast(e, e->obs_mean, obs)) ||
-      (rc = broadcast(e, e->width, width_row)) || (e->cov && (rc = broadcast(e, e->cov, c0, true))) ||
-      (e->factor && (rc = broadcast(e, e->factor, f0, true))) || (rc = upload_shared_factor(e, f0.data())))
+  if ((rc = broadcast(e, e->x, init, e->x_layout)) || (rc = broadcast(e, e->mean, init)) || (rc = broadcast(e, e->obs_mean, obs)) ||
+      (rc = broadcast(e, e->width, width_row)) || (e->cov && (rc = broadcast(e, e->cov, c0, STATE_TILE_ROWS))) ||
+      (e->factor && (rc = broadcast(e, e->factor, f0, STATE_TILE_ROWS))) || (rc = upload_shared_factor(e, f0.data())))
     return rc;
   e->cov_kind = identity ? CK_IDENTITY : (e->ks->n_real < 0 && e->factor) ? CK_PER_CHAIN : CK_SHARED;
   return ME_OK;
@@ -618,7 +619,7 @@
     return fail(e, ME_ERR_UNSUPPORTED, is_user_kind(energy_kind)
                     ? std::string("no user-energy plugin named '") + (user_name ? user_name : "") + "' is loaded for these dimensions"
                     : "energy kind " + std::to_string(energy_kind) + " is not compiled for these dimensions");
-  if (ks->tiled_state != e->ks->tiled_state || ks->per_chain_cov != e->ks->per_chain_cov || ks->streams_packed != e->ks->streams_packed ||
+  if (ks->state_layout != e->ks->state_layout || ks->per_chain_cov != e->ks->per_chain_cov || ks->streams_packed != e->ks->streams_packed ||
       ks->tracks_cov != e->ks->tracks_cov)
     return fail(e, ME_ERR_UNSUPPORTED, "me_set_energy: the plugin was built with other per-chain covariance options than this engine's kernel set");
   if (e->reject_kind == ME_REJECT_USER && !ks->has_user_reject)
@@ -813,7 +814,7 @@
     const int rows_valid = (e->width_rows == 3 && e->widths_synced) ? 1 : e->width_rows;
     double *row = e->trace.dev.get<double>() + e->trace.rows * cols * e->trace.chains;
     ME_HIP(e, launch_trace(e->x.get(), e->energy.get(), e->width.get(), e->n, e->d, e->n_terms, rows_valid, e->dtype, e->trace.chains,
-                           e->trace.stride, row, e->stream, e->x_tiled));
+                           e->trace.stride, row, e->stream, e->x_layout));
     if (rows_valid != e->width_rows) {
       double *widths = row + (size_t)(e->d + e->n_terms) * e->trace.chains;
       for (int r = 1; r < 3; ++r)
@@ -919,8 +920,9 @@
   int rc = field_info(e, field, &ptr, &comps);
   if (rc != ME_OK) return rc;
   if (n_chains == 0) return ME_OK;
-  if (field == ME_FIELD_COV || field == ME_FIELD_FACTOR || (field == ME_FIELD_PARAMS && e->x_tiled))
-    return copy_tiled(e, ptr, comps, chain_begin, n_chains, dst, nullptr);
+  if (field == ME_FIELD_PARAMS && e->x_layout != STATE_COMPONENT_MAJOR)
+    return copy_tiled(e, ptr, comps, chain_begin, n_chains, dst, nullptr, e->x_layout);
+  if (field == ME_FIELD_COV || field == ME_FIELD_FACTOR) return copy_tiled(e, ptr, comps, chain_begin, n_chains, dst, nullptr);
   std::vector<unsigned char> tmp((size_t)comps * n_chains * e->esize);
   for (int r = 0; r < comps; ++r)
     ME_HIP(e, hipMemcpyAsync(tmp.data() + (size_t)r * n_chains * e->esize,
@@ -945,8 +947,8 @@
   if (field == ME_FIELD_WIDTH && e->width_rows == 3 && (chain_begin != 0 || n_chains != e->n))
     return fail(e, ME_ERR_INVALID, "widths of a mixed engine must be set for all chains at once");
   if (n_chains == 0) return ME_OK;
-  if (field == ME_FIELD_COV || field == ME_FIELD_FACTOR || (field == ME_FIELD_PARAMS && e->x_tiled)) {
-    rc = copy_tiled(e, ptr, comps, chain_begin, n_chains, nullptr, src);
+  if (field == ME_FIELD_COV || field == ME_FIELD_FACTOR || (field == ME_FIELD_PARAMS && e->x_layout != STATE_COMPONENT_MAJOR)) {
+    rc = copy_tiled(e, ptr, comps, chain_begin, n_chains, nullptr, src, field == ME_FIELD_PARAMS ? e->x_layout : STATE_TILE_ROWS);
     if (rc != ME_OK) return rc;
     if (field == ME_FIELD_FACTOR) e->cov_kind = CK_PER_CHAIN;
     return ME_OK;
@@ -1054,7 +1056,7 @@
 }
 int enqueue_pool_reduce(me_engine *e, const void *x, long long n_chains, long long n_slots, double proposed, double *device_out) {
   hipError_t err = launch_pool_reduce(x, n_chains, e->nr, e->nc, e->dtype, e->accept_slots.get<unsigned long long>(), n_slots, proposed,
-                                      e->pool.partials.get<double>(), device_out, e->stream, e->ks->pool_stage1, e->x_tiled);
+                                      e->pool.partials.get<double>(), device_out, e->stream, e->ks->pool_stage1, e->x_layout);
   if (err == hipErrorInvalidValue) return fail(e, ME_ERR_UNSUPPORTED, "pooled moments: dimension too large for the reduction kernel");
   ME_HIP(e, err);
   return ME_OK;
@@ -1093,7 +1095,7 @@
   int rc = check_pooled(e, n_doubles);
   if (rc != ME_OK) return rc;
   const unsigned char *x = e->x.get<unsigned char>();
-  if (e->x_tiled) {
+  if (e->x_layout != STATE_COMPONENT_MAJOR) {
     x += (size_t)chain_begin * e->d * e->esize;
   } else {
     const size_t row = (size_t)n_chains * e->esize;
diff --git a/metropolisengine_amd/csrc/me_device.h b/metropolisengine_amd/csrc/me_device.h
--- a/metropolisengine_amd/csrc/me_device.h
+++ b/metropolisengine_amd/csrc/me_device.h
@@ -235,28 +235,99 @@
 #define ME_TILED_STATE_DOF 16
 #endif
 constexpr int kTiledStateDof = ME_TILED_STATE_DOF;
+#if defined(ME_NR) && defined(ME_NC)
+constexpr bool kPureRealSet = ME_NC == 0;
+#else
+constexpr bool kPureRealSet = false;
+#endif
+template <typename R, int D>
+constexpr int state_layout() {
+  if (D < kTiledStateDof) return STATE_COMPONENT_MAJOR;
+  return (kPureRealSet && sizeof(R) == 8 && D * sizeof(R) == 128) ? STATE_TILE_LINES : STATE_TILE_ROWS;
+}
+template <typename R>
+__device__ __forceinline__ unsigned int line_offset(long long c, int rows) {
+  return (unsigned int)(c * (long long)rows * (long long)sizeof(R));
+}
+template <typename R>
+struct LineField : TiledField<R> {
+  using TiledField<R>::TiledField;
+  template <int AUX>
+  __device__ __forceinline__ R load_aux(int row, unsigned int line_off) const {
+    if constexpr (sizeof(R) == 4) {
+      return __builtin_bit_cast(R, __builtin_amdgcn_raw_buffer_load_b32(this->rsrc, line_off, (unsigned int)row * 4u, AUX));
+    } else {
+      const auto v = __builtin_amdgcn_raw_buffer_load_b64(this->rsrc, line_off, (unsigned int)row * 8u, AUX);
+      return __builtin_bit_cast(R, v);
+    }
+  }
+  template <int AUX>
+  __device__ __forceinline__ void store_aux(int row, unsigned int line_off, R value) const {
+    if constexpr (sizeof(R) == 4) {
+      __builtin_amdgcn_raw_buffer_store_b32(__builtin_bit_cast(unsigned int, value), this->rsrc, line_off, (unsigned int)row * 4u, AUX);
+    } else {
+      using v2 = decltype(__builtin_amdgcn_raw_buffer_load_b64(this->rsrc, 0u, 0u, 0));
+      __builtin_amdgcn_raw_buffer_store_b64(__builtin_bit_cast(v2, value), this->rsrc, line_off, (unsigned int)row * 8u, AUX);
+    }
+  }
+  __device__ __forceinline__ R load(int row, unsigned int line_off) const { return load_aux<0>(row, line_off); }
+  __device__ __forceinline__ void store(int row, unsigned int line_off, R value) const { store_aux<0>(row, line_off, value); }
+};
 template <typename R, int D, bool NTS = false>
 struct XField {
-  static constexpr bool kTiled = D >= kTiledStateDof;
-  std::conditional_t<kTiled, TiledField<R>, StateField<R, NTS>> f;
+  static constexpr int kLayout = state_layout<R, D>();
+  static constexpr bool kTiled = kLayout != STATE_COMPONENT_MAJOR;
+  static constexpr bool kLines = kLayout == STATE_TILE_LINES;
+  static constexpr int kAux = 0;
+  std::conditional_t<kLines, LineField<R>, std::conditional_t<kTiled, TiledField<R>, StateField<R, NTS>>> f;
   __device__ __forceinline__ XField(const R *base, long long n) : f(base, n, D) {}
   static __device__ __forceinline__ unsigned int offset(long long c) {
-    if constexpr (kTiled) return tiled_offset<R>(c, D);
+    if constexpr (kLines) return line_offset<R>(c, D);
+    else if constexpr (kTiled) return tiled_offset<R>(c, D);
     else return (unsigned int)c * (unsigned int)sizeof(R);
   }
   __device__ __forceinline__ R load(int row, unsigned int off) const {
-    if constexpr (kTiled && NTS) return f.load_nt(row, off);
+    if constexpr (kLines) return f.template load_aux<kAux>(row, off);
+    else if constexpr (kTiled && NTS) return f.load_nt(row, off);
     else return f.load(row, off);
   }
   __device__ __forceinline__ void store(int row, unsigned int off, R value) const {
-    if constexpr (kTiled && NTS) f.store_nt(row, off, value);
+    if constexpr (kLines) f.template store_aux<kAux>(row, off, value);
+    else if constexpr (kTiled && NTS) f.store_nt(row, off, value);
     else f.store(row, off, value);
+  }
+  __device__ __forceinline__ void load_state(unsigned int off, R (&x)[D]) const {
+    if constexpr (kLines) {
+      struct Pair { R a, b; };
+#pragma unroll
+      for (int j = 0; j < D / 2; ++j) {
+        const Pair p = __builtin_bit_cast(Pair, __builtin_amdgcn_raw_buffer_load_b128(f.rsrc, off, (unsigned int)j * 16u, kAux));
+        x[2 * j] = p.a;
+        x[2 * j + 1] = p.b;
+      }
+    } else {
+#pragma unroll
+      for (int d = 0; d < D; ++d) x[d] = load(d, off);
+    }
+  }
+  __device__ __forceinline__ void store_state(unsigned int off, const R (&x)[D], [[maybe_unused]] bool dirty) const {
+    if constexpr (kLines) {
+      struct Pair { R a, b; };
+      using v4 = decltype(__builtin_amdgcn_raw_buffer_load_b128(f.rsrc, 0u, 0u, 0));
+      if (dirty) {
+#pragma unroll
+        for (int j = 0; j < D / 2; ++j)
+          __builtin_amdgcn_raw_buffer_store_b128(__builtin_bit_cast(v4, Pair{x[2 * j], x[2 * j + 1]}), f.rsrc, off, (unsigned int)j * 16u, kAux);
+      }
+    } else {
+#pragma unroll
+      for (int d = 0; d < D; ++d) store(d, off, x[d]);
+    }
   }
 };
 template <typename R, int D>
 __device__ __forceinline__ long long state_index(long long c, int row, long long n) {
-  if constexpr (D >= kTiledStateDof) return ((c >> 6) * (long long)D + row) * 64 + (c & 63);
-  else return (long long)row * n + c;
+  return state_value_index(state_layout<R, D>(), c, row, D, n);
 }
 
 constexpr int kMaxPackedInRegisters = 160;
@@ -660,7 +731,7 @@
 __device__ __forceinline__ void decide_step(const StepArgs<R> &a, long long c, const Energy &en, bool stale_total, R u,
                                             const R (&g)[2 * ((NR + 2 * NC + 1) / 2)], R (&x)[NR + 2 * NC], const R (&xp)[NR + 2 * NC],
                                             Ledger &ledger, R &total_q5, R &w, R &w_r, R &w_c, unsigned int &wave_accepted,
-                                            bool &bad_energy) {
+                                            bool &bad_energy, bool &dirty) {
   [[maybe_unused]] constexpr int D = NR + 2 * NC;
   constexpr bool MOVE_REAL = NR > 0 && GROUP != GROUP_COMPLEX;
   constexpr bool MOVE_COMPLEX = NC > 0 && GROUP != GROUP_REAL;
@@ -700,19 +771,20 @@
   else if constexpr (GROUP == GROUP_REAL) w_r = w;
   else w_c = w;
   wave_accepted += (unsigned int)__popcll(__ballot(accept));
+  dirty |= accept;
 }
 
 template <typename R, int NR, int NC, class Energy, int CK, bool INJECT, int GROUP, bool LADDER, class Ledger, class Fac>
 __device__ __forceinline__ void run_sweeps(const StepArgs<R> &a, const Energy &en, long long c, unsigned long long gid,
                                            bool stale_total, R (&x)[NR + 2 * NC], Ledger &ledger, R &total_q5, R &w, R &w_r,
-                                           R &w_c, Fac &&fac, unsigned int &wave_accepted, bool &bad_energy) {
+                                           R &w_c, Fac &&fac, unsigned int &wave_accepted, bool &bad_energy, bool &dirty) {
   constexpr int D = NR + 2 * NC;
   constexpr int NW = 2 * ((D + 1) / 2);
   for (int s = 0; s < a.n_sweeps; ++s) {
     R g[NW], u, xp[D];
     draw_step<R, NR, NC, INJECT>(a, c, gid, s, g, u);
     propose_registers<R, NR, NC, CK, GROUP>(x, g, w_r, w_c, fac, xp);
-    decide_step<R, NR, NC, Energy, CK, GROUP, LADDER>(a, c, en, stale_total, u, g, x, xp, ledger, total_q5, w, w_r, w_c, wave_accepted, bad_energy);
+    decide_step<R, NR, NC, Energy, CK, GROUP, LADDER>(a, c, en, stale_total, u, g, x, xp, ledger, total_q5, w, w_r, w_c, wave_accepted, bad_energy, dirty);
   }
 }
 
@@ -766,8 +838,8 @@
     const unsigned int coff = (unsigned int)c * (unsigned int)sizeof(R);
     const unsigned int xoff = fx.offset(c);
     R x[D];
-#pragma unroll
-    for (int d = 0; d < D; ++d) x[d] = fx.load(d, xoff);
+    fx.load_state(xoff, x);
+    bool dirty = false;
     Ledger ledger;
     R total_q5 = R(0);
     if (stale_total) total_q5 = fe.load(Ledger::T, coff);
@@ -893,13 +965,13 @@
         else if constexpr (GROUP == GROUP_REAL) w_r = w;
         else w_c = w;
         wave_accepted += (unsigned int)__popcll(__ballot(accept));
+        dirty |= accept;
       }
     } else {
-      run_sweeps<R, NR, NC, Energy, CK, INJECT, GROUP, LADDER>(a, en, c, gid, stale_total, x, ledger, total_q5, w, w_r, w_c, fac, wave_accepted, bad_energy);
+      run_sweeps<R, NR, NC, Energy, CK, INJECT, GROUP, LADDER>(a, en, c, gid, stale_total, x, ledger, total_q5, w, w_r, w_c, fac, wave_accepted, bad_energy, dirty);
     }
     bad_width |= !(w > R(0));
-#pragma unroll
-    for (int d = 0; d < D; ++d) fx.store(d, xoff, x[d]);
+    fx.store_state(xoff, x, dirty);
     if (stale_total) fe.store(Ledger::T, coff, total_q5);
     else ledger.store(fe, coff);
     fw.store(MIXED ? GROUP : 0, coff, w);
@@ -1135,8 +1207,7 @@
     const unsigned int coff = (unsigned int)c * (unsigned int)sizeof(R);
     const unsigned int xoff = fx.offset(c);
     R x[D];
-#pragma unroll
-    for (int d = 0; d < D; ++d) x[d] = fx.load(d, xoff);
+    fx.load_state(xoff, x);
     measure_chain<R, NR, NC, PER_CHAIN_COV, FUSED, NT, NTM>(a, c, x, fmean, fobs, fcov, ffac, s_delta, [&](R &w_real, R &w_cplx) {
       constexpr bool MIXED = NR > 0 && NC > 0;
       w_real = fw.load((MIXED && a.split_widths) ? 1 : 0, coff);
@@ -1171,8 +1242,8 @@
     const unsigned int coff = (unsigned int)c * (unsigned int)sizeof(R);
     const unsigned int xoff = fx.offset(c);
     R x[D];
-#pragma unroll
-    for (int d = 0; d < D; ++d) x[d] = fx.load(d, xoff);
+    fx.load_state(xoff, x);
+    bool dirty = false;
     Ledger ledger;
     R total_q5 = R(0);
     if (stale_total) total_q5 = fe.load(Ledger::T, coff);
@@ -1192,10 +1263,9 @@
       else return a.factor[k];
     };
     run_sweeps<R, NR, NC, Energy, CKX, false, GROUP_ALL, LADDER>(a, en, c, gid, stale_total, x, ledger, total_q5, w, w_r, w_c, fac,
-                                                         wave_accepted, bad_energy);
+                                                         wave_accepted, bad_energy, dirty);
     bad_width |= !(w > R(0));
-#pragma unroll
-    for (int d = 0; d < D; ++d) fx.store(d, xoff, x[d]);
+    fx.store_state(xoff, x, dirty);
     if (stale_total) fe.store(Ledger::T, coff, total_q5);
     else ledger.store(fe, coff);
     fw.store(0, coff, w);
diff --git a/metropolisengine_amd/csrc/me_engine.h b/metropolisengine_amd/csrc/me_engine.h
--- a/metropolisengine_amd/csrc/me_engine.h
+++ b/metropolisengine_amd/csrc/me_engine.h
@@ -142,7 +142,7 @@
   me::DeviceBuffer accept_slots, accept_total;
   long long n_slots = 0;
   unsigned long long proposed = 0;
-  bool x_tiled = false;
+  int x_layout = me::STATE_COMPONENT_MAJOR;
   int width_rows = 1;
   bool widths_synced = true;
   me::DeviceBuffer status;
diff --git a/metropolisengine_amd/csrc/me_generic.hip b/metropolisengine_amd/csrc/me_generic.hip
--- a/metropolisengine_amd/csrc/me_generic.hip
+++ b/metropolisengine_amd/csrc/me_generic.hip
@@ -12,10 +12,10 @@
 }
 
 template <typename R>
-__global__ void __launch_bounds__(kBlockThreads) k_broadcast_tiled(R *dst, const R *entry_values, int entries, long long n_padded) {
+__global__ void __launch_bounds__(kBlockThreads) k_broadcast_tiled(R *dst, const R *entry_values, int entries, long long n_padded, int lines) {
   const long long total = n_padded * entries, stride = (long long)gridDim.x * kBlockThreads;
   for (long long i = (long long)blockIdx.x * kBlockThreads + threadIdx.x; i < total; i += stride)
-    dst[i] = entry_values[(i >> 6) % entries];
+    dst[i] = entry_values[(lines ? i : (i >> 6)) % entries];
 }
 
 __device__ __forceinline__ void pair_of(int p, int &i, int &j) {
@@ -28,7 +28,7 @@
 constexpr int kMaxEntries = 12;
 
 template <typename R, int TILE>
-__global__ void __launch_bounds__(kBlockThreads) k_pool_reduce(const R *x, long long n, int nr, int nc, int entry_base, int tiled, double *partials) {
+__global__ void __launch_bounds__(kBlockThreads) k_pool_reduce(const R *x, long long n, int nr, int nc, int entry_base, int layout, double *partials) {
   extern __shared__ __attribute__((aligned(16))) unsigned char smem_raw[];
   R *tile = reinterpret_cast<R *>(smem_raw);
   constexpr int kTilePitch = TILE + 1;
@@ -37,7 +37,7 @@
   const int n_pair = d * (d + 1) / 2;
   const int n_entries = 1 + n_aug + n_pair;
   const int tid = threadIdx.x;
-  auto at = [&](int r, long long c) -> long long { return tiled ? ((c >> 6) * (long long)d + r) * 64 + (c & 63) : (long long)r * n + c; };
+  auto at = [&](int r, long long c) -> long long { return state_value_index(layout, c, r, d, n); };
 
   int row_i[kMaxEntries], row_j[kMaxEntries];
   bool active[kMaxEntries];
@@ -182,17 +182,17 @@
 }
 
 hipError_t launch_broadcast_tiled(void *dst, const void *entry_values, int entries, long long n, int dtype,
-                                  hipStream_t stream) {
+                                  hipStream_t stream, bool lines) {
   const long long n_padded = (n + 63) / 64 * 64;
   long long blocks = (n_padded * entries + kBlockThreads - 1) / kBlockThreads;
   if (blocks > 8192) blocks = 8192;
   if (blocks < 1) blocks = 1;
   if (dtype == ME_F32)
     hipLaunchKernelGGL(k_broadcast_tiled<float>, dim3((unsigned)blocks), dim3(kBlockThreads), 0, stream, (float *)dst,
-                       (const float *)entry_values, entries, n_padded);
+                       (const float *)entry_values, entries, n_padded, lines ? 1 : 0);
   else
     hipLaunchKernelGGL(k_broadcast_tiled<double>, dim3((unsigned)blocks), dim3(kBlockThreads), 0, stream, (double *)dst,
-                       (const double *)entry_values, entries, n_padded);
+                       (const double *)entry_values, entries, n_padded, lines ? 1 : 0);
   return hipGetLastError();
 }
 
@@ -225,12 +225,12 @@
 template <typename R>
 __global__ void __launch_bounds__(kBlockThreads) k_trace(const R *x, const R *energy, const R *width, long long n, int d,
                                                          int n_terms, int width_rows, long long n_traced, long long stride,
-                                                         int tiled, double *out) {
+                                                         int layout, double *out) {
   const long long t = (long long)blockIdx.x * kBlockThreads + threadIdx.x;
   if (t >= n_traced) return;
   const long long c = t * stride;
   for (int k = 0; k < d; ++k)
-    out[(long long)k * n_traced + t] = (double)x[tiled ? ((c >> 6) * (long long)d + k) * 64 + (c & 63) : (long long)k * n + c];
+    out[(long long)k * n_traced + t] = (double)x[state_value_index(layout, c, k, d, n)];
   for (int k = 0; k < n_terms; ++k) out[(long long)(d + k) * n_traced + t] = (double)energy[(long long)k * n + c];
   for (int r = 0; r < width_rows; ++r)
     out[(long long)(d + n_terms + r) * n_traced + t] = (double)width[(long long)r * n + c];
@@ -238,14 +238,14 @@
 
 hipError_t launch_trace(const void *x, const void *energy, const void *width, long long n, int d, int n_terms,
                         int width_rows, int dtype, long long n_traced, long long stride, double *out, hipStream_t stream,
-                        bool tiled_state) {
+                        int state_layout) {
   const dim3 grid((unsigned)((n_traced + kBlockThreads - 1) / kBlockThreads)), block(kBlockThreads);
   if (dtype == ME_F32)
     hipLaunchKernelGGL(k_trace<float>, grid, block, 0, stream, (const float *)x, (const float *)energy, (const float *)width,
-                       n, d, n_terms, width_rows, n_traced, stride, tiled_state ? 1 : 0, out);
+                       n, d, n_terms, width_rows, n_traced, stride, state_layout, out);
   else
     hipLaunchKernelGGL(k_trace<double>, grid, block, 0, stream, (const double *)x, (const double *)energy,
-                       (const double *)width, n, d, n_terms, width_rows, n_traced, stride, tiled_state ? 1 : 0, out);
+                       (const double *)width, n, d, n_terms, width_rows, n_traced, stride, state_layout, out);
   return hipGetLastError();
 }
 
@@ -279,21 +279,21 @@
 
 namespace {
 template <typename R, int TILE>
-hipError_t launch_pool_stage1(const void *x, long long n, int nr, int nc, int n_entries, int blocks, double *partials, hipStream_t stream, bool tiled) {
+hipError_t launch_pool_stage1(const void *x, long long n, int nr, int nc, int n_entries, int blocks, double *partials, hipStream_t stream, int layout) {
   const size_t lds = (size_t)(nr + 2 * nc + nr + nc) * (size_t)(TILE + 1) * sizeof(R);
   if (lds > 64 * 1024)
     if (hipError_t rc = raise_lds_limit<k_pool_reduce<R, TILE>>(kPoolLdsLimit); rc != hipSuccess) return rc;
   for (int base = 0; base < n_entries; base += kMaxEntries * kBlockThreads)
     hipLaunchKernelGGL((k_pool_reduce<R, TILE>), dim3((unsigned)blocks), dim3(kBlockThreads), lds, stream, (const R *)x, n, nr, nc, base,
-                       tiled ? 1 : 0, partials);
+                       layout, partials);
   return hipGetLastError();
 }
 template <typename R>
-hipError_t launch_pool_stage1_tile(int tile, const void *x, long long n, int nr, int nc, int n_entries, int blocks, double *partials, hipStream_t stream, bool tiled) {
+hipError_t launch_pool_stage1_tile(int tile, const void *x, long long n, int nr, int nc, int n_entries, int blocks, double *partials, hipStream_t stream, int layout) {
   switch (tile) {
-    case 64: return launch_pool_stage1<R, 64>(x, n, nr, nc, n_entries, blocks, partials, stream, tiled);
-    case 32: return launch_pool_stage1<R, 32>(x, n, nr, nc, n_entries, blocks, partials, stream, tiled);
-    case 16: return launch_pool_stage1<R, 16>(x, n, nr, nc, n_entries, blocks, partials, stream, tiled);
+    case 64: return launch_pool_stage1<R, 64>(x, n, nr, nc, n_entries, blocks, partials, stream, layout);
+    case 32: return launch_pool_stage1<R, 32>(x, n, nr, nc, n_entries, blocks, partials, stream, layout);
+    case 16: return launch_pool_stage1<R, 16>(x, n, nr, nc, n_entries, blocks, partials, stream, layout);
     default: return hipErrorInvalidValue;
   }
 }
@@ -302,7 +302,7 @@
 hipError_t launch_pool_reduce(const void *x, long long n, int nr, int nc, int dtype, const unsigned long long *slots,
                               long long n_slots, double proposed, double *partials, double *out_device,
                               hipStream_t stream,
-                              hipError_t (*stage1)(const void *, long long, double *, int, hipStream_t), bool tiled_state) {
+                              hipError_t (*stage1)(const void *, long long, double *, int, hipStream_t), int state_layout) {
   const int d = nr + 2 * nc;
   const int n_aug = d + nr + nc;
   const int n_entries = 1 + n_aug + d * (d + 1) / 2;
@@ -311,8 +311,8 @@
   const int blocks = pool_reduce_blocks(n, nr, nc);
   hipError_t err;
   if (stage1) err = stage1(x, n, partials, blocks, stream);
-  else if (dtype == ME_F32) err = launch_pool_stage1_tile<float>(tile, x, n, nr, nc, n_entries, blocks, partials, stream, tiled_state);
-  else err = launch_pool_stage1_tile<double>(tile, x, n, nr, nc, n_entries, blocks, partials, stream, tiled_state);
+  else if (dtype == ME_F32) err = launch_pool_stage1_tile<float>(tile, x, n, nr, nc, n_entries, blocks, partials, stream, state_layout);
+  else err = launch_pool_stage1_tile<double>(tile, x, n, nr, nc, n_entries, blocks, partials, stream, state_layout);
   if (err != hipSuccess) return err;
   hipLaunchKernelGGL(k_pool_finish, dim3((unsigned)((n_entries + 63) / 64 + 1)), dim3(kFinishThreads), 0, stream,
                      (const double *)partials, blocks, nr, nc, slots, n_slots, proposed, out_device);
diff --git a/metropolisengine_amd/csrc/me_internal.h b/metropolisengine_amd/csrc/me_internal.h
--- a/metropolisengine_amd/csrc/me_internal.h
+++ b/metropolisengine_amd/csrc/me_internal.h
@@ -80,6 +80,13 @@
 
 constexpr int kMaxRegisterDof = 96;
 
+enum StateLayout : int { STATE_COMPONENT_MAJOR = 0, STATE_TILE_ROWS = 1, STATE_TILE_LINES = 2 };
+__host__ __device__ inline long long state_value_index(int layout, long long c, int row, int d, long long n) {
+  if (layout == STATE_TILE_ROWS) return ((c >> 6) * (long long)d + row) * 64 + (c & 63);
+  if (layout == STATE_TILE_LINES) return c * (long long)d + row;
+  return (long long)row * n + c;
+}
+
 struct KernelSet {
   const char *user_name;
   int dtype, n_real, n_complex;
@@ -97,7 +104,7 @@
   bool has_user_reject;
   bool streams_packed;
   hipError_t (*cycle)(const StepLaunch &, const MeasureLaunch &, hipStream_t);
-  bool tiled_state;
+  int state_layout;
 };
 
 void register_kernel_set(const KernelSet *set);
@@ -107,18 +114,18 @@
 hipError_t launch_broadcast_rows(void *dst, const void *row_values, int rows, long long n, int dtype,
                                  hipStream_t stream);
 hipError_t launch_broadcast_tiled(void *dst, const void *entry_values, int entries, long long n, int dtype,
-                                  hipStream_t stream);
+                                  hipStream_t stream, bool lines = false);
 hipError_t launch_pool_reduce(const void *x, long long n, int n_real, int n_complex, int dtype,
                               const unsigned long long *slots, long long n_slots, double proposed, double *partials,
                               double *out_device, hipStream_t stream,
                               hipError_t (*stage1)(const void *, long long, double *, int, hipStream_t) = nullptr,
-                              bool tiled_state = false);
+                              int state_layout = STATE_COMPONENT_MAJOR);
 int pool_reduce_blocks(long long n, int n_real, int n_complex);
 bool pool_reduce_supported(int n_real, int n_complex, int dtype);
 int pool_tile_chains(int n_real, int n_complex, int dtype);
 hipError_t launch_trace(const void *x, const void *energy, const void *width, long long n, int d, int n_terms,
                         int width_rows, int dtype, long long n_traced, long long stride, double *out, hipStream_t stream,
-                        bool tiled_state = false);
+                        int state_layout = STATE_COMPONENT_MAJOR);
 hipError_t launch_sum_slots(const unsigned long long *slots, long long n_slots, unsigned long long *total,
                             hipStream_t stream);
 
diff --git a/metropolisengine_amd/csrc/me_kernels.hip b/metropolisengine_amd/csrc/me_kernels.hip
--- a/metropolisengine_amd/csrc/me_kernels.hip
+++ b/metropolisengine_amd/csrc/me_kernels.hip
@@ -460,12 +460,12 @@
 #if ME_ONLY_DTYPE != 64
 const KernelSet kSetF32 = {ME_SET_NAME, ME_F32, NR, NC, ME_PER_CHAIN != 0, (ME_PER_CHAIN != 0 || ME_TRACK_COV != 0), has_energy, energy_terms, step<float>,
                            (NC > 0 && ME_PER_CHAIN == 1) ? magphase<float> : nullptr, measure<float>, init_energy<float>,
-                           ME_PREPARE_MATRIX_F32, kHasUserReject, ME_PER_CHAIN == 2, cycle<float>, D >= kTiledStateDof};
+                           ME_PREPARE_MATRIX_F32, kHasUserReject, ME_PER_CHAIN == 2, cycle<float>, state_layout<float, D>()};
 #endif
 #if ME_ONLY_DTYPE != 32
 const KernelSet kSetF64 = {ME_SET_NAME, ME_F64, NR, NC, ME_PER_CHAIN != 0, (ME_PER_CHAIN != 0 || ME_TRACK_COV != 0), has_energy, energy_terms, step<double>,
                            (NC > 0 && ME_PER_CHAIN == 1) ? magphase<double> : nullptr, measure<double>, init_energy<double>,
-                           ME_PREPARE_MATRIX_F64, kHasUserReject, ME_PER_CHAIN == 2, cycle<double>, D >= kTiledStateDof};
+                           ME_PREPARE_MATRIX_F64, kHasUserReject, ME_PER_CHAIN == 2, cycle<double>, state_layout<double, D>()};
 #endif
 
 struct Registrar {
diff --git a/metropolisengine_amd/csrc/me_mbar_obs.hip b/metropolisengine_amd/csrc/me_mbar_obs.hip
--- a/metropolisengine_amd/csrc/me_mbar_obs.hip
+++ b/metropolisengine_amd/csrc/me_mbar_obs.hip
@@ -15,13 +15,13 @@
 
 template <typename R>
 __global__ void __launch_bounds__(kThreads) k_observable_record(const R *__restrict__ x, const R *__restrict__ energy, long long n,
-                                                                 int nr, int nc, int n_terms, int tiled, ObsSelection sel,
+                                                                 int nr, int nc, int n_terms, int layout, ObsSelection sel,
                                                                  int n_sel, double *dst) {
   const long long c = (long long)blockIdx.x * kThreads + threadIdx.x;
   if (c >= n) return;
   const int d = nr + 2 * nc, nobs = 2 * nr + nc;
-  const long long x0 = tiled ? (c >> 6) * (long long)d * 64 + (c & 63) : c;
-  const long long xs = tiled ? 64 : n;
+  const long long x0 = state_value_index(layout, c, 0, d, n);
+  const long long xs = state_value_index(layout, c, 1, d, n) - x0;
   for (int j = 0; j < n_sel; ++j) {
     const int q = sel.q[j];
     double v;
@@ -311,10 +311,10 @@
   const dim3 grid((unsigned)((e->n + kThreads - 1) / kThreads));
   if (e->dtype == ME_F32)
     hipLaunchKernelGGL(k_observable_record<float>, grid, dim3(kThreads), 0, e->stream, e->x.get<const float>(), e->energy.get<const float>(),
-                       e->n, e->nr, e->nc, e->n_terms, e->x_tiled ? 1 : 0, sel, s.n_obs, dst);
+                       e->n, e->nr, e->nc, e->n_terms, e->x_layout, sel, s.n_obs, dst);
   else
     hipLaunchKernelGGL(k_observable_record<double>, grid, dim3(kThreads), 0, e->stream, e->x.get<const double>(),
-                       e->energy.get<const double>(), e->n, e->nr, e->nc, e->n_terms, e->x_tiled ? 1 : 0, sel, s.n_obs, dst);
+                       e->energy.get<const double>(), e->n, e->nr, e->nc, e->n_terms, e->x_layout, sel, s.n_obs, dst);
   return hipGetLastError();
 }
 
diff --git a/metropolisengine_amd/csrc/me_population.hip b/metropolisengine_amd/csrc/me_population.hip
--- a/metropolisengine_amd/csrc/me_population.hip
+++ b/metropolisengine_amd/csrc/me_population.hip
@@ -280,13 +280,14 @@
 template <typename R>
 __global__ void __launch_bounds__(kPopThreads) k_pop_gather(const R *x, const R *energy, const long long *fam, R *x_out,
                                                            R *energy_out, long long *fam_out, long long n, int d, int n_terms,
-                                                           int tiled, const unsigned int *ancestors, const PopParams *params) {
+                                                           int layout, const unsigned int *ancestors, const PopParams *params) {
   const long long j = (long long)blockIdx.x * kPopThreads + threadIdx.x;
   if (j >= n) return;
   const long long hi = params->hi;
   const long long a = (long long)ancestors[j < hi ? j : hi - 1];
   const unsigned int a_off = (unsigned int)a * (unsigned int)sizeof(R), j_off = (unsigned int)j * (unsigned int)sizeof(R);
-  if (tiled) copy_rows(TiledField<R>(x, n, d), TiledField<R>(x_out, n, d), tiled_offset<R>(a, d), tiled_offset<R>(j, d), d);
+  if (layout == STATE_TILE_ROWS) copy_rows(TiledField<R>(x, n, d), TiledField<R>(x_out, n, d), tiled_offset<R>(a, d), tiled_offset<R>(j, d), d);
+  else if (layout == STATE_TILE_LINES) copy_rows(LineField<R>(x, n, d), LineField<R>(x_out, n, d), line_offset<R>(a, d), line_offset<R>(j, d), d);
   else copy_rows(Field<R>(x, n, d), Field<R>(x_out, n, d), a_off, j_off, d);
   copy_rows(Field<R>(energy, n, n_terms), Field<R>(energy_out, n, n_terms), a_off, j_off, n_terms);
   fam_out[j] = fam[a];
@@ -316,7 +317,7 @@
                      (const PopParams *)params, pop.anc.get<unsigned int>());
   hipLaunchKernelGGL(k_pop_gather<R>, dim3(slot_blocks), dim3(kPopThreads), 0, stream, e->x.get<const R>(), e->energy.get<const R>(),
                      pop.fam.get<const long long>(), pop.x.get<R>(), pop.energy.get<R>(), pop.fam_out.get<long long>(), n, e->d,
-                     e->n_terms, e->x_tiled ? 1 : 0, pop.anc.get<const unsigned int>(), (const PopParams *)params);
+                     e->n_terms, e->x_layout, pop.anc.get<const unsigned int>(), (const PopParams *)params);
   return hipGetLastError();
 }
 
diff --git a/metropolisengine_amd/csrc/me_replica.hip b/metropolisengine_amd/csrc/me_replica.hip
--- a/metropolisengine_amd/csrc/me_replica.hip
+++ b/metropolisengine_amd/csrc/me_replica.hip
@@ -20,7 +20,7 @@
   long long n, rung_chains;
   unsigned long long chain_offset, round;
   uint32_t seed_lo, seed_hi;
-  int d, n_terms, first_rung, tiled;
+  int d, n_terms, first_rung, layout;
 };
 
 template <class F>
@@ -59,7 +59,8 @@
   const R delta = dbeta * (ea - eb);
   const bool accept = N_::finite(ea) && N_::finite(eb) && (delta >= R(0) || N_::uphill(u, eb - ea, dbeta, dbeta_log2e));
   if (accept) {
-    if (s.tiled) swap_rows(TiledField<R>(s.x, s.n, s.d), tiled_offset<R>(a, s.d), tiled_offset<R>(b, s.d), s.d);
+    if (s.layout == STATE_TILE_ROWS) swap_rows(TiledField<R>(s.x, s.n, s.d), tiled_offset<R>(a, s.d), tiled_offset<R>(b, s.d), s.d);
+    else if (s.layout == STATE_TILE_LINES) swap_rows(LineField<R>(s.x, s.n, s.d), line_offset<R>(a, s.d), line_offset<R>(b, s.d), s.d);
     else swap_rows(Field<R>(s.x, s.n, s.d), ea_off, eb_off, s.d);
     swap_rows(fe, ea_off, eb_off, s.n_terms);
   }
@@ -92,7 +93,7 @@
 }
 
 template <typename R>
-hipError_t launch(void *x, void *energy, long long n, int d, int n_terms, bool tiled_state, const void *ladder, int n_rungs,
+hipError_t launch(void *x, void *energy, long long n, int d, int n_terms, int state_layout, const void *ladder, int n_rungs,
                   unsigned long long round, unsigned long long chain_offset, unsigned long long seed,
                   unsigned long long *pair_counts, hipStream_t stream) {
   SwapArgs<R> s;
@@ -110,7 +111,7 @@
   s.seed_hi = (uint32_t)(seed >> 32);
   s.d = d;
   s.n_terms = n_terms;
-  s.tiled = tiled_state ? 1 : 0;
+  s.layout = state_layout;
   if (n_pairs == 0) return hipSuccess;
   const long long per_pair = std::min<long long>((s.rung_chains + kSwapThreads - 1) / kSwapThreads, std::max(kSwapBlocks / n_pairs, 1));
   hipLaunchKernelGGL(k_replica_swap<R>, dim3((unsigned)per_pair, (unsigned)n_pairs), dim3(kSwapThreads), 0, stream, s);
@@ -183,7 +184,7 @@
   ME_HIP(e, hipSetDevice(e->device));
   const auto swap = e->dtype == ME_F32 ? launch<float> : launch<double>;
   for (int i = 0; i < n_rounds; ++i) {
-    ME_HIP(e, swap(e->x.get(), e->energy.get(), e->n, e->d, e->n_terms, e->x_tiled, e->ladder.table.get(), e->ladder.n_rungs, e->ladder.round,
+    ME_HIP(e, swap(e->x.get(), e->energy.get(), e->n, e->d, e->n_terms, e->x_layout, e->ladder.table.get(), e->ladder.n_rungs, e->ladder.round,
                    e->chain_offset, e->seed, e->ladder.pair_counts.get<unsigned long long>(), e->stream));
     e->ladder.round += 1;
   }
```

Result: slower. 16.67 billion (-13.6%).
